# jayleicn/ClipBERT

Measured on AMD Instinct MI355X. Metric: clips/sec/node (2×2 frames, 224px, L_txt=32) at 1/2/4/8 MI355X, higher is better.
Workload: dtype bf16; 1 GPU; MSRVTT retrieval training step (msrvtt_ret_base_resnet50.json; BASELINE configs[1]/[2] family) at the metric's shape: 16 videos x N_clip=2 x N_frame=2 uint8 frames 224px + 2 texts/video (pos+neg, r=2) L_txt=32 per GPU = 32 clips, 64 frames, 64 (text, clip) pairs per step; ImageNorm + fwd + lse-pooling loss + bwd + all-reduce + clip + AdamW in the timed step; clips folded into one forward; mode=train, videos_per_gpu=16, n_clips=2, n_frames=2, img_size=224, txt_len=32, texts_per_video=2, pairs_per_gpu=64, score_agg_func=lse, clips_folded=True, input=uint8 frames in HBM, parallelism=dp1, hip_graph=True, replay_plan=eager hyper-parameter upload + one hipGraph, n_graphs=1, dropout=True

## Files before the change

clipbert_amd/_lib.py:

```python
import ctypes as C
import os

HERE = os.path.dirname(os.path.abspath(__file__))
LIB_PATH = os.path.join(HERE, "lib", "libclipbert_hip.so")

CB_F32, CB_BF16 = 0, 1
ACT_NONE, ACT_RELU, ACT_GELU, ACT_TANH = 0, 1, 2, 3
SPLITK_WS_COUNTER_BYTES = 65536
ACT_GELU_SAVE_GRAD, ACT_SAVED_GRAD = 4, 5
ROWK, ROWK_GATHER, KROW, KROW_TAPS, KROW_GATHER = 0, 1, 2, 3, 4
(HP_LR, HP_BETA1, HP_BETA2, HP_EPS, HP_WD, HP_BC1, HP_BC2, HP_MAX_NORM, HP_GRAD_SCALE, HP_SKIP, HP_COUNT) = range(11)
OPT_ADAMW, OPT_ADAM, OPT_ADAMAX = 0, 1, 2
YUV_LAYOUTS = {"i420": 0, "nv12": 1}
YUV_MATRICES = {"bt601": 0, "bt601-full": 1, "bt709": 2, "bt709-full": 3}

vp, i32, i64, f32, u64 = C.c_void_p, C.c_int32, C.c_int64, C.c_float, C.c_uint64


class GemmDesc(C.Structure):
    _fields_ = [
        ("dtype", i32), ("M", i32), ("N", i32), ("K", i32), ("a_mode", i32), ("b_mode", i32),
        ("A", vp), ("B", vp), ("lda", i64), ("ldb", i64), ("a_tab", vp), ("b_tab", vp),
        ("R", i32), ("S", i32), ("Cin", i32), ("H", i32), ("W", i32),
        ("sH", i64), ("sW", i64), ("flip_taps", i32), ("schedule", i32),
        ("C", vp), ("ldc", i64), ("c_rowmap", vp), ("c_f32", i32), ("accumulate", i32),
        ("split_k", i32), ("act", i32), ("scale", vp), ("shift", vp), ("residual", vp), ("ldr", i64),
        ("relu_after", i32), ("zero_fill_pitch", i32), ("mask", vp), ("ldm", i64), ("C2", vp), ("ldc2", i64),
        ("alpha", f32), ("dropout_p", f32), ("dropout_seed", u64), ("dropout_seed_ptr", vp), ("tile", i32),
        ("xcd_order", i32), ("a_bytes", i64), ("b_bytes", i64), ("gelu_grad_pre", vp), ("ld_gelu", i64), ("a_rowsum", vp),
        ("batch", i32), ("relu_bwd", i32), ("batch_stride_a", i64), ("batch_stride_b", i64), ("batch_stride_c", i64),
        ("batch_stride_rowsum", i64), ("post_scale", vp), ("post_scale2", vp), ("splitk_ws", vp), ("splitk_ws_bytes", i64),
        ("sq_slots", vp), ("sq_slots_n", i64),
    ]


class Res2Desc(C.Structure):
    _fields_ = [("x", vp), ("out", vp), ("w1", vp), ("w2", vp), ("w3", vp), ("wsc", vp),
                ("scale1", vp), ("shift1", vp), ("scale2", vp), ("shift2", vp), ("scale3", vp), ("shift3", vp),
                ("scale_sc", vp), ("shift_sc", vp), ("N", i32), ("H", i32), ("W", i32), ("cin", i32)]


_SIGNATURES = {
    "cb_gemm": [C.POINTER(GemmDesc), vp],
    "cb_res2_block": [C.POINTER(Res2Desc), vp],
    "cb_stem_pool": [vp, vp, vp, vp, vp, i32, i32, i32, i32, i32, i32, i32, vp],
    "cb_stem_pool_u8": [vp, vp, vp, vp, vp, vp, vp, i32, i32, i32, i32, i32, i32, i32, vp],
    "cb_gemm_plan": [vp, i32, vp],
    "cb_gemm_group": [vp, i32, vp],
    "cb_gemm_workspace_bytes": [vp, vp],
    "cb_build_pixel_table": [vp, i32, i32, i32, i32, i32, i64, i64, i64, vp],
    "cb_stem_pack": [i32, vp, i32, vp, vp, vp, i32, i32, i32, i32, i32, i32, vp],
    "cb_resize_pack_u8": [i32, vp, i64, vp, vp, i32, i32, vp, vp, vp, i32, i32, i32, i32, vp],
    "cb_resize_pack_yuv420": [i32, vp, i64, vp, vp, i32, i32, i32, vp, vp, vp, i32, i32, i32, i32, vp],
    "cb_image_norm": [vp, vp, vp, vp, i64, i64, vp],
    "cb_maxpool_fwd": [i32, vp, vp, i32, i32, i32, i32, i32, i32, i32, i32, i32, i32, vp],
    "cb_maxpool2_bwd": [i32, vp, vp, vp, vp, i32, i32, i32, i32, i32, i32, i32, vp],
    "cb_relu_scale_bwd": [i32, vp, vp, vp, vp, vp, vp, vp, i64, i32, vp],
    "cb_layernorm_fwd": [i32, vp, vp, vp, vp, vp, vp, i64, i32, f32, i32, i32, i32, vp],
    "cb_layernorm_bwd": [i32, vp, vp, vp, vp, vp, vp, vp, vp, i64, i32, vp, f32, u64, vp, i32, i32, i32, vp],
    "cb_layernorm_bwd_part": [i32, vp, vp, vp, vp, vp, vp, vp, i32, i64, i32, vp, f32, u64, vp, i32, i32, i32, vp],
    "cb_ln_partials_reduce": [vp, vp, vp, vp, i32, i32, i32, vp],
    "cb_comm_unique_id": [vp],
    "cb_comm_init": [i32, i32, vp],
    "cb_comm_info": [vp, vp],
    "cb_allreduce_bucket": [vp, i64, i32, vp],
    "cb_reduce_scatter_bucket": [vp, vp, i64, i32, vp],
    "cb_allgather_bucket": [vp, vp, i64, i32, vp],
    "cb_broadcast_bucket": [vp, i64, i32, i32, vp],
    "cb_comm_destroy": [],
    "cb_text_embed_fwd": [i32, vp, vp, vp, vp, vp, vp, vp, vp, vp, vp, i32, i32, i32, i32, f32, vp, vp, i32, vp],
    "cb_visual_embed_fwd": [i32, vp, vp, vp, vp, vp, vp, vp, vp, vp, vp, vp, vp, i32, i32, i32, i32, i32,
                            i32, i32, i32, f32, vp, vp],
    "cb_text_embed_bwd": [i32, vp, vp, vp, vp, vp, i32, i32, i32, i32, i64, i32, vp],
    "cb_head_loss": [i32, vp, vp, vp, vp, vp, i64, i32, f32, vp],
    "cb_retrieval_scores": [vp, vp, i64, i32, vp],
    "cb_sq_sum_fold": [vp, vp, i32, vp, i64, vp, vp, i32, vp],
    "cb_mean_fwd": [vp, i64, vp, vp],
    "cb_mean_bwd": [vp, i64, vp, vp],
    "cb_counter_add": [vp, i64, vp],
    "cb_zero": [vp, i64, vp],
    "cb_zero_ranges": [vp, vp, i32, vp],
    "cb_copy_ranges": [vp, vp, vp, i32, vp],
    "cb_visual_embed_bwd": [i32, vp, vp, vp, vp, vp, vp, vp, i32, i32, i32, i32, i32, i32, i32, i32, vp],
    "cb_attention_fwd": [i32, vp, vp, vp, vp, i32, i32, i32, f32, u64, vp, vp],
    "cb_attention_bwd": [i32, vp, vp, vp, vp, vp, vp, vp, i32, i32, i32, f32, u64, vp, vp],
# ... 65 lines not shown
```

clipbert_amd/csrc/common.hip:

```cpp
#include "common.h"

#include <stdarg.h>
#include <stdio.h>

namespace {
thread_local char g_err[512] = "";
}

int cb_fail(const char* fmt, ...) {
    va_list ap;
    va_start(ap, fmt);
    vsnprintf(g_err, sizeof(g_err), fmt, ap);
    va_end(ap);
    return -1;
}

int cb_launch_status(const char* what) {
    hipError_t e = hipGetLastError();
    if (e != hipSuccess) return cb_fail("%s: kernel launch failed: %s", what, hipGetErrorString(e));
    return 0;
}

extern "C" const char* cb_last_error(void) { return g_err; }
extern "C" int cb_version(void) { return 13; }
```

clipbert_amd/csrc/gemm.hip:

```cpp

#include "gemm8_impl.h"
#include "gemm_stream_impl.h"
#include <stdio.h>
#include <vector>

using namespace cbgemm;

namespace cbgemm {
extern template int launch_gemm<float, 64, 64, 2>(const GP&, bool, hipStream_t);
extern template int launch_gemm<bf16, 128, 128, 2>(const GP&, bool, hipStream_t);
extern template int launch_gemm<bf16, 128, 64, 2>(const GP&, bool, hipStream_t);
extern template int launch_gemm<bf16, 64, 64, 3>(const GP&, bool, hipStream_t);
extern template int launch_gemm<bf16, 128, 128, 1, 2>(const GP&, bool, hipStream_t);
extern template int launch_gemm_group<float, 64, 64, 2, 1>(const GroupArgs&, int, hipStream_t);
extern template int launch_gemm_group<bf16, 64, 64, 3, 1>(const GroupArgs&, int, hipStream_t);
extern template int launch_gemm_group<bf16, 128, 128, 1, 2>(const GroupArgs&, int, hipStream_t);
#define CB_G8_DECL(BM, BN, WGM, WGN, NST)                                                             \
    extern template int launch_gemm8_fwd<BM, BN, WGM, WGN, NST>(const GP&, int, float*, hipStream_t);   \
    extern template int launch_gemm8_dgrad<BM, BN, WGM, WGN, NST>(const GP&, int, float*, hipStream_t); \
    extern template int launch_gemm8_wgrad<BM, BN, WGM, WGN, NST>(const GP&, int, float*, hipStream_t);
CB_G8_DECL(256, 256, 2, 4, 2)
CB_G8_DECL(128, 256, 2, 4, 3)
CB_G8_DECL(256, 128, 4, 2, 3)
#undef CB_G8_DECL
// ... 78 lines not shown
#pragma unroll
        for (int r = 0; r < 8; ++r) v[r] += t[r];
    }
    if (p.scale) load8(p.scale + n, sc);
    if (p.shift) load8(p.shift + n, sh);
    const int64_t orow = p.c_rowmap ? (int64_t)p.c_rowmap[m] : (int64_t)m;
    epilogue8<T>(p, v, sc, sh, m, orow, n);
}

template <int BM, int BN, int WGM, int WGN, int NST>
int launch8(int form, const GP& p, int mode, float* ws, hipStream_t st) {
    if (form == 1) return launch_gemm8_fwd<BM, BN, WGM, WGN, NST>(p, mode, ws, st);
    if (form == 2) return launch_gemm8_dgrad<BM, BN, WGM, WGN, NST>(p, mode, ws, st);
    return launch_gemm8_wgrad<BM, BN, WGM, WGN, NST>(p, mode, ws, st);
}

int gemm_prepare(const cb_gemm_desc* d, Prepared& out) {
    CB_REQUIRE(d != nullptr, "cb_gemm: null descriptor");
    CB_REQUIRE(d->dtype == CB_F32 || d->dtype == CB_BF16, "cb_gemm: bad dtype %d", d->dtype);
    CB_REQUIRE(d->M >= 0 && d->N >= 0 && d->K >= 0, "cb_gemm: negative dims");
    CB_REQUIRE(d->A && d->B && d->C, "cb_gemm: null operand");
    const int esz = d->dtype == CB_BF16 ? 2 : 4;
    const int eps = 16 / esz;
    GP& p = out.p;
    p = GP{};
    p.A = d->A; p.B = d->B; p.C = d->C; p.C2 = d->C2; p.residual = d->residual; p.mask = d->mask;
    p.dact_pre = d->gelu_grad_pre; p.ldd = d->ld_gelu; p.a_rowsum = d->a_rowsum;
    p.relu_bwd = d->relu_bwd != 0; p.post_scale = d->post_scale; p.post_scale2 = d->post_scale2;
    if (p.relu_bwd) {
        CB_REQUIRE(d->mask && (!d->c_f32 || d->dtype == CB_F32) && !d->scale && !d->shift && d->act == CB_ACT_NONE && d->dropout_p <= 0.f && !d->relu_after &&
                   !d->gelu_grad_pre && (d->split_k <= 1),
                   "cb_gemm: relu_bwd needs a mask and excludes scale/shift/act/dropout/relu_after/gelu_grad_pre/split_k and an fp32 C next to bf16 operands");
        CB_REQUIRE((!d->post_scale || aligned16(d->post_scale)) && (!d->post_scale2 || aligned16(d->post_scale2)),
                   "cb_gemm: post_scale vectors must be 16-byte aligned");
    } else {
        CB_REQUIRE(!d->post_scale && !d->post_scale2, "cb_gemm: post_scale / post_scale2 need relu_bwd");
    }
    p.batch = d->batch > 1 ? d->batch : 1;
    p.bs_a = d->batch_stride_a * esz; p.bs_b = d->batch_stride_b * esz;
    p.bs_c = d->batch_stride_c * (d->c_f32 ? 4 : esz); p.bs_r = d->batch_stride_rowsum;
    if (p.batch > 1) {
        CB_REQUIRE(!d->C2 && !d->residual && !d->mask && !d->gelu_grad_pre && !d->a_tab && !d->b_tab && !d->c_rowmap,
                   "cb_gemm: batch > 1 supports plain operands only (no residual / mask / second output / gather / row map)");
        CB_REQUIRE((d->batch_stride_a * esz) % 16 == 0 && (d->batch_stride_b * esz) % 16 == 0 && (p.bs_c % 16) == 0,
                   "cb_gemm: batch strides must keep 16-byte alignment");
    }
    CB_REQUIRE(!d->a_rowsum || (d->a_mode == CB_KROW && d->b_mode == CB_KROW), "cb_gemm: a_rowsum needs the weight-gradient form (A and B both CB_KROW)");
    p.scale = d->scale; p.shift = d->shift; p.a_tab = d->a_tab; p.b_tab = d->b_tab; p.c_rowmap = d->c_rowmap; p.zfill = d->zero_fill_pitch;
    p.lda = d->lda; p.ldb = d->ldb; p.ldc = d->ldc; p.ldc2 = d->ldc2; p.ldr = d->ldr; p.ldm = d->ldm;
    p.sH = d->sH; p.sW = d->sW;
    p.M = d->M; p.N = d->N; p.K = d->K;
    p.a_mode = d->a_mode; p.b_mode = d->b_mode;
    p.R = d->R > 0 ? d->R : 1; p.S = d->S > 0 ? d->S : 1; p.Ct = d->Cin; p.H = d->H; p.W = d->W; p.flip = d->flip_taps;
    CB_REQUIRE(d->accumulate >= 0 && d->accumulate <= 2 && (d->accumulate != 2 || d->dtype == CB_BF16), "cb_gemm: bad accumulate %d (2 = first writer: bf16 problems)", d->accumulate);
    p.c_f32 = d->c_f32; p.accumulate = d->accumulate == 1; p.split_k = d->split_k > 0 ? d->split_k : 1;
    p.act = d->act; p.relu_after = d->relu_after;
    p.alpha = d->alpha == 0.f ? 1.f : d->alpha;
    p.dropout_p = d->dropout_p; p.seed = d->dropout_seed; p.seed_ptr = d->dropout_seed_ptr;
    const int bk = d->dtype == CB_BF16 ? Tr<bf16>::BK : Tr<float>::BK;
    p.ktiles = (d->K + bk - 1) / bk;
    {
        const bool ok = d->dtype == CB_BF16 && !d->c_f32 && (int64_t)d->M * (d->ldc > d->ldc2 ? d->ldc : d->ldc2) * 2 * (p.batch) < 0xffffffffll && !d->c_rowmap;
        p.wt = ok ? switches().wt : 0;
    }
    {
        const bool fe_off = switches().fast_epi_off;
        p.fast_epi = 0;
        auto rows_ok = [&](const void* q, int64_t ld) { return q == nullptr || (ld % 8 == 0 && aligned16(q) && (int64_t)d->M * ld * 2 < 0x7fffffffll); };
        const bool wg_store = !fe_off && d->dtype == CB_BF16 && d->c_f32 && d->a_mode == CB_KROW && d->accumulate != 1 && p.alpha == 1.f && !d->scale && !d->shift &&
                              d->act == CB_ACT_NONE && !d->C2 && !d->residual && !d->mask && !d->gelu_grad_pre && d->dropout_p <= 0.f && !d->relu_after && !d->c_rowmap &&
                              !d->zero_fill_pitch && !d->relu_bwd && d->N % 8 == 0 && d->ldc % 8 == 0 && aligned16(d->C) && (int64_t)d->M * d->ldc * 4 < 0xffffffffll;
        if (wg_store) p.fast_epi = FAST_EPI_F32;
        p.sq_slots = nullptr;
        if (d->sq_slots) {
            const int64_t need = (int64_t)((d->M + 63) / 64) * ((d->N + 63) / 64) * p.batch;
            CB_REQUIRE(wg_store, "cb_gemm: sq_slots needs a bf16 weight-gradient form storing an aligned fp32 C with a plain epilogue (accumulate 0 / 2)");
            CB_REQUIRE(d->sq_slots_n >= need, "cb_gemm: sq_slots_n %lld < %lld (one slot per 64x64 tile and batch member)", (long long)d->sq_slots_n, (long long)need);
            p.sq_slots = d->sq_slots;
        }
        const bool plain = !wg_store && !fe_off && p.wt == 1 && p.batch == 1 && d->accumulate != 1 && p.alpha == 1.f && !d->zero_fill_pitch && !d->a_rowsum &&
                           d->N % 8 == 0 && d->ldc % 8 == 0 && aligned16(d->C) && (!d->shift || aligned16(d->shift)) && (!d->scale || aligned16(d->scale)) &&
                           rows_ok(d->residual, d->ldr) && rows_ok(d->mask, d->ldm) && rows_ok(d->gelu_grad_pre, d->ld_gelu) &&
                           !(d->mask && d->gelu_grad_pre);
        if (plain && d->relu_bwd) {
            const bool ok = d->C2 && d->post_scale && d->ldc2 % 8 == 0 && aligned16(d->C2) && (int64_t)d->M * d->ldc2 * 2 < 0xffffffffll;
            const int flags = EF_RBWD | (d->residual ? EF_RES : 0) | (d->post_scale2 ? EF_PS2 : 0);
            if (ok)
                for (int i = 1; i < FAST_EPI_N; ++i)
                    if (FAST_EPI_COMBOS[i] == flags) { p.fast_epi = i; break; }
        } else if (plain) {
            int flags = 0;
            bool ok = true;
            if (d->scale) flags |= EF_SCALE;
            if (d->shift) flags |= EF_SHIFT;
            if (d->act == CB_ACT_RELU) flags |= EF_RELU;
            else if (d->act == CB_ACT_GELU_SAVE_GRAD && d->C2) flags |= EF_GELU2;
            else if (d->act == CB_ACT_GELU && !d->C2) flags |= EF_GELU1;
            else if (d->act == CB_ACT_SAVED_GRAD && d->gelu_grad_pre) flags |= EF_MULAUX;
            else if (d->act != CB_ACT_NONE) ok = false;
            if (d->C2 && !(flags & EF_GELU2)) ok = false;
            if (d->C2) ok = ok && d->ldc2 % 8 == 0 && aligned16(d->C2) && (int64_t)d->M * d->ldc2 * 2 < 0xffffffffll;
            if (d->gelu_grad_pre && !(flags & EF_MULAUX)) ok = false;
            if (d->dropout_p > 0.f) flags |= EF_DROP;
            if (d->residual) flags |= EF_RES;
            if (d->relu_after) flags |= EF_RELU_AFTER;
            if (d->mask) flags |= EF_MASK;
            if (ok)
                for (int i = 1; i < FAST_EPI_N; ++i)
                    if (FAST_EPI_COMBOS[i] == flags) { p.fast_epi = i; break; }
        }
    }
    const bool a_krow = d->a_mode == CB_KROW;
    const bool b_krow = d->b_mode == CB_KROW || d->b_mode == CB_KROW_TAPS || d->b_mode == CB_KROW_GATHER;
    CB_REQUIRE(d->a_mode == CB_ROWK || d->a_mode == CB_ROWK_GATHER || d->a_mode == CB_KROW, "cb_gemm: bad a_mode %d", d->a_mode);
    CB_REQUIRE(d->b_mode == CB_ROWK || b_krow, "cb_gemm: bad b_mode %d", d->b_mode);
    const int taps = p.R * p.S;
    const bool tapped = d->a_mode == CB_ROWK_GATHER || d->b_mode == CB_KROW_TAPS || d->b_mode == CB_KROW_GATHER;
    if (tapped) {
        CB_REQUIRE(p.Ct > 0, "cb_gemm: Cin (channels per tap) must be set for conv modes");
        CB_REQUIRE(p.Ct % eps == 0, "cb_gemm: channels per tap (%d) must be a multiple of %d", p.Ct, eps);
    }
    const int64_t lim = 0x7fffffffll;
    bool fast = d->a_bytes > 0 && d->b_bytes > 0 && d->a_bytes < lim && d->b_bytes < lim && aligned16(d->A) && aligned16(d->B);
    if (d->a_mode == CB_ROWK_GATHER) {
        CB_REQUIRE(d->a_tab, "cb_gemm: a_tab missing");
        CB_REQUIRE(d->K == taps * p.Ct, "cb_gemm: K (%d) != R*S*Cin (%d)", d->K, taps * p.Ct);
        fast = fast && (p.R == 1 || d->sH % eps == 0) && (p.S == 1 || d->sW % eps == 0);
    } else if (d->a_mode == CB_ROWK) {
        fast = fast && (d->lda % eps == 0) && (d->K % eps == 0);
    } else {
        const int64_t need = ((int64_t)(d->K - 1) * d->lda + (d->M + eps - 1) / eps * eps) * esz;
        fast = fast && (d->lda % eps == 0) && (d->M % eps == 0 || need <= d->a_bytes);
    }
    if (d->b_mode == CB_ROWK) {
        fast = fast && (d->ldb % eps == 0) && (d->K % eps == 0);
    } else if (d->b_mode == CB_KROW) {
        const int64_t need = ((int64_t)(d->K - 1) * d->ldb + (d->N + eps - 1) / eps * eps) * esz;
        fast = fast && (d->ldb % eps == 0) && (d->N % eps == 0 || need <= d->b_bytes);
    } else if (d->b_mode == CB_KROW_TAPS) {
        CB_REQUIRE(d->K == taps * p.Ct, "cb_gemm: K (%d) != R*S*Ct (%d)", d->K, taps * p.Ct);
        fast = fast && (d->ldb % eps == 0) && (d->N % eps == 0);
    } else {
        CB_REQUIRE(d->b_tab, "cb_gemm: b_tab missing");
        CB_REQUIRE(d->N == taps * p.Ct, "cb_gemm: N (%d) != R*S*Cin (%d)", d->N, taps * p.Ct);
        fast = fast && (p.R == 1 || d->sH % eps == 0) && (p.S == 1 || d->sW % eps == 0);
    }
    p.a_bytes = (uint32_t)(fast ? d->a_bytes : 0);
    p.b_bytes = (uint32_t)(fast ? d->b_bytes : 0);
    CB_REQUIRE(d->tile >= 0 && d->tile <= 9, "cb_gemm: bad tile %d", d->tile);
    CB_REQUIRE(d->xcd_order >= 0 && d->xcd_order <= 2, "cb_gemm: bad xcd_order %d", d->xcd_order);
    CB_REQUIRE(d->dropout_p >= 0.f && d->dropout_p < 1.f, "cb_gemm: dropout_p out of range");
    const int cesz = d->c_f32 ? 4 : esz;
    bool cv = (d->ldc % 4 == 0) && ((reinterpret_cast<uintptr_t>(d->C) % (4 * cesz)) == 0);
    if (d->C2) cv = cv && (d->ldc2 % 4 == 0) && ((reinterpret_cast<uintptr_t>(d->C2) % (4 * esz)) == 0);
    if (d->residual) cv = cv && (d->ldr % 4 == 0) && ((reinterpret_cast<uintptr_t>(d->residual) % (4 * esz)) == 0);
    if (d->mask) cv = cv && (d->ldm % 4 == 0) && ((reinterpret_cast<uintptr_t>(d->mask) % (4 * esz)) == 0);
    if (d->gelu_grad_pre) cv = cv && (d->ld_gelu % 4 == 0) && ((reinterpret_cast<uintptr_t>(d->gelu_grad_pre) % (4 * esz)) == 0);
    if (d->scale) cv = cv && aligned16(d->scale);
    if (d->shift) cv = cv && aligned16(d->shift);
// ... 50 lines not shown
        return cb_launch_status("cb_gemm (split-K reduce)");
    }
    if (d->dtype == CB_F32) return launch_gemm<float, 64, 64, 2>(p, pr.fast, st);
    CB_STAMP_ASSIGN(p, d, lp.tile, p.split_k, 0, 0, 1);
    if (lp.tile == 4) return launch_gemm<bf16, 128, 128, 1, 2>(p, pr.fast, st);
    if (lp.tile == 1) return launch_gemm<bf16, 128, 128, 2>(p, pr.fast, st);
    if (lp.tile == 3) return launch_gemm<bf16, 128, 64, 2>(p, pr.fast, st);
    return launch_gemm<bf16, 64, 64, 3>(p, pr.fast, st);
}

int gemm_run(const cb_gemm_desc* d, const Prepared& pr, void* stream) {
    LaunchPlan lp;
    const int rc = gemm_choose(d, pr, true, false, lp);
    if (lp.tile != 0 && switches().trace) trace_plan(d, pr, lp);
    return rc != 0 ? rc : gemm_launch(d, pr, lp, cb_stream(stream));
}
}

extern "C" int cb_gemm(const cb_gemm_desc* d, void* stream) {
    Prepared pr;
    bool empty;
    if (int rc = gemm_validate(d, pr, empty)) return rc;
    return empty ? 0 : gemm_run(d, pr, stream);
}

extern "C" int cb_gemm_plan(const cb_gemm_desc* d, int32_t use_table, int32_t* out4) {
    CB_REQUIRE(out4 != nullptr, "cb_gemm_plan: null output");
    out4[0] = out4[1] = out4[2] = out4[3] = 0;
    Prepared pr;
    LaunchPlan lp;
    bool empty;
    if (int rc = gemm_validate(d, pr, empty)) return rc;
    if (empty) return 0;
    if (int rc = gemm_choose(d, pr, use_table != 0, false, lp)) return rc;
    out4[0] = lp.tile; out4[1] = lp.split_k; out4[2] = lp.sched; out4[3] = lp.xcd_remap ? 1 : 2;
    return 0;
}

extern "C" int cb_gemm_workspace_bytes(const cb_gemm_desc* d, int64_t* bytes) {
    CB_REQUIRE(d != nullptr && bytes != nullptr, "cb_gemm_workspace_bytes: null argument");
    *bytes = 0;
    Prepared pr;
    LaunchPlan lp;
    bool empty;
    if (int rc = gemm_validate(d, pr, empty)) return rc;
    if (empty) return 0;
    if (int rc = gemm_choose(d, pr, true, true, lp)) return rc;
    if (lp.slab) *bytes = (int64_t)lp.split_k * pr.p.batch * d->M * d->N * 4 + CB_SPLITK_WS_COUNTER_BYTES;
    return 0;
}

namespace {
int group_class(const cb_gemm_desc* d, const Prepared& pr) {
    if (!pr.fast || d->zero_fill_pitch || d->tile >= 5 || d->tile == 1 || d->tile == 3) return -1;
    if (d->batch > 1 || d->a_rowsum) {
        const bool ok = d->dtype == CB_BF16 && pr.form == FORM_WGRAD && d->split_k <= 1 && d->tile != 2 && !d->c_rowmap;
        return ok ? GC_WGRAD_RS : -1;
    }
    return GROUP_CLASS_OF[pr.form];
}

struct GroupItem { const cb_gemm_desc* d; Prepared pr; int cls; };

bool group_split_free(const GroupItem& it) { return a_reduction_major(it.pr.form) && it.d->c_f32 && it.d->accumulate != 0 && it.pr.epi_scale_only; }
inline int64_t group_tiles(const cb_gemm_desc* d, int B) { return (int64_t)((d->M + B - 1) / B) * ((d->N + B - 1) / B); }

double group_cost(const std::vector<GroupItem*>& g, int tile, int s, int* splits) {
    const int B = tile == 4 ? 128 : 64;
    int maxkt = 1;
    for (auto* it : g) maxkt = it->pr.p.ktiles > maxkt ? it->pr.p.ktiles : maxkt;
    const int kt_target = (maxkt + s - 1) / s;
    int64_t W = 0;
    int kt_per_max = 1;
    double atom = 0.0;
    for (size_t i = 0; i < g.size(); ++i) {
        const cb_gemm_desc* d = g[i]->d;
        const int kt = g[i]->pr.p.ktiles;
        int si = g[i]->pr.p.split_k;
        if (group_split_free(*g[i])) {
            si = (kt + kt_target / 2) / kt_target;
            if (si < 1) si = 1;
            while (si > 1 && kt / si < 4) --si;
        }
        if (si > kt) si = kt > 0 ? kt : 1;
        splits[i] = si;
        W += group_tiles(d, B) * si;
        const int per = (kt + si - 1) / si;
        kt_per_max = per > kt_per_max ? per : kt_per_max;
        if (si > 1) atom += (double)d->M * d->N * 4.0 * si;
    }
    static const int cus = [] {
        int dev = 0, n = 0;
        return (hipGetDevice(&dev) == hipSuccess && hipDeviceGetAttribute(&n, hipDeviceAttributeMultiprocessorCount, dev) == hipSuccess && n > 0) ? n : 256;
    }();
    const int64_t per_cu = (W + cus - 1) / cus;
    double unit;
    if (tile == 4) unit = per_cu <= 1 ? 1.0 : 0.77;
    else unit = per_cu <= 1 ? 0.45 : (per_cu == 2 ? 0.35 : 0.30);
    return 8.0 + (double)per_cu * kt_per_max * unit + atom / 2.0e6;
}

struct GroupPlan {
    int tile = 2;
    int splits[GROUP_MAX];
    float* slab = nullptr;
    int* cnt = nullptr;
};
// ... 155 lines not shown
```

clipbert_amd/csrc/gemm_choose.h:

```cpp
#pragma once
#include "gemm_impl.h"
#include <cmath>
#include "gemm_tuned.h"
#include "gemm_model.h"

namespace cbgemm {
bool skinny_covers(const cb_gemm_desc* d, const GP& p);
}
using namespace cbgemm;

namespace {
inline int env_int(const char* name, int dflt) { const char* v = getenv(name); return v != nullptr ? atoi(v) : dflt; }
struct Switches {
    bool trace = getenv("CB_GEMM_TRACE") != nullptr;
    bool no_tuned = getenv("CB_GEMM_NO_TUNED") != nullptr;
    bool no_model = getenv("CB_GEMM_NO_MODEL") != nullptr;
    bool no_xcd_remap = getenv("CB_GEMM_NO_XCD_REMAP") != nullptr;
    bool no_stream = getenv("CB_GEMM_NO_STREAM") != nullptr;
    bool no_group = getenv("CB_GEMM_NO_GROUP") != nullptr;
    bool no_skinny = getenv("CB_GEMM_NO_SKINNY") != nullptr;
    bool group_slab_off = env_int("CB_GROUP_SLAB", 1) == 0;
    bool fast_epi_off = env_int("CB_GEMM_FAST_EPI", 1) == 0;
    int wt = env_int("CB_GEMM_WT", 1);
};
// ... 11 lines not shown
};
Form operand_form(int a_mode, int b_mode, int taps) {
    if (a_mode == CB_KROW) return b_mode == CB_KROW ? FORM_WGRAD : (b_mode == CB_KROW_GATHER ? FORM_WGRAD_GATHER : FORM_WGRAD_OTHER);
    if (b_mode == CB_ROWK) return a_mode == CB_ROWK ? FORM_FWD : FORM_FWD_GATHER;
    if (a_mode == CB_ROWK && (b_mode == CB_KROW || (b_mode == CB_KROW_TAPS && taps == 1))) return FORM_DGRAD;
    if (a_mode == CB_ROWK_GATHER && b_mode == CB_KROW_TAPS) return FORM_DGRAD_TAPS;
    return FORM_DGRAD_OTHER;
}
inline bool a_reduction_major(Form f) { return f >= FORM_WGRAD; }
inline int model_form(Form f) { return f >= FORM_WGRAD ? 2 : (f >= FORM_DGRAD ? 1 : 0); }
const int FORM8_OF[8] = {1, 1, 2, 2, 0, 3, 3, 0};
const int GROUP_CLASS_OF[8] = {GC_FWD, GC_FWD_GATHER, -1, -1, -1, GC_WGRAD, GC_WGRAD_GATHER, -1};

struct Prepared {
    GP p;
    bool fast, cv8;
    Form form;
    int taps;
    bool epi_scale_only;
    bool atomics_ok;
};
constexpr int GROUP_COUNTERS = CB_SPLITK_WS_COUNTER_BYTES / (int)sizeof(int);
inline int64_t splitk_payload_bytes(int64_t ws_bytes) { return ws_bytes > CB_SPLITK_WS_COUNTER_BYTES ? ws_bytes - CB_SPLITK_WS_COUNTER_BYTES : 0; }
inline int* splitk_counters(void* ws, int64_t ws_bytes) {
    return ws && ws_bytes > CB_SPLITK_WS_COUNTER_BYTES ? reinterpret_cast<int*>(reinterpret_cast<unsigned char*>(ws) + (ws_bytes - CB_SPLITK_WS_COUNTER_BYTES)) : nullptr;
}

struct ModelPick { int tile = 0, split = 0, sched = 0; double us = 1e300; };
const int MODEL_TILE_ID[7] = {2, 3, 1, 4, 5, 6, 7};
const int MODEL_BM[7] = {64, 128, 128, 128, 256, 128, 256};
const int MODEL_BN[7] = {64, 64, 128, 128, 256, 256, 128};

double model_us(int ti, int form, int64_t M, int64_t N, int64_t K, int64_t batch, int s, bool taps, bool m2, int c_esz) {
    using namespace cbgemm;
    const double* g = MODEL_G;
    const int64_t wg = ((M + MODEL_BM[ti] - 1) / MODEL_BM[ti]) * ((N + MODEL_BN[ti] - 1) / MODEL_BN[ti]) * batch * s;
    const int64_t kt = ((K + 63) / 64 + s - 1) / s;
    const double r = (double)wg / (256.0 * MODEL_OCC[ti]);
    const double q = ti >= 4 ? g[7] : g[3];
    const double rounds = q * std::ceil(r - 1e-9) + (1.0 - q) * (r > 1.0 ? r : 1.0);
    const double ck = MODEL_C[ti][form] * (1.0 + g[4] * (taps ? 1 : 0)) * (1.0 + g[8] * (m2 ? 1 : 0));
    const double ab = (double)(M * K + N * K) * 2.0 * batch, cb = (double)M * N * batch * c_esz;
    const double red = (ti >= 4 && s > 1) ? (double)M * N * batch * s * 8.0 : 0.0;
    const double atom = (ti < 4 && s > 1) ? (double)M * N * batch * s * 4.0 : 0.0;
    return MODEL_A[ti] + rounds * (MODEL_B[ti][form] + kt * ck) + ab / (g[0] * 1e6) + cb / (g[5] * 1e6) + red / (g[1] * 1e6) + atom / (g[2] * 1e6) +
           g[6] * (m2 ? 1 : 0);
}

ModelPick model_pick(const cb_gemm_desc* d, const Prepared& pr, bool can8, int64_t ws_bytes, bool free_split) {
    const GP& p = pr.p;
    const int form = model_form(pr.form), split_caller = p.split_k;
    const bool taps = pr.taps > 1;
    const int c_esz = d->c_f32 ? 4 : 2;
    const int64_t M = d->M, N = d->N, K = d->K, batch = p.batch;
    ModelPick best;
    auto consider = [&](int ti, int s, int sched) {
        const double us = model_us(ti, form, M, N, K, batch, s, taps, sched == 3, c_esz);
        if (us < best.us) { best.us = us; best.tile = MODEL_TILE_ID[ti]; best.split = s; best.sched = sched; }
    };
    static const int SPLITS4[] = {1, 2, 3, 4, 6, 8, 12, 16, 24, 32, 48};
    for (int ti = 0; ti < 4; ++ti) {
        if (N <= 64 && ti >= 2) continue;
        consider(ti, split_caller, 0);
        if (free_split)
            for (int s : SPLITS4)
                if (s != split_caller && s <= (p.ktiles / 4 > 1 ? p.ktiles / 4 : 1)) consider(ti, s, 0);
    }
    if (can8)
        for (int ti = 4; ti < 7; ++ti) {
            const int64_t tiles = ((M + MODEL_BM[ti] - 1) / MODEL_BM[ti]) * ((N + MODEL_BN[ti] - 1) / MODEL_BN[ti]) * batch;
            int cand[3] = {1, 0, 0};
            int n = 1;
            for (int target : {256, 512}) {
                const int s = (int)std::lround((double)target / (double)tiles);
                if (s > 1 && p.ktiles / s >= 2 && (int64_t)s * batch * M * N * 4 <= ws_bytes && s != cand[1]) cand[n++] = s;
            }
            for (int i = 0; i < n; ++i) { consider(ti, cand[i], 1); consider(ti, cand[i], 3); }
        }
    return best;
}

int stream_variant(const cb_gemm_desc* d, const Prepared& pr) {
    const GP& p = pr.p;
    if (!pr.fast || !pr.cv8 || d->dtype != CB_BF16 || pr.form != FORM_FWD || p.batch > 1 || p.split_k > 1) return -1;
    if (d->c_f32 || d->accumulate || d->c_rowmap || d->zero_fill_pitch || d->a_rowsum || d->gelu_grad_pre || d->dropout_p > 0.f || d->mask || d->relu_bwd ||
        d->C2) return -1;
    if (d->K % 8 != 0 || d->M < 64) return -1;
    if ((int64_t)d->M * (d->N > d->K ? d->N : d->K) * 2 >= 0x7fffffffll) return -1;
    if (p.ktiles == 1 && d->N % 256 == 0) return 0;
    if (p.ktiles == 2 && d->N % 128 == 0) return 1;
    return -1;
}

struct LaunchPlan {
    int tile = 0;
    int split_k = 1;
    int sched = 0;
    bool xcd_remap = false;
    bool slab = false;
    bool c_vec8 = false;
    int form8 = 0;
    int picked = 0;
};
struct Pick { int tile = 0, split = 0, sched = 0; };
constexpr int64_t WS_UNLIMITED = (int64_t)1 << 60;
constexpr int STREAM_MIN_ROWS = 32768;

int gemm_choose(const cb_gemm_desc* d, const Prepared& pr, bool use_table, bool assume_ws, LaunchPlan& lp) {
    const Switches& sw = switches();
    const GP& p = pr.p;
    const bool bf = d->dtype == CB_BF16, explicit_tile = d->tile != 0;
    const int split_caller = p.split_k;
    lp = LaunchPlan{};
    const bool covers9 = skinny_covers(d, p);
    CB_REQUIRE(d->tile != 9 || covers9, "cb_gemm: tile 9 (few rows) does not cover this problem (bf16, A k-contiguous, B k-contiguous or aligned reduction-major, no batch / K split / row sums)");
    if (d->tile == 9 || (!explicit_tile && use_table && !sw.no_skinny && covers9 && d->M <= 64)) { lp.tile = 9; return 0; }
    const int sv = stream_variant(d, pr);
    CB_REQUIRE(d->tile != 8 || sv >= 0, "cb_gemm: tile 8 (streaming) does not cover this problem (M=%d N=%d K=%d modes %d/%d)", d->M, d->N, d->K, d->a_mode, d->b_mode);
    const cbgemm::TunedEntry* tabled =
        (bf && use_table && !sw.no_tuned) ? cbgemm::tuned_lookup(d->a_mode, d->b_mode, d->M, d->N, d->K, p.batch, pr.taps, split_caller) : nullptr;
    if (d->tile == 8 || (!explicit_tile && use_table && !sw.no_stream && !tabled && sv >= 0 && d->M >= STREAM_MIN_ROWS && d->N <= 512)) {
        lp.tile = 8; lp.sched = sv; lp.c_vec8 = true;
        return 0;
    }

    const int form8 = (bf && pr.fast && pr.cv8 && (pr.form != FORM_DGRAD_TAPS || p.Ct % 64 == 0)) ? FORM8_OF[pr.form] : 0;
    const int64_t ws_room = assume_ws ? splitk_payload_bytes(WS_UNLIMITED)
                                      : (d->splitk_ws && aligned16(d->splitk_ws) ? splitk_payload_bytes(d->splitk_ws_bytes) : 0);
    const bool free_split = !explicit_tile && a_reduction_major(pr.form) && pr.atomics_ok;
    const int xcd = d->xcd_order != 0 ? d->xcd_order : (tabled ? tabled->xcd : 0);
    auto model = [&](bool allow8) {
        Pick k;
        if (!bf || sw.no_model) return k;
        const ModelPick mp = model_pick(d, pr, allow8 && form8 != 0, ws_room, free_split && !d->a_rowsum && p.batch == 1);
        k.tile = mp.tile; k.split = (mp.tile >= 5 || mp.split != split_caller) ? mp.split : 0; k.sched = mp.sched;
        return k;
    };
    auto split8 = [&](const Pick& k) { return explicit_tile ? split_caller : (k.split > 0 ? k.split : 1); };
    Pick pick;
    if (explicit_tile) pick.tile = d->tile;
    else if (tabled) pick = Pick{tabled->tile, tabled->new_split, tabled->sched};
    if (pick.tile >= 5 && form8 == 0) pick = Pick{};
    if (pick.tile == 0) pick = model(true);
    if (pick.tile >= 5 && d->sq_slots && split8(pick) > 1) pick = model(false);
    if (pick.tile >= 5) {
        int split = split8(pick);
        if (split > p.ktiles) split = p.ktiles;
        if (split > 1) {
            const int per = (p.ktiles + split - 1) / split;
            split = (p.ktiles + per - 1) / per;
            if ((int64_t)split * p.batch * d->M * d->N * 4 > ws_room) {
                pick = model(!explicit_tile);
                split = pick.split > 0 ? pick.split : 1;
            }
        }
        if (pick.tile >= 5) {
            lp.tile = lp.picked = pick.tile; lp.form8 = form8;
            lp.split_k = split; lp.slab = split > 1;
            lp.sched = d->schedule > 0 ? d->schedule : (pick.sched > 0 ? pick.sched : 3);
            lp.c_vec8 = true;
            lp.xcd_remap = !sw.no_xcd_remap && xcd != 2;
            CB_REQUIRE(d->schedule >= 0 && d->schedule <= 3, "cb_gemm: bad schedule %d", d->schedule);
            return 0;
        }
    }

    lp.picked = pick.tile; lp.form8 = form8;
    lp.tile = pick.tile == 0 ? 2 : pick.tile;
    if (!bf) lp.tile = 2;
    else if ((lp.tile == 1 || lp.tile == 4) && d->N <= 64) lp.tile = 3;
    lp.xcd_remap = !sw.no_xcd_remap && xcd != 2;
    int split = split_caller;
    if (d->tile >= 5 && split > 1 && !pr.atomics_ok) split = 1;
    if (d->accumulate == 2 || d->sq_slots) split = 1;
    if (pick.split > 0 && free_split) split = pick.split;
    if (split > 1) {
        CB_REQUIRE(d->c_f32 && d->accumulate == 1, "cb_gemm: split_k > 1 needs an fp32 output that is accumulated into (accumulate = 1)");
        CB_REQUIRE(pr.epi_scale_only, "cb_gemm: split_k > 1 supports only scale/alpha in the epilogue");
        if (split > p.ktiles) split = p.ktiles;
// ... 10 lines not shown
```

clipbert_amd/csrc/gemm_impl.h:

```cpp
#pragma once
#include "common.h"
#include <stdlib.h>
#include <type_traits>

namespace cbgemm {


constexpr int NTHREADS = 256;

template <typename T> struct Tr;
template <> struct Tr<bf16> { static constexpr int EPS = 8, BK = 64, SEGS = 8, ROWB = 128, RB = 8; };
template <> struct Tr<float> { static constexpr int EPS = 4, BK = 32, SEGS = 8, ROWB = 144, RB = 4; };

template <typename T> __device__ __forceinline__ int lds_off(int row, int seg);
template <> __device__ __forceinline__ int lds_off<bf16>(int row, int seg) { return row * 128 + ((seg ^ (row & 7)) << 4); }
template <> __device__ __forceinline__ int lds_off<float>(int row, int seg) { return row * 144 + (seg << 4); }

struct GP {
    const void* A; const void* B; void* C; void* C2; const void* residual; const void* mask;
    const void* dact_pre; float* a_rowsum; int64_t ldd;
    int relu_bwd; const float* post_scale; const float* post_scale2;
    int batch; int64_t bs_a, bs_b, bs_c, bs_r;
    const float* scale; const float* shift;
    const cb_pixel* a_tab; const cb_pixel* b_tab; const int32_t* c_rowmap;
    int64_t lda, ldb, ldc, ldc2, ldr, ldm, sH, sW;
    int M, N, K;
    int a_mode, b_mode;
    int R, S, Ct, H, W, flip;
    int c_f32, accumulate, split_k, act, relu_after;
    float alpha, dropout_p;
    uint64_t seed;
    const uint64_t* seed_ptr;
    short c_vec, c_vec8;
    short xcd_remap;
    short wt;
    int zfill;
    uint32_t a_bytes, b_bytes;
    int ktiles;
    int slab_base, cnt_base;
    int fast_epi;
    float* sq_slots;
#ifdef CB_STAMPS
    unsigned long long* stamps;
#endif
};

enum { EF_SCALE = 1, EF_SHIFT = 2, EF_RELU = 4, EF_GELU2 = 8, EF_DROP = 16, EF_RES = 32, EF_RELU_AFTER = 64, EF_MASK = 128, EF_MULAUX = 256,
       EF_RBWD = 512,
       EF_PS2 = 1024,
       EF_F32 = 2048,
       EF_GELU1 = 4096 };
constexpr int FAST_EPI_COMBOS[] = {
    -1,
    0,
    EF_SHIFT,
    EF_SHIFT | EF_GELU2,
    EF_SHIFT | EF_DROP | EF_RES,
    EF_SHIFT | EF_RES,
    EF_MULAUX,
    EF_RES,
    EF_SCALE | EF_SHIFT | EF_RELU,
    EF_SCALE | EF_SHIFT,
    EF_SCALE | EF_SHIFT | EF_RES | EF_RELU_AFTER,
    EF_SCALE | EF_MASK,
    EF_RBWD,
    EF_RBWD | EF_RES,
    EF_RBWD | EF_PS2,
    EF_RBWD | EF_PS2 | EF_RES,
    EF_F32,
    EF_SHIFT | EF_GELU1,
};
constexpr int FAST_EPI_F32 = 16;
constexpr int FAST_EPI_N = sizeof(FAST_EPI_COMBOS) / sizeof(int);

#ifdef CB_STAMPS
constexpr int CB_STAMP_WGS = 512, CB_STAMP_REC = 6, CB_STAMP_HDR = 3;
constexpr int CB_STAMP_AREA = CB_STAMP_HDR + CB_STAMP_WGS * CB_STAMP_REC;
struct Stamps {
    unsigned long long t[5];
    __device__ __forceinline__ void mark(int i) { t[i] = __builtin_amdgcn_s_memrealtime(); }
    __device__ __forceinline__ void flush(unsigned long long* area, unsigned lin, int tid) {
        if (!area || tid != 0) return;
        asm volatile("s_waitcnt vmcnt(0)" ::: "memory");
        const unsigned long long t4 = __builtin_amdgcn_s_memrealtime();
        atomicMin(area, t[0]);
        atomicMax(area + 1, t4);
        atomicAdd(area + 2, 1ull);
        if (lin < (unsigned)CB_STAMP_WGS) {
            unsigned long long* r = area + CB_STAMP_HDR + (size_t)lin * CB_STAMP_REC;
            r[0] = t[0]; r[1] = t[1]; r[2] = t[2]; r[3] = t[3]; r[4] = t4;
            unsigned hw;
            asm volatile("s_getreg_b32 %0, hwreg(HW_REG_HW_ID)" : "=s"(hw));
            unsigned xcc;
            asm volatile("s_getreg_b32 %0, hwreg(HW_REG_XCC_ID)" : "=s"(xcc));
            r[5] = ((unsigned long long)xcc << 32) | hw;
        }
    }
};
#define CB_STAMP_DECL() Stamps stamps_
#define CB_STAMP(i) stamps_.mark(i)
#define CB_STAMP_FLUSH(p, lin, tid) stamps_.flush((p).stamps, (lin), (tid))
#else
#define CB_STAMP_DECL() do {} while (0)
#define CB_STAMP(i) do {} while (0)
#define CB_STAMP_FLUSH(p, lin, tid) do {} while (0)
#endif

template <typename T> __device__ __forceinline__ u32x4 load_guarded(const T* src, int nvalid) {
    constexpr int EPS = Tr<T>::EPS;
    union { u32x4 v; T e[EPS]; } u;
#pragma unroll
    for (int i = 0; i < EPS; ++i) u.e[i] = (i < nvalid) ? src[i] : (T)0.f;
    return u.v;
}

constexpr uint32_t OOB = 0x80000000u;
typedef decltype(__builtin_amdgcn_make_buffer_rsrc((void*)nullptr, (short)0, 0, 0)) rsrc_t;
__device__ __forceinline__ rsrc_t make_rsrc(const void* p, uint32_t bytes) {
    return __builtin_amdgcn_make_buffer_rsrc(const_cast<void*>(p), (short)0, (int)bytes, 0x00020000);
}
__device__ __forceinline__ u32x4 bload16(rsrc_t r, uint32_t off) { return __builtin_amdgcn_raw_buffer_load_b128(r, off, 0, 0); }

struct Opnd {
    const void* base; const cb_pixel* tab; int64_t ld; int mode; uint32_t bytes;
};

template <typename T, int ROWS, bool FAST> struct RowkLoader {
    using X = Tr<T>;
    static constexpr bool TR = false;
    static constexpr bool KROW = false;
    static constexpr int NS = ROWS * X::SEGS / NTHREADS;
    static constexpr int ESZ = (int)sizeof(T);
    static_assert(ROWS * X::SEGS % NTHREADS == 0, "tile/threads mismatch");
    struct Stage { u32x4 r[NS]; };
    int64_t off[NS];
    uint32_t boff[NS];
    int ih[NS], iw[NS];
    bool ok[NS];
    int c, rr, ss;
    bool gather;
    rsrc_t rs;
    const T* base;

    __device__ __forceinline__ void init(const GP& p, const Opnd& o, int row0, int bound, int kt0, int tid) {
        gather = o.mode == CB_ROWK_GATHER;
        base = reinterpret_cast<const T*>(o.base);
        if constexpr (FAST) rs = make_rsrc(o.base, o.bytes);
        int k = kt0 * X::BK + (tid % X::SEGS) * X::EPS;
        c = k; rr = 0; ss = 0;
        if (gather) {
            int tap = k / p.Ct;
            c = k - tap * p.Ct;
            rr = tap / p.S; ss = tap - rr * p.S;
        }
#pragma unroll
        for (int i = 0; i < NS; ++i) {
            int idx = tid + i * NTHREADS;
            int row = row0 + idx / X::SEGS;
            ok[i] = row < bound;
            ih[i] = 0; iw[i] = 0;
            int64_t e = (int64_t)row * o.ld;
            if (gather) {
                cb_pixel px = {0, 0, 0};
                if (ok[i]) px = o.tab[row];
                e = px.off; ih[i] = px.ih0; iw[i] = px.iw0;
            }
            off[i] = e;
            boff[i] = ok[i] ? (uint32_t)e * (uint32_t)ESZ : OOB;
        }
    }
    template <bool CHECK> __device__ __forceinline__ void load(Stage& st, const GP& p) {
        const bool kv = gather ? (rr < p.R) : (c < p.K);
        const int klim = gather ? p.Ct : p.K;
        const int64_t tapoff = gather ? (rr * p.sH + ss * p.sW) : 0;
#pragma unroll
// ... 25 lines not shown
template <typename T, int ROWS, bool FAST> struct KrowLoader {
    using X = Tr<T>;
    static constexpr bool TR = false;
    static constexpr bool KROW = true;
    static constexpr int RBLK = ROWS / X::RB;
    static constexpr int CNT = RBLK * (X::BK / 4);
    static constexpr int NI = (CNT + NTHREADS - 1) / NTHREADS;
    static constexpr int ESZ = (int)sizeof(T);
    struct Stage { u32x4 r[NI][4]; };
    int mode, bound;
    int64_t ld;
    const cb_pixel* tab;
    const T* base;
    rsrc_t rs;
    int kb0[NI];
    int co[NI], tap[NI];
    int row[NI];
    int rr[NI], ss[NI];
    int64_t rowoff[NI];
    bool act[NI];

    __device__ __forceinline__ void init(const GP& p, const Opnd& o, int row0, int bnd, int kt0, int tid) {
        mode = o.mode; bound = bnd; ld = o.ld; tab = o.tab;
        base = reinterpret_cast<const T*>(o.base);
        if constexpr (FAST) rs = make_rsrc(o.base, o.bytes);
#pragma unroll
        for (int it = 0; it < NI; ++it) {
            int b = tid + it * NTHREADS;
            act[it] = b < CNT;
            int rb = b % RBLK, kb = b / RBLK;
            row[it] = row0 + rb * X::RB;
            kb0[it] = kt0 * X::BK + kb * 4;
            rowoff[it] = row[it];
            co[it] = kb0[it]; tap[it] = 0; rr[it] = 0; ss[it] = 0;
            if (mode == CB_KROW_TAPS) {
                tap[it] = kb0[it] / p.Ct;
                co[it] = kb0[it] - tap[it] * p.Ct;
            } else if (mode == CB_KROW_GATHER) {
                int tp = row[it] / p.Ct;
                int ch = row[it] - tp * p.Ct;
                rr[it] = tp / p.S; ss[it] = tp - rr[it] * p.S;
                rowoff[it] = rr[it] * p.sH + ss[it] * p.sW + ch;
            }
        }
    }
    template <bool CHECK> __device__ __forceinline__ void load(Stage& st, const GP& p) {
        u32x4 z = {0u, 0u, 0u, 0u};
#pragma unroll
        for (int it = 0; it < NI; ++it) {
            if (!act[it]) { st.r[it][0] = z; st.r[it][1] = z; st.r[it][2] = z; st.r[it][3] = z; continue; }
            const int nvalid = bound - row[it];
            int64_t ro = rowoff[it];
            if (mode == CB_KROW_TAPS) {
                int tapw = p.flip ? (p.R * p.S - 1 - tap[it]) : tap[it];
                ro = (int64_t)tapw * bound + row[it];
            }
#pragma unroll
            for (int j = 0; j < 4; ++j) {
                const int k = kb0[it] + j;
                bool v = k < p.K && nvalid > 0;
                int64_t e;
                if (mode == CB_KROW_GATHER) {
                    cb_pixel px = {0, 0, 0};
                    if (v) px = tab[k];
                    v = v && (unsigned)(px.ih0 + rr[it]) < (unsigned)p.H && (unsigned)(px.iw0 + ss[it]) < (unsigned)p.W;
                    e = px.off + ro;
                } else if (mode == CB_KROW_TAPS) {
                    e = (int64_t)(co[it] + j) * ld + ro;
                } else {
                    e = (int64_t)k * ld + ro;
                }
                if constexpr (FAST) {
                    st.r[it][j] = bload16(rs, v ? (uint32_t)e * (uint32_t)ESZ : OOB);
                } else {
                    st.r[it][j] = v ? load_guarded<T>(base + e, nvalid) : z;
                }
            }
            kb0[it] += X::BK;
            if (mode == CB_KROW_TAPS) {
                co[it] += X::BK;
                while (co[it] >= p.Ct) { co[it] -= p.Ct; ++tap[it]; }
            }
        }
    }
    __device__ __forceinline__ void store(const Stage& st, unsigned char* tile, int tid) const {
#pragma unroll
        for (int it = 0; it < NI; ++it) {
            int b = tid + it * NTHREADS;
            if (b >= CNT) continue;
            int rb = b % RBLK, kb = b / RBLK;
            int r0 = rb * X::RB;
            if constexpr (sizeof(T) == 2) {
#pragma unroll
                for (int d = 0; d < 4; ++d) {
                    uint32_t a0 = st.r[it][0][d], a1 = st.r[it][1][d], a2 = st.r[it][2][d], a3 = st.r[it][3][d];
                    u32x2 even = {(a0 & 0xffffu) | (a1 << 16), (a2 & 0xffffu) | (a3 << 16)};
                    u32x2 odd = {(a0 >> 16) | (a1 & 0xffff0000u), (a2 >> 16) | (a3 & 0xffff0000u)};
                    *reinterpret_cast<u32x2*>(tile + lds_off<T>(r0 + 2 * d, kb >> 1) + (kb & 1) * 8) = even;
                    *reinterpret_cast<u32x2*>(tile + lds_off<T>(r0 + 2 * d + 1, kb >> 1) + (kb & 1) * 8) = odd;
                }
            } else {
#pragma unroll
                for (int e = 0; e < 4; ++e) {
                    u32x4 o = {st.r[it][0][e], st.r[it][1][e], st.r[it][2][e], st.r[it][3][e]};
                    *reinterpret_cast<u32x4*>(tile + lds_off<T>(r0 + e, kb)) = o;
                }
            }
// ... 91 lines not shown
    const cb_pixel* tab;
    uint32_t ldb;
    uint32_t voff[NI];
    int kb0[NI];
    int co[NI], tap[NI];
    int rr[NI], ss[NI];
    cb_pixel px[NI][KB];
    bool act[NI];
    uint32_t bound;

    __device__ __forceinline__ void init(const GP& p, const Opnd& o, int row0, int bnd, int kt0, int tid) {
        rs = make_rsrc(o.base, o.bytes);
        tab = o.tab; ldb = (uint32_t)o.ld * ESZ; bound = (uint32_t)bnd;
#pragma unroll
        for (int it = 0; it < NI; ++it) {
            const int b = ((tid + SHIFT) % NTHREADS) + it * NTHREADS;
            const int kb = b % NKB, rb = b / NKB;
            const int row = row0 + rb * X::RB;
            act[it] = (b < CNT) && (row < bnd);
            kb0[it] = kt0 * X::BK + kb * KB;
            co[it] = kb0[it]; tap[it] = 0; rr[it] = 0; ss[it] = 0;
            if constexpr (KMODE == KM_PLAIN) {
                voff[it] = ((uint32_t)kb0[it] * (uint32_t)o.ld + (uint32_t)row) * ESZ;
            } else if constexpr (KMODE == KM_TAPS) {
                tap[it] = kb0[it] / p.Ct;
                co[it] = kb0[it] - tap[it] * p.Ct;
                voff[it] = (uint32_t)row * ESZ;
            } else {
                const int tp = row / p.Ct, ch = row - tp * p.Ct;
                rr[it] = tp / p.S; ss[it] = tp - rr[it] * p.S;
                voff[it] = (uint32_t)(rr[it] * (int)p.sH + ss[it] * (int)p.sW + ch) * ESZ;
#pragma unroll
                for (int j = 0; j < KB; ++j) {
                    cb_pixel e = {0, (int16_t)-30000, (int16_t)-30000};
                    if (act[it] && kb0[it] + j < p.K) e = tab[kb0[it] + j];
                    px[it][j] = e;
                }
            }
        }
    }
    template <bool CHECK> __device__ __forceinline__ void load(Stage& st, const GP& p) {
#pragma unroll
        for (int it = 0; it < NI; ++it) {
            if constexpr (KMODE == KM_PLAIN) {
#pragma unroll
                for (int j = 0; j < KB; ++j) {
                    bool v = act[it];
                    if (CHECK) v = v && (kb0[it] + j < p.K);
                    st.r[it][j] = bload16(rs, v ? voff[it] + (uint32_t)j * ldb : OOB);
                }
                voff[it] += X::BK * ldb;
                kb0[it] += X::BK;
            } else if constexpr (KMODE == KM_TAPS) {
                const int tapw = p.flip ? (p.R * p.S - 1 - tap[it]) : tap[it];
                const bool v = act[it] && tap[it] < p.R * p.S;
                const uint32_t base = (uint32_t)co[it] * ldb + (uint32_t)tapw * bound * ESZ + voff[it];
#pragma unroll
                for (int j = 0; j < KB; ++j) st.r[it][j] = bload16(rs, v ? base + (uint32_t)j * ldb : OOB);
                co[it] += X::BK;
                while (co[it] >= p.Ct) { co[it] -= p.Ct; ++tap[it]; }
            } else {
#pragma unroll
                for (int j = 0; j < KB; ++j) {
                    const cb_pixel e = px[it][j];
                    const bool v = (unsigned)(e.ih0 + rr[it]) < (unsigned)p.H && (unsigned)(e.iw0 + ss[it]) < (unsigned)p.W;
                    st.r[it][j] = bload16(rs, v ? (uint32_t)e.off * ESZ + voff[it] : OOB);
                }
                kb0[it] += X::BK;
#pragma unroll
                for (int j = 0; j < KB; ++j) {
                    cb_pixel e = {0, (int16_t)-30000, (int16_t)-30000};
                    if (act[it] && kb0[it] + j < p.K) e = tab[kb0[it] + j];
                    px[it][j] = e;
                }
            }
        }
    }
    __device__ __forceinline__ void store(const Stage& st, unsigned char* tile, int tid) const {
#pragma unroll
        for (int it = 0; it < NI; ++it) {
            const int b = ((tid + SHIFT) % NTHREADS) + it * NTHREADS;
            if (b >= CNT) continue;
            const int kb = b % NKB, rb = b / NKB;
            const int r0 = rb * X::RB;
            if constexpr (sizeof(T) == 2 && KB == 8) {
#pragma unroll
                for (int d = 0; d < 4; ++d) {
                    u32x4 even, odd;
#pragma unroll
                    for (int q = 0; q < 4; ++q) {
                        even[q] = __builtin_amdgcn_perm(st.r[it][2 * q + 1][d], st.r[it][2 * q][d], 0x05040100u);
                        odd[q] = __builtin_amdgcn_perm(st.r[it][2 * q + 1][d], st.r[it][2 * q][d], 0x07060302u);
                    }
                    *reinterpret_cast<u32x4*>(tile + lds_off<T>(r0 + 2 * d, kb)) = even;
                    *reinterpret_cast<u32x4*>(tile + lds_off<T>(r0 + 2 * d + 1, kb)) = odd;
                }
            } else if constexpr (sizeof(T) == 2 && KB == 2) {
#pragma unroll
                for (int d = 0; d < 4; ++d) {
                    const uint32_t even = __builtin_amdgcn_perm(st.r[it][1][d], st.r[it][0][d], 0x05040100u);
                    const uint32_t odd = __builtin_amdgcn_perm(st.r[it][1][d], st.r[it][0][d], 0x07060302u);
                    *reinterpret_cast<uint32_t*>(tile + lds_off<T>(r0 + 2 * d, kb >> 2) + (kb & 3) * 4) = even;
                    *reinterpret_cast<uint32_t*>(tile + lds_off<T>(r0 + 2 * d + 1, kb >> 2) + (kb & 3) * 4) = odd;
                }
            } else if constexpr (sizeof(T) == 2) {
#pragma unroll
                for (int d = 0; d < 4; ++d) {
// ... 45 lines not shown
    static constexpr int CH = ROWS / 8;
    static constexpr int NS = CH * X::BK / NTHREADS;
    static_assert(CH * X::BK % NTHREADS == 0, "tile/threads mismatch");
    static constexpr uint32_t ESZ = 2;
    struct Stage { u32x4 r[NS]; };
    rsrc_t rs;
    const cb_pixel* tab;
    uint32_t ldb, bound;
    uint32_t voff[NS];
    int kl[NS];
    int co[NS], tap[NS];
    int rr, ss;
    cb_pixel px[NS];
    bool act[NS];

    __device__ __forceinline__ void init(const GP& p, const Opnd& o, int row0, int bnd, int kt0, int tid) {
        rs = make_rsrc(o.base, o.bytes);
        tab = o.tab; ldb = (uint32_t)o.ld * ESZ; bound = (uint32_t)bnd;
        rr = 0; ss = 0;
#pragma unroll
        for (int i = 0; i < NS; ++i) {
            const int idx = tid + i * NTHREADS;
            const int chunk = idx % CH, kline = idx / CH;
            const int row = row0 + chunk * 8;
            act[i] = row < bnd;
            kl[i] = kt0 * X::BK + kline;
            co[i] = kl[i]; tap[i] = 0;
            if constexpr (KMODE == KM_PLAIN) {
                voff[i] = ((uint32_t)kl[i] * (uint32_t)o.ld + (uint32_t)row) * ESZ;
            } else if constexpr (KMODE == KM_TAPS) {
                tap[i] = kl[i] / p.Ct;
                co[i] = kl[i] - tap[i] * p.Ct;
                voff[i] = (uint32_t)row * ESZ;
            } else {
                const int tp = row / p.Ct, ch = row - tp * p.Ct;
                rr = tp / p.S; ss = tp - rr * p.S;
                voff[i] = (uint32_t)(rr * (int)p.sH + ss * (int)p.sW + ch) * ESZ;
                cb_pixel e = {0, (int16_t)-30000, (int16_t)-30000};
                if (act[i] && kl[i] < p.K) e = tab[kl[i]];
                px[i] = e;
            }
        }
    }
    template <bool CHECK> __device__ __forceinline__ void load(Stage& st, const GP& p) {
#pragma unroll
        for (int i = 0; i < NS; ++i) {
            if constexpr (KMODE == KM_PLAIN) {
                bool v = act[i];
                if (CHECK) v = v && (kl[i] < p.K);
                st.r[i] = bload16(rs, v ? voff[i] : OOB);
                voff[i] += X::BK * ldb;
                kl[i] += X::BK;
            } else if constexpr (KMODE == KM_TAPS) {
                const int tapw = p.flip ? (p.R * p.S - 1 - tap[i]) : tap[i];
                const bool v = act[i] && tap[i] < p.R * p.S;
                st.r[i] = bload16(rs, v ? (uint32_t)co[i] * ldb + (uint32_t)tapw * bound * ESZ + voff[i] : OOB);
                co[i] += X::BK;
                while (co[i] >= p.Ct) { co[i] -= p.Ct; ++tap[i]; }
            } else {
                const cb_pixel e = px[i];
                const bool v = (unsigned)(e.ih0 + rr) < (unsigned)p.H && (unsigned)(e.iw0 + ss) < (unsigned)p.W;
                st.r[i] = bload16(rs, v ? (uint32_t)e.off * ESZ + voff[i] : OOB);
                kl[i] += X::BK;
                cb_pixel nx = {0, (int16_t)-30000, (int16_t)-30000};
                if (act[i] && kl[i] < p.K) nx = tab[kl[i]];
                px[i] = nx;
            }
        }
    }
    __device__ __forceinline__ void store(const Stage& st, unsigned char* tile, int tid) const {
#pragma unroll
        for (int i = 0; i < NS; ++i) {
            const int idx = tid + i * NTHREADS;
            const int chunk = idx % CH, kline = idx / CH;
            *reinterpret_cast<u32x4*>(tile + kline * (ROWS * 2) + ((chunk ^ tr_chunk_swz<ROWS>(kline)) << 4)) = st.r[i];
        }
    }
};

struct TileId { int bx, by, bz; };
__device__ __forceinline__ TileId tile_id(const GP& p) {
    TileId t;
    if (!p.xcd_remap) { t.bx = blockIdx.x; t.by = blockIdx.y; t.bz = blockIdx.z; return t; }
    const unsigned gx = gridDim.x, gy = gridDim.y;
    const unsigned total = gx * gy * gridDim.z;
    const unsigned lin = blockIdx.x + gx * (blockIdx.y + gy * blockIdx.z);
    const unsigned xcd = lin & 7u, i = lin >> 3;
    const unsigned q = total >> 3, r = total & 7u;
    const unsigned l2 = (xcd < r ? xcd * (q + 1) : r * (q + 1) + (xcd - r) * q) + i;
    t.bx = (int)(l2 % gx);
    const unsigned rest = l2 / gx;
    t.by = (int)(rest % gy);
    t.bz = (int)(rest / gy);
    return t;
}

__device__ __forceinline__ void apply_batch(GP& p, TileId& t) {
    if (p.batch <= 1) return;
    const int b = t.bz / p.split_k;
    t.bz -= b * p.split_k;
    const int64_t oa = b * p.bs_a, ob = b * p.bs_b;
    p.A = reinterpret_cast<const unsigned char*>(p.A) + oa;
    p.B = reinterpret_cast<const unsigned char*>(p.B) + ob;
    p.C = reinterpret_cast<unsigned char*>(p.C) + b * p.bs_c;
    if (p.a_bytes) p.a_bytes -= (uint32_t)oa;
    if (p.b_bytes) p.b_bytes -= (uint32_t)ob;
    if (p.a_rowsum) p.a_rowsum += b * p.bs_r;
}

template <typename T>
__device__ __forceinline__ float act_of(int act, float v) {
    if constexpr (sizeof(T) == 2) {
        if (act == CB_ACT_GELU || act == CB_ACT_GELU_SAVE_GRAD) return gelu_erf_pk(v);
    }
    return apply_act(act, v);
}

template <typename T>
__device__ __forceinline__ float scale_shift(float x, float sc, float sh) {
    if constexpr (sizeof(T) == 2) return __builtin_fmaf(x, sc, sh);
    else {
#pragma clang fp contract(off)
        const float t = x * sc;
        return t + sh;
    }
}

template <typename T>
__device__ __forceinline__ void epilogue_vec(const GP& p, f32x4 v, int m, int64_t orow, int nb) {
    v = v * p.alpha;
    if (p.relu_bwd) {
        T* c = reinterpret_cast<T*>(p.C) + orow * p.ldc + nb;
        if (p.accumulate) v = v + load4(c);
        if (p.residual) v = v + load4(reinterpret_cast<const T*>(p.residual) + orow * p.ldr + nb);
        const f32x4 mk = load4(reinterpret_cast<const T*>(p.mask) + orow * p.ldm + nb);
#pragma unroll
        for (int r = 0; r < 4; ++r) v[r] = mk[r] > 0.f ? v[r] : 0.f;
        if (p.C2) store4(reinterpret_cast<T*>(p.C2) + orow * p.ldc2 + nb, p.post_scale2 ? v * load4(p.post_scale2 + nb) : v);
        store4(c, p.post_scale ? v * load4(p.post_scale + nb) : v);
        return;
    }
    if (p.scale && p.shift) {
        const f32x4 sc = load4(p.scale + nb), sh = load4(p.shift + nb);
#pragma unroll
        for (int r = 0; r < 4; ++r) v[r] = scale_shift<T>(v[r], sc[r], sh[r]);
    }
    else if (p.scale) v = v * load4(p.scale + nb);
    else if (p.shift) v = v + load4(p.shift + nb);
    if (p.act == CB_ACT_GELU_SAVE_GRAD && p.C2) {
        f32x4 dv;
#pragma unroll
        for (int r = 0; r < 4; ++r) {
            float y, dy;
            if constexpr (sizeof(T) == 2) gelu_erf_both_pk(v[r], y, dy);
            else gelu_erf_both(v[r], y, dy);
            v[r] = y; dv[r] = dy;
        }
        store4(reinterpret_cast<T*>(p.C2) + orow * p.ldc2 + nb, dv);
    } else {
        if (p.C2) store4(reinterpret_cast<T*>(p.C2) + orow * p.ldc2 + nb, v);
        if (p.act != CB_ACT_NONE) {
#pragma unroll
            for (int r = 0; r < 4; ++r) v[r] = act_of<T>(p.act, v[r]);
        }
    }
    if (p.dropout_p > 0.f) {
        v = v * dropout_mult4(p.seed, (uint64_t)m * ((p.N + 3) >> 2) + (nb >> 2), p.dropout_p);
    }
    if (p.residual) v = v + load4(reinterpret_cast<const T*>(p.residual) + orow * p.ldr + nb);
    if (p.relu_after) {
#pragma unroll
        for (int r = 0; r < 4; ++r) v[r] = v[r] > 0.f ? v[r] : 0.f;
    }
    if (p.mask) {
        f32x4 mk = load4(reinterpret_cast<const T*>(p.mask) + orow * p.ldm + nb);
#pragma unroll
        for (int r = 0; r < 4; ++r) v[r] = mk[r] > 0.f ? v[r] : 0.f;
    }
    if (p.dact_pre) {
        f32x4 pr = load4(reinterpret_cast<const T*>(p.dact_pre) + orow * p.ldd + nb);
#pragma unroll
        for (int r = 0; r < 4; ++r) v[r] *= p.act == CB_ACT_SAVED_GRAD ? pr[r] : gelu_erf_grad(pr[r]);
    }
    if (p.c_f32) {
        float* c = reinterpret_cast<float*>(p.C) + orow * p.ldc + nb;
        if (p.split_k > 1) {
#pragma unroll
            for (int r = 0; r < 4; ++r) atomicAdd(c + r, v[r]);
        } else {
            if (p.accumulate) v = v + load4(c);
            store4(c, v);
        }
    } else {
        T* c = reinterpret_cast<T*>(p.C) + orow * p.ldc + nb;
        if (p.accumulate) v = v + load4(c);
        store4(c, v);
    }
}

template <typename T>
__device__ __forceinline__ void epilogue_elem(const GP& p, float x, int m, int64_t orow, int n) {
    x *= p.alpha;
    if (p.relu_bwd) {
        T* c = reinterpret_cast<T*>(p.C) + orow * p.ldc + n;
        if (p.accumulate) x += to_f32(*c);
        if (p.residual) x += to_f32(reinterpret_cast<const T*>(p.residual)[orow * p.ldr + n]);
        x = to_f32(reinterpret_cast<const T*>(p.mask)[orow * p.ldm + n]) > 0.f ? x : 0.f;
        if (p.C2) reinterpret_cast<T*>(p.C2)[orow * p.ldc2 + n] = from_f32<T>(p.post_scale2 ? x * p.post_scale2[n] : x);
        *c = from_f32<T>(p.post_scale ? x * p.post_scale[n] : x);
        return;
    }
    if (p.scale && p.shift) x = scale_shift<T>(x, p.scale[n], p.shift[n]);
    else if (p.scale) x *= p.scale[n];
    else if (p.shift) x += p.shift[n];
    if (p.act == CB_ACT_GELU_SAVE_GRAD && p.C2) {
        float dx;
        if constexpr (sizeof(T) == 2) gelu_erf_both_pk(x, x, dx);
        else gelu_erf_both(x, x, dx);
        reinterpret_cast<T*>(p.C2)[orow * p.ldc2 + n] = from_f32<T>(dx);
    } else {
        if (p.C2) reinterpret_cast<T*>(p.C2)[orow * p.ldc2 + n] = from_f32<T>(x);
        x = act_of<T>(p.act, x);
    }
    if (p.dropout_p > 0.f) x *= dropout_mult1(p.seed, (uint64_t)m * ((p.N + 3) >> 2) + (n >> 2), n & 3, p.dropout_p);
    if (p.residual) x += to_f32(reinterpret_cast<const T*>(p.residual)[orow * p.ldr + n]);
    if (p.relu_after) x = x > 0.f ? x : 0.f;
    if (p.mask) x = to_f32(reinterpret_cast<const T*>(p.mask)[orow * p.ldm + n]) > 0.f ? x : 0.f;
    if (p.dact_pre) {
        const float t = to_f32(reinterpret_cast<const T*>(p.dact_pre)[orow * p.ldd + n]);
        x *= p.act == CB_ACT_SAVED_GRAD ? t : gelu_erf_grad(t);
    }
    if (p.c_f32) {
        float* c = reinterpret_cast<float*>(p.C) + orow * p.ldc + n;
        if (p.split_k > 1) atomicAdd(c, x);
        else *c = p.accumulate ? (*c + x) : x;
    } else {
        T* c = reinterpret_cast<T*>(p.C) + orow * p.ldc + n;
        *c = from_f32<T>(p.accumulate ? (to_f32(*c) + x) : x);
    }
}

__device__ __forceinline__ void load8(const float* q, float (&v)[8]) {
    f32x4 a = load4(q), b = load4(q + 4);
#pragma unroll
    for (int r = 0; r < 4; ++r) { v[r] = a[r]; v[4 + r] = b[r]; }
}
__device__ __forceinline__ void load8(const bf16* q, float (&v)[8]) {
    bf16x8 x = *reinterpret_cast<const bf16x8*>(q);
#pragma unroll
    for (int r = 0; r < 8; ++r) v[r] = (float)x[r];
}
__device__ __forceinline__ void store8(float* q, const float (&v)[8]) {
    f32x4 a = {v[0], v[1], v[2], v[3]}, b = {v[4], v[5], v[6], v[7]};
    store4(q, a); store4(q + 4, b);
}
__device__ __forceinline__ void store8(bf16* q, const float (&v)[8]) {
    bf16x8 x;
#pragma unroll
    for (int r = 0; r < 8; ++r) x[r] = (bf16)v[r];
    *reinterpret_cast<bf16x8*>(q) = x;
}

template <int AUX = 16 >
__device__ __forceinline__ void store8_wt(void* base, int64_t elem_off, const float (&v)[8]) {
    union { bf16x8 x; u32x4 r; } u;
#pragma unroll
    for (int r = 0; r < 8; ++r) u.x[r] = (bf16)v[r];
    const rsrc_t rs = __builtin_amdgcn_make_buffer_rsrc(base, (short)0, (int)0xffffffffu, 0x00020000);
    __builtin_amdgcn_raw_buffer_store_b128(u.r, rs, (uint32_t)(elem_off * 2), 0, AUX);
}

template <typename T>
__device__ __forceinline__ void zero_patch8(T* base, int64_t ld, int64_t orow, int n, int pitch) {
    const float z[8] = {0.f, 0.f, 0.f, 0.f, 0.f, 0.f, 0.f, 0.f};
    store8(base + (orow + 1) * ld + n, z);
    store8(base + (orow + pitch) * ld + n, z);
    store8(base + (orow + pitch + 1) * ld + n, z);
}

#ifdef CB_EPI_NOSTORE
#define CB_EPI_ST(...) do { if (p.alpha == 12345.f) { __VA_ARGS__; } } while (0)
#else
#define CB_EPI_ST(...) do { __VA_ARGS__; } while (0)
#endif
template <typename T, int EPF = 0>
__device__ __forceinline__ void epilogue8(const GP& p, float (&v)[8], const float (&sc)[8], const float (&sh)[8],
                                          int m, int64_t orow, int n, bf16x8 rpre = bf16x8{}, bf16x8 apre = bf16x8{}) {
    auto load_res = [&](float (&t)[8]) {
        if constexpr (EPF == 2) {
#pragma unroll
            for (int r = 0; r < 8; ++r) t[r] = (float)rpre[r];
        } else load8(reinterpret_cast<const T*>(p.residual) + orow * p.ldr + n, t);
    };
    auto load_aux = [&](const void* base, int64_t ld, float (&t)[8]) {
        if constexpr (EPF >= 1) {
#pragma unroll
            for (int r = 0; r < 8; ++r) t[r] = (float)apre[r];
        } else load8(reinterpret_cast<const T*>(base) + orow * ld + n, t);
    };
#ifdef CB_EPI_NOMATH
    if constexpr (sizeof(T) == 2) {
        if (!p.c_f32 && p.wt) {
            store8_wt(p.C, orow * p.ldc + n, v);
            if (p.C2) store8_wt(p.C2, orow * p.ldc2 + n, v);
            return;
        }
    }
#endif
#pragma unroll
    for (int r = 0; r < 8; ++r) v[r] *= p.alpha;
    if (p.relu_bwd) {
        T* c = reinterpret_cast<T*>(p.C) + orow * p.ldc + n;
        float t[8];
        if (p.accumulate) {
            load8(c, t);
#pragma unroll
            for (int r = 0; r < 8; ++r) v[r] += t[r];
        }
        if (p.residual) {
            load_res(t);
#pragma unroll
            for (int r = 0; r < 8; ++r) v[r] += t[r];
        }
        load_aux(p.mask, p.ldm, t);
#pragma unroll
        for (int r = 0; r < 8; ++r) v[r] = t[r] > 0.f ? v[r] : 0.f;
        if (p.C2) {
            float u[8];
            if (p.post_scale2) {
                load8(p.post_scale2 + n, t);
#pragma unroll
                for (int r = 0; r < 8; ++r) u[r] = v[r] * t[r];
            } else {
#pragma unroll
                for (int r = 0; r < 8; ++r) u[r] = v[r];
            }
            if constexpr (sizeof(T) == 2) {
                if (p.wt) CB_EPI_ST(store8_wt(p.C2, orow * p.ldc2 + n, u));
                else CB_EPI_ST(store8(reinterpret_cast<T*>(p.C2) + orow * p.ldc2 + n, u));
            } else CB_EPI_ST(store8(reinterpret_cast<T*>(p.C2) + orow * p.ldc2 + n, u));
        }
        if (p.post_scale) {
            load8(p.post_scale + n, t);
#pragma unroll
            for (int r = 0; r < 8; ++r) v[r] *= t[r];
        }
        if constexpr (sizeof(T) == 2) {
            if (p.wt) CB_EPI_ST(store8_wt(p.C, orow * p.ldc + n, v));
            else CB_EPI_ST(store8(c, v));
        } else CB_EPI_ST(store8(c, v));
        if (p.zfill) {
            zero_patch8(reinterpret_cast<T*>(p.C), p.ldc, orow, n, p.zfill);
            if (p.C2) zero_patch8(reinterpret_cast<T*>(p.C2), p.ldc2, orow, n, p.zfill);
        }
        return;
    }
    if (p.scale && p.shift) {
#pragma unroll
        for (int r = 0; r < 8; ++r) v[r] = scale_shift<T>(v[r], sc[r], sh[r]);
    } else if (p.scale) {
#pragma unroll
        for (int r = 0; r < 8; ++r) v[r] *= sc[r];
    } else if (p.shift) {
#pragma unroll
        for (int r = 0; r < 8; ++r) v[r] += sh[r];
    }
    const bool save_grad = p.act == CB_ACT_GELU_SAVE_GRAD && p.C2 != nullptr;
    float dv[8];
    if (save_grad) {
#pragma unroll
        for (int r = 0; r < 8; r += 2) {
            if constexpr (sizeof(T) == 2) {
                f32x2 y, dy;
                gelu_erf_both2(f32x2{v[r], v[r + 1]}, y, dy);
                v[r] = y[0]; v[r + 1] = y[1]; dv[r] = dy[0]; dv[r + 1] = dy[1];
            } else {
                gelu_erf_both(v[r], v[r], dv[r]);
                gelu_erf_both(v[r + 1], v[r + 1], dv[r + 1]);
            }
        }
    }
    if (p.C2) {
        const float (&w)[8] = save_grad ? dv : v;
        if constexpr (sizeof(T) == 2) {
            if (p.wt & 2) CB_EPI_ST(store8_wt<18 >(p.C2, orow * p.ldc2 + n, w));
            else if (p.wt) CB_EPI_ST(store8_wt(p.C2, orow * p.ldc2 + n, w));
            else CB_EPI_ST(store8(reinterpret_cast<T*>(p.C2) + orow * p.ldc2 + n, w));
        } else CB_EPI_ST(store8(reinterpret_cast<T*>(p.C2) + orow * p.ldc2 + n, w));
    }
    if (p.act != CB_ACT_NONE && !save_grad) {
#pragma unroll
        for (int r = 0; r < 8; ++r) v[r] = act_of<T>(p.act, v[r]);
    }
    if (p.dropout_p > 0.f) {
        const uint64_t grp = (uint64_t)m * ((p.N + 3) >> 2) + (n >> 2);
        const f32x4 d0 = dropout_mult4(p.seed, grp, p.dropout_p), d1 = dropout_mult4(p.seed, grp + 1, p.dropout_p);
#pragma unroll
        for (int r = 0; r < 4; ++r) { v[r] *= d0[r]; v[4 + r] *= d1[r]; }
    }
    if (p.residual) {
        float t[8];
        load_res(t);
#pragma unroll
        for (int r = 0; r < 8; ++r) v[r] += t[r];
    }
    if (p.relu_after) {
#pragma unroll
        for (int r = 0; r < 8; ++r) v[r] = v[r] > 0.f ? v[r] : 0.f;
    }
    if (p.mask) {
        float t[8];
        load_aux(p.mask, p.ldm, t);
#pragma unroll
        for (int r = 0; r < 8; ++r) v[r] = t[r] > 0.f ? v[r] : 0.f;
    } else if (p.dact_pre) {
        float t[8];
        load_aux(p.dact_pre, p.ldd, t);
        if (p.act == CB_ACT_SAVED_GRAD) {
#pragma unroll
            for (int r = 0; r < 8; ++r) v[r] *= t[r];
        } else {
#pragma unroll
            for (int r = 0; r < 8; ++r) v[r] *= gelu_erf_grad(t[r]);
        }
    }
    if (p.c_f32) {
        float* c = reinterpret_cast<float*>(p.C) + orow * p.ldc + n;
        if (p.accumulate) {
            float t[8];
            load8(c, t);
#pragma unroll
            for (int r = 0; r < 8; ++r) v[r] += t[r];
        }
        CB_EPI_ST(store8(c, v));
    } else {
        T* c = reinterpret_cast<T*>(p.C) + orow * p.ldc + n;
        if (p.accumulate) {
            float t[8];
            load8(c, t);
#pragma unroll
            for (int r = 0; r < 8; ++r) v[r] += t[r];
        }
        if constexpr (sizeof(T) == 2) {
            if (p.wt) CB_EPI_ST(store8_wt(p.C, orow * p.ldc + n, v));
            else CB_EPI_ST(store8(c, v));
        } else CB_EPI_ST(store8(c, v));
    }
    if (p.zfill) {
        if (p.c_f32) zero_patch8(reinterpret_cast<float*>(p.C), p.ldc, orow, n, p.zfill);
        else zero_patch8(reinterpret_cast<T*>(p.C), p.ldc, orow, n, p.zfill);
        if (p.C2) zero_patch8(reinterpret_cast<T*>(p.C2), p.ldc2, orow, n, p.zfill);
    }
}

__device__ __forceinline__ u32x4 pack_bf16x8(const f32x2 (&v)[4]) {
    union { bf16x8 x; u32x4 r; } u;
#pragma unroll
    for (int r = 0; r < 4; ++r) { u.x[2 * r] = (bf16)v[r][0]; u.x[2 * r + 1] = (bf16)v[r][1]; }
    return u.r;
}
__device__ __forceinline__ void unpack_bf16x8(u32x4 raw, f32x2 (&v)[4]) {
    union { u32x4 r; bf16x8 x; } u;
    u.r = raw;
#pragma unroll
    for (int r = 0; r < 4; ++r) v[r] = f32x2{(float)u.x[2 * r], (float)u.x[2 * r + 1]};
}

template <int FLAGS, int NT, int BN, int PR, int NPASS, typename StageFn>
__device__ __forceinline__ void fast_epilogue(const GP& p, unsigned char* smem, int m0, int n0, int tid, StageFn stage, const bf16x8* pre_r = nullptr,
                                              const bf16x8* pre_a = nullptr, int tile_lin = 0) {
    constexpr int SROW = BN * 4 + 16, CPR = BN / 8, ITER = PR * CPR / NT, RSTEP = NT / CPR, NCH = NPASS * ITER;
    static_assert(PR * CPR % NT == 0 && NT % CPR == 0, "chunk map");
    constexpr bool HAS_RES = (FLAGS & EF_RES) != 0, HAS_AUX = (FLAGS & (EF_MASK | EF_MULAUX | EF_RBWD)) != 0;
    constexpr bool ALL = NCH <= 8;
    constexpr bool ROLL = (FLAGS & (EF_GELU2 | EF_GELU1)) != 0 || NPASS > 2;
    const int cc = tid % CPR, n = n0 + cc * 8, rl0 = tid / CPR;
    const bool nok = n < p.N;
    const unsigned char* const read_base = smem + rl0 * SROW + cc * 32;
    const rsrc_t rc = __builtin_amdgcn_make_buffer_rsrc(p.C, (short)0, (int)0xffffffffu, 0x00020000);
    const rsrc_t rc2 = __builtin_amdgcn_make_buffer_rsrc((FLAGS & (EF_GELU2 | EF_RBWD)) ? p.C2 : p.C, (short)0, (int)0xffffffffu, 0x00020000);
    constexpr uint32_t CESZ = (FLAGS & EF_F32) ? 4u : 2u;
    const uint32_t ldcb = (uint32_t)p.ldc * CESZ, ldc2b = (uint32_t)p.ldc2 * 2u, nb = (uint32_t)n * 2u;
    float sq = 0.f;
    const rsrc_t rr = make_rsrc(HAS_RES ? p.residual : p.C, HAS_RES ? (uint32_t)((int64_t)p.M * p.ldr * 2) : 0u);
    const void* auxp = (FLAGS & (EF_MASK | EF_RBWD)) ? p.mask : p.dact_pre;
    const int64_t lda = (FLAGS & (EF_MASK | EF_RBWD)) ? p.ldm : p.ldd;
    const rsrc_t ra = make_rsrc(HAS_AUX ? auxp : p.C, HAS_AUX ? (uint32_t)((int64_t)p.M * lda * 2) : 0u);
    const uint32_t ldrb = (uint32_t)p.ldr * 2u, ldab = (uint32_t)lda * 2u;
    f32x2 sc[4], sh[4];
#pragma unroll
    for (int r = 0; r < 4; ++r) { sc[r] = f32x2{1.f, 1.f}; sh[r] = f32x2{0.f, 0.f}; }
    if (nok) {
        if constexpr ((FLAGS & EF_SCALE) != 0) {
            const f32x4 a = load4(p.scale + n), b = load4(p.scale + n + 4);
            sc[0] = f32x2{a[0], a[1]}; sc[1] = f32x2{a[2], a[3]}; sc[2] = f32x2{b[0], b[1]}; sc[3] = f32x2{b[2], b[3]};
        }
        if constexpr ((FLAGS & EF_SHIFT) != 0) {
            const f32x4 a = load4(p.shift + n), b = load4(p.shift + n + 4);
            sh[0] = f32x2{a[0], a[1]}; sh[1] = f32x2{a[2], a[3]}; sh[2] = f32x2{b[0], b[1]}; sh[3] = f32x2{b[2], b[3]};
        }
        if constexpr ((FLAGS & EF_RBWD) != 0) {
            const f32x4 a = load4(p.post_scale + n), b = load4(p.post_scale + n + 4);
            sc[0] = f32x2{a[0], a[1]}; sc[1] = f32x2{a[2], a[3]}; sc[2] = f32x2{b[0], b[1]}; sc[3] = f32x2{b[2], b[3]};
            if constexpr ((FLAGS & EF_PS2) != 0) {
                const f32x4 c = load4(p.post_scale2 + n), e = load4(p.post_scale2 + n + 4);
                sh[0] = f32x2{c[0], c[1]}; sh[1] = f32x2{c[2], c[3]}; sh[2] = f32x2{e[0], e[1]}; sh[3] = f32x2{e[2], e[3]};
            }
        }
    }
    u32x4 res[HAS_RES ? (ALL ? NCH : ITER) : 1], aux[HAS_AUX ? (ALL ? NCH : ITER) : 1];
    auto request = [&](int h) __attribute__((always_inline)) {
#pragma unroll
        for (int it = 0; it < ITER; ++it) {
            const int m = m0 + h * PR + rl0 + it * RSTEP;
            const bool ok = m < p.M && nok;
            const int slot = (ALL ? h * ITER : 0) + it;
            if constexpr (HAS_RES) {
                if (ALL && pre_r) { union { bf16x8 x; u32x4 r; } u; u.x = pre_r[h * ITER + it]; res[slot] = u.r; }
                else res[slot] = bload16(rr, ok ? (uint32_t)m * ldrb + nb : OOB);
            }
            if constexpr (HAS_AUX) {
                if (ALL && pre_a) { union { bf16x8 x; u32x4 r; } u; u.x = pre_a[h * ITER + it]; aux[slot] = u.r; }
                else aux[slot] = bload16(ra, ok ? (uint32_t)m * ldab + nb : OOB);
            }
        }
    };
    auto chunk = [&](int h, int it, int slot) __attribute__((always_inline)) {
        const int m = m0 + h * PR + rl0 + it * RSTEP;
        if (!(m < p.M && nok)) return;
        const f32x4 a = *reinterpret_cast<const f32x4*>(read_base + it * RSTEP * SROW);
        const f32x4 b = *reinterpret_cast<const f32x4*>(read_base + it * RSTEP * SROW + 16);
        if constexpr ((FLAGS & EF_F32) != 0) {
            union { f32x4 f; u32x4 r; } ua, ub;
            ua.f = a; ub.f = b;
            const uint32_t off = (uint32_t)m * ldcb + (uint32_t)n * 4u;
            __builtin_amdgcn_raw_buffer_store_b128(ua.r, rc, off, 0, 0);
            __builtin_amdgcn_raw_buffer_store_b128(ub.r, rc, off + 16u, 0, 0);
            sq += (a[0] * a[0] + a[1] * a[1]) + (a[2] * a[2] + a[3] * a[3]) + (b[0] * b[0] + b[1] * b[1]) + (b[2] * b[2] + b[3] * b[3]);
            return;
        }
        f32x2 v[4] = {f32x2{a[0], a[1]}, f32x2{a[2], a[3]}, f32x2{b[0], b[1]}, f32x2{b[2], b[3]}};
        if constexpr ((FLAGS & EF_RBWD) != 0) {
            f32x2 t[4];
            if constexpr (HAS_RES) {
                unpack_bf16x8(res[slot], t);
#pragma unroll
                for (int r = 0; r < 4; ++r) v[r] = v[r] + t[r];
            }
            unpack_bf16x8(aux[slot], t);
            f32x2 u[4];
#pragma unroll
            for (int r = 0; r < 4; ++r) {
                v[r] = f32x2{t[r][0] > 0.f ? v[r][0] : 0.f, t[r][1] > 0.f ? v[r][1] : 0.f};
                u[r] = (FLAGS & EF_PS2) != 0 ? v[r] * sh[r] : v[r];
                v[r] = v[r] * sc[r];
            }
            __builtin_amdgcn_raw_buffer_store_b128(pack_bf16x8(u), rc2, (uint32_t)m * ldc2b + nb, 0, 16 );
            __builtin_amdgcn_raw_buffer_store_b128(pack_bf16x8(v), rc, (uint32_t)m * ldcb + nb, 0, 16 );
            return;
        }
#pragma unroll
        for (int r = 0; r < 4; ++r) {
            if constexpr ((FLAGS & EF_SCALE) != 0 && (FLAGS & EF_SHIFT) != 0) v[r] = pk_fma(v[r], sc[r], sh[r]);
            else if constexpr ((FLAGS & EF_SCALE) != 0) v[r] = v[r] * sc[r];
            else if constexpr ((FLAGS & EF_SHIFT) != 0) v[r] = v[r] + sh[r];
        }
        if constexpr ((FLAGS & EF_GELU2) != 0) {
            f32x2 dv[4];
#pragma unroll
            for (int r = 0; r < 4; ++r) gelu_erf_both2(v[r], v[r], dv[r]);
            __builtin_amdgcn_raw_buffer_store_b128(pack_bf16x8(dv), rc2, (uint32_t)m * ldc2b + nb, 0, 16 );
        }
        if constexpr ((FLAGS & EF_GELU1) != 0) {
#pragma unroll
            for (int r = 0; r < 4; ++r) { f32x2 dv; gelu_erf_both2(v[r], v[r], dv); }
        }
        if constexpr ((FLAGS & EF_RELU) != 0) {
#pragma unroll
            for (int r = 0; r < 4; ++r) v[r] = f32x2{fmaxf(v[r][0], 0.f), fmaxf(v[r][1], 0.f)};
        }
        if constexpr ((FLAGS & EF_DROP) != 0) {
            const uint64_t grp = (uint64_t)m * ((p.N + 3) >> 2) + (n >> 2);
            const f32x4 d0 = dropout_mult4(p.seed, grp, p.dropout_p), d1 = dropout_mult4(p.seed, grp + 1, p.dropout_p);
            v[0] = v[0] * f32x2{d0[0], d0[1]}; v[1] = v[1] * f32x2{d0[2], d0[3]};
            v[2] = v[2] * f32x2{d1[0], d1[1]}; v[3] = v[3] * f32x2{d1[2], d1[3]};
        }
        if constexpr (HAS_RES) {
            f32x2 t[4];
            unpack_bf16x8(res[slot], t);
#pragma unroll
            for (int r = 0; r < 4; ++r) v[r] = v[r] + t[r];
        }
        if constexpr ((FLAGS & EF_RELU_AFTER) != 0) {
#pragma unroll
            for (int r = 0; r < 4; ++r) v[r] = f32x2{fmaxf(v[r][0], 0.f), fmaxf(v[r][1], 0.f)};
        }
        if constexpr (HAS_AUX) {
            f32x2 t[4];
            unpack_bf16x8(aux[slot], t);
#pragma unroll
            for (int r = 0; r < 4; ++r) {
                if constexpr ((FLAGS & EF_MASK) != 0) v[r] = f32x2{t[r][0] > 0.f ? v[r][0] : 0.f, t[r][1] > 0.f ? v[r][1] : 0.f};
                else v[r] = v[r] * t[r];
            }
        }
        __builtin_amdgcn_raw_buffer_store_b128(pack_bf16x8(v), rc, (uint32_t)m * ldcb + nb, 0, 16 );
    };
    auto pass = [&](int h) __attribute__((always_inline)) {
        if constexpr ((HAS_RES || HAS_AUX) && !ALL) request(h);
        __syncthreads();
        stage(h);
        __syncthreads();
        if constexpr ((FLAGS & (EF_GELU2 | EF_GELU1)) != 0) {
#pragma unroll 1
            for (int it = 0; it < ITER; ++it) chunk(h, it, 0);
        } else {
#pragma unroll
            for (int it = 0; it < ITER; ++it) chunk(h, it, (ALL ? h * ITER : 0) + it);
        }
    };
    if constexpr ((HAS_RES || HAS_AUX) && ALL) {
#pragma unroll
        for (int h = 0; h < NPASS; ++h) request(h);
    }
    if constexpr (ROLL && !((HAS_RES || HAS_AUX) && ALL)) {
#pragma unroll 1
        for (int h = 0; h < NPASS; ++h) pass(h);
    } else {
#pragma unroll
        for (int h = 0; h < NPASS; ++h) pass(h);
    }
    if constexpr ((FLAGS & EF_F32) != 0) {
        if (p.sq_slots) {
            sq = wave_sum(sq);
            __syncthreads();
            float* red = reinterpret_cast<float*>(smem);
            if ((tid & 63) == 0) red[tid >> 6] = sq;
            __syncthreads();
            if (tid == 0) {
                float t = 0.f;
#pragma unroll
                for (int w = 0; w < NT / 64; ++w) t += red[w];
                p.sq_slots[tile_lin] = t;
            }
        }
    }
}

__host__ __device__ constexpr bool fe_in_form(int idx, int form) {
    if (form == 1) return idx == 1 || idx == 2 || idx == 3 || idx == 4 || idx == 5 || idx == 8 || idx == 9 || idx == 10 || idx == 17;
    if (form == 2) return idx == 1 || idx == 6 || idx == 7 || (idx >= 11 && idx <= 15);
    return true;
}
template <int NT, int BN, int PR, int NPASS, bool WG = false, int FORM = 0, typename StageFn>
__device__ __forceinline__ void fast_epilogue_dispatch(const GP& p, unsigned char* smem, int m0, int n0, int tid, StageFn stage,
                                                       const bf16x8* pre_r = nullptr, const bf16x8* pre_a = nullptr, int tile_lin = 0) {
    if constexpr (WG) {
        fast_epilogue<EF_F32, NT, BN, PR, NPASS>(p, smem, m0, n0, tid, stage, nullptr, nullptr, tile_lin);
        return;
    }
    switch (p.fast_epi) {
#define CB_FE_CASE(I) case I: if constexpr (fe_in_form(I, FORM)) fast_epilogue<FAST_EPI_COMBOS[I], NT, BN, PR, NPASS>(p, smem, m0, n0, tid, stage, pre_r, pre_a); break;
        CB_FE_CASE(1) CB_FE_CASE(2) CB_FE_CASE(3) CB_FE_CASE(4) CB_FE_CASE(5) CB_FE_CASE(6) CB_FE_CASE(7) CB_FE_CASE(8) CB_FE_CASE(9) CB_FE_CASE(10)
        CB_FE_CASE(11) CB_FE_CASE(12) CB_FE_CASE(13) CB_FE_CASE(14) CB_FE_CASE(15) CB_FE_CASE(17)
#undef CB_FE_CASE
        default: break;
    }
}
static_assert(FAST_EPI_N == 18 && FAST_EPI_COMBOS[FAST_EPI_F32] == EF_F32, "fast_epilogue_dispatch lists every combination");

template <int BM, int BN, bool WITH_R = true>
struct EpiPre {
    static constexpr int WM = BM / 2, CPR = BN / 8, ITER = WM * CPR / NTHREADS, NCH = 2 * ITER;
    static constexpr bool HAS_R = WITH_R;
    bf16x8 r[WITH_R ? NCH : 1], a[NCH];
};

template <typename T, int BM, int BN, bool WITH_R>
__device__ __forceinline__ void epi_prefetch(const GP& p, EpiPre<BM, BN, WITH_R>& pre, int m0, int n0, int tid) {
    using E = EpiPre<BM, BN, WITH_R>;
    const int cc = tid % E::CPR, n = n0 + cc * 8;
    const void* aux = p.mask ? p.mask : p.dact_pre;
    const int64_t lda = p.mask ? p.ldm : p.ldd;
#pragma unroll
    for (int h = 0; h < 2; ++h)
#pragma unroll
        for (int it = 0; it < E::ITER; ++it) {
            const int m = m0 + h * E::WM + (tid + it * NTHREADS) / E::CPR;
            bf16x8 z = {};
            if constexpr (WITH_R) pre.r[h * E::ITER + it] = z;
            pre.a[h * E::ITER + it] = z;
            if (m < p.M && n < p.N) {
                const int64_t orow = p.c_rowmap ? (int64_t)p.c_rowmap[m] : (int64_t)m;
                if constexpr (WITH_R) {
                    if (p.residual) pre.r[h * E::ITER + it] = *reinterpret_cast<const bf16x8*>(reinterpret_cast<const T*>(p.residual) + orow * p.ldr + n);
                }
                if (aux) pre.a[h * E::ITER + it] = *reinterpret_cast<const bf16x8*>(reinterpret_cast<const T*>(aux) + orow * lda + n);
            }
        }
}

template <typename T, int BM, int BN, int SMEM_BYTES, int EPF = 0, bool WG = false, int FORM = 0>
__device__ __forceinline__ void tile_epilogue(GP& p, f32x4 (&acc)[BM / 32][BN / 32], unsigned char* smem, int m0, int n0, int tid,
                                              const EpiPre<BM, BN, EPF != 1>& pre = EpiPre<BM, BN, EPF != 1>{}, bool use_pre = false, int tile_lin = 0) {
    constexpr int WM = BM / 2, WN = BN / 2, FM = WM / 16, FN = WN / 16;
    const int lane = tid & 63, wave = tid >> 6;
    const int wm = wave >> 1, wn = wave & 1;
    if (p.dropout_p > 0.f && p.seed_ptr) p.seed += *p.seed_ptr;
    const bool fast = p.c_vec && (n0 + BN <= p.N);
    if constexpr (sizeof(T) == 2) {
        if (p.c_vec8 && p.fast_epi != 0 && (WG == (p.fast_epi == FAST_EPI_F32)) && fe_in_form(p.fast_epi, FORM)) {
            static_assert((BM / 2) * (BN * 4 + 16) <= SMEM_BYTES, "staging does not fit");
            auto stage = [&](int h) __attribute__((always_inline)) {
                if (wm == h) {
#pragma unroll
                    for (int i = 0; i < FM; ++i)
#pragma unroll
                        for (int j = 0; j < FN; ++j)
                            *reinterpret_cast<f32x4*>(smem + (i * 16 + (lane & 15)) * (BN * 4 + 16) + (wn * WN + j * 16 + 4 * (lane >> 4)) * 4) = acc[i][j];
                }
            };
            const bf16x8* pre_r = nullptr;
            const bf16x8* pre_a = nullptr;
            if constexpr (EPF == 2) { if (use_pre) pre_r = pre.r; }
            if constexpr (EPF != 0) { if (use_pre) pre_a = pre.a; }
            fast_epilogue_dispatch<NTHREADS, BN, BM / 2, 2, WG, FORM>(p, smem, m0, n0, tid, stage, pre_r, pre_a, tile_lin);
            return;
        }
    }
    if (p.c_vec8) {
        constexpr int SROW = BN * 4 + 16;
        constexpr int CPR = BN / 8;
        constexpr int ITER = WM * CPR / NTHREADS;
        static_assert(WM * SROW <= SMEM_BYTES, "staging does not fit");
        static_assert(WM * CPR % NTHREADS == 0 && NTHREADS % CPR == 0, "chunk map");
        const int cc = tid % CPR, n = n0 + cc * 8;
        const bool nok = n < p.N;
        float sc[8], sh[8];
        if (p.scale && nok) load8(p.scale + n, sc);
        if (p.shift && nok) load8(p.shift + n, sh);
#pragma unroll 1
        for (int h = 0; h < 2; ++h) {
            __syncthreads();
            if (wm == h) {
#pragma unroll
                for (int i = 0; i < FM; ++i)
#pragma unroll
                    for (int j = 0; j < FN; ++j)
                        *reinterpret_cast<f32x4*>(smem + (i * 16 + (lane & 15)) * SROW + (wn * WN + j * 16 + 4 * (lane >> 4)) * 4) = acc[i][j];
            }
            __syncthreads();
#pragma unroll 1
            for (int it = 0; it < ITER; ++it) {
                const int rl = (tid + it * NTHREADS) / CPR;
                const int m = m0 + h * WM + rl;
                bf16x8 rp = {}, ap = {};
                if constexpr (EPF != 0) {
                    if (use_pre) {
#pragma unroll
                        for (int q = 0; q < 2 * ITER; ++q) {
                            if (q == h * ITER + it) {
                                if constexpr (EPF == 2) rp = pre.r[q];
                                ap = pre.a[q];
                            }
                        }
                    }
                }
                if (m < p.M && nok) {
                    const int64_t orow = p.c_rowmap ? (int64_t)p.c_rowmap[m] : (int64_t)m;
                    float v[8];
                    load8(reinterpret_cast<const float*>(smem + rl * SROW + cc * 32), v);
                    if constexpr (EPF == 2) {
                        if (use_pre) epilogue8<T, 2>(p, v, sc, sh, m, orow, n, rp, ap);
                        else epilogue8<T>(p, v, sc, sh, m, orow, n);
                    } else if constexpr (EPF == 1) {
                        if (use_pre) epilogue8<T, 1>(p, v, sc, sh, m, orow, n, bf16x8{}, ap);
                        else epilogue8<T>(p, v, sc, sh, m, orow, n);
                    } else epilogue8<T>(p, v, sc, sh, m, orow, n);
                }
            }
        }
    } else if (p.split_k > 1 && p.c_vec) {
        constexpr int SROW = BN * 4 + 16;
        static_assert(WM * SROW <= SMEM_BYTES, "staging does not fit");
        float* cbase = reinterpret_cast<float*>(p.C);
#pragma unroll
        for (int h = 0; h < 2; ++h) {
            __syncthreads();
            if (wm == h) {
#pragma unroll
                for (int i = 0; i < FM; ++i)
#pragma unroll
                    for (int j = 0; j < FN; ++j)
                        *reinterpret_cast<f32x4*>(smem + (i * 16 + (lane & 15)) * SROW + (wn * WN + j * 16 + 4 * (lane >> 4)) * 4) = acc[i][j];
            }
            __syncthreads();
#pragma unroll 4
            for (int idx = tid; idx < WM * BN; idx += NTHREADS) {
                const int rl = idx / BN, cl = idx % BN;
                const int m = m0 + h * WM + rl, n = n0 + cl;
                if (m < p.M && n < p.N) {
                    const int64_t orow = p.c_rowmap ? (int64_t)p.c_rowmap[m] : (int64_t)m;
                    float x = *reinterpret_cast<const float*>(smem + rl * SROW + cl * 4) * p.alpha;
                    if (p.scale) x *= p.scale[n];
#ifdef CB_EPI_NOATOMIC
                    cbase[orow * p.ldc + n] = x;
#else
                    atomicAdd(cbase + orow * p.ldc + n, x);
#endif
                }
            }
        }
    } else if (fast) {
#pragma unroll
        for (int i = 0; i < FM; ++i) {
            const int m = m0 + wm * WM + i * 16 + (lane & 15);
            const bool mok = m < p.M;
            const int64_t orow = (mok && p.c_rowmap) ? (int64_t)p.c_rowmap[m] : (int64_t)m;
#pragma unroll
            for (int j = 0; j < FN; ++j) {
                const int nb = n0 + wn * WN + j * 16 + 4 * (lane >> 4);
                if (mok) epilogue_vec<T>(p, acc[i][j], m, orow, nb);
            }
        }
    } else {
        float* stage = reinterpret_cast<float*>(smem);
        static_assert(WM * BN * 4 <= SMEM_BYTES, "staging does not fit");
#pragma unroll
        for (int h = 0; h < 2; ++h) {
            __syncthreads();
            if (wm == h) {
#pragma unroll
                for (int i = 0; i < FM; ++i)
#pragma unroll
                    for (int j = 0; j < FN; ++j)
                        *reinterpret_cast<f32x4*>(stage + (i * 16 + (lane & 15)) * BN + wn * WN + j * 16 + 4 * (lane >> 4)) = acc[i][j];
            }
            __syncthreads();
            for (int idx = tid; idx < WM * BN; idx += NTHREADS) {
                const int rl = idx / BN, cl = idx % BN;
                const int m = m0 + h * WM + rl, n = n0 + cl;
                if (m < p.M && n < p.N) {
                    const int64_t orow = p.c_rowmap ? (int64_t)p.c_rowmap[m] : (int64_t)m;
                    epilogue_elem<T>(p, stage[idx], m, orow, n);
                }
            }
        }
    }
}


template <typename T, int BM, int BN, typename LA, typename LB, int PF, bool RS, int OCC>
__device__ __forceinline__ void gemm_tile(GP& p, TileId bid, float* slab = nullptr, int* cnt = nullptr) {
    using X = Tr<T>;
    constexpr int BK = X::BK;
    constexpr int WM = BM / 2, WN = BN / 2, FM = WM / 16, FN = WN / 16;
    constexpr int TILE_A = BM * X::ROWB, TILE_B = BN * X::ROWB;
    constexpr int SMEM_BYTES = 2 * (TILE_A + TILE_B);
    __shared__ __attribute__((aligned(16))) unsigned char smem[SMEM_BYTES];

    const int tid = threadIdx.x, lane = tid & 63, wave = tid >> 6;
    const int wm = wave >> 1, wn = wave & 1;
    CB_STAMP_DECL();
    CB_STAMP(0);
#ifdef CB_STAMPS
    const unsigned stamp_lin = (unsigned)bid.bx + (unsigned)((p.N + BN - 1) / BN) * ((unsigned)bid.by + (unsigned)((p.M + BM - 1) / BM) * (unsigned)bid.bz);
#endif
    const int tile_lin = ((p.batch > 1 ? bid.bz / p.split_k : 0) * ((p.M + BM - 1) / BM) + bid.by) * ((p.N + BN - 1) / BN) + bid.bx;
    apply_batch(p, bid);
    const int m0 = bid.by * BM, n0 = bid.bx * BN;
    const int kt_per = (p.ktiles + p.split_k - 1) / p.split_k;
    const int kt0 = bid.bz * kt_per;
    const int nt = ((kt0 + kt_per < p.ktiles) ? kt0 + kt_per : p.ktiles) - kt0;
    if (nt <= 0) return;

    LA la;
    LB lb;
    {
        Opnd oa = {p.A, p.a_tab, p.lda, p.a_mode, p.a_bytes};
        Opnd ob = {p.B, p.b_tab, p.ldb, p.b_mode, p.b_bytes};
        la.init(p, oa, m0, p.M, kt0, tid);
        lb.init(p, ob, n0, p.N, kt0, tid);
    }
    typename LA::Stage sa[PF];
    typename LB::Stage sb[PF];

    auto load_tiles = [&](typename LA::Stage& xa, typename LB::Stage& xb) {
        la.template load<false>(xa, p);
        lb.template load<false>(xb, p);
    };
    auto load_tiles_checked = [&](typename LA::Stage& xa, typename LB::Stage& xb) {
        la.template load<true>(xa, p);
        lb.template load<true>(xb, p);
    };
    auto store_tiles = [&](const typename LA::Stage& xa, const typename LB::Stage& xb, int buf) {
        unsigned char* As = smem + buf * (TILE_A + TILE_B);
        la.store(xa, As, tid);
        lb.store(xb, As + TILE_A, tid);
    };

    f32x4 acc[FM][FN];
#pragma unroll
    for (int i = 0; i < FM; ++i)
#pragma unroll
        for (int j = 0; j < FN; ++j) { f32x4 z = {0.f, 0.f, 0.f, 0.f}; acc[i][j] = z; }
    f32x4 accr[RS ? FM : 1];
#pragma unroll
    for (int i = 0; i < (RS ? FM : 1); ++i) { f32x4 z = {0.f, 0.f, 0.f, 0.f}; accr[i] = z; }
    const bool rs_on = RS && p.a_rowsum != nullptr && bid.bx == 0 && wn == 0;

#pragma unroll
    for (int s = 0; s < PF; ++s)
        if (s < nt) load_tiles_checked(sa[s], sb[s]);
    constexpr bool DGRAD = sizeof(T) == 2 && !LA::KROW && LB::KROW;
    constexpr int EPF = !DGRAD ? 0 : (BM * BN <= 128 * 64 ? 2 : (OCC >= 2 ? 1 : 0));
    EpiPre<BM, BN, EPF != 1> epre;
    const bool epf_on = EPF != 0 && p.c_vec8 && (EPF == 2 ? p.relu_bwd != 0 : (p.dact_pre != nullptr && !p.relu_bwd));
    if constexpr (EPF != 0) {
        if (epf_on) epi_prefetch<T, BM, BN, EPF != 1>(p, epre, m0, n0, tid);
    }
    store_tiles(sa[0], sb[0], 0);
    if (PF < nt) load_tiles_checked(sa[0], sb[0]);
// ... 220 lines not shown
        if constexpr (GATHER) {
            int tap = k / p.Ct;
            c = k - tap * p.Ct;
            rr = tap / p.S; ss = tap - rr * p.S;
        }
#pragma unroll
        for (int i = 0; i < NI; ++i) {
            const int row = row0 + (i * 4 + wave) * 8 + rin;
            const bool ok = row < bound;
            ih[i] = 0; iw[i] = 0;
            if constexpr (GATHER) {
                cb_pixel px = {0, 0, 0};
                if (ok) px = o.tab[row];
                ih[i] = px.ih0; iw[i] = px.iw0;
                voff[i] = ok ? (uint32_t)px.off * 2u : OOB;
            } else {
                voff[i] = ok ? ((uint32_t)row * (uint32_t)o.ld + (uint32_t)k) * 2u : OOB;
            }
        }
    }
    template <bool CHECK> __device__ __forceinline__ void issue(const GP& p, unsigned char* tile, int wave) {
        if constexpr (GATHER) {
            const bool kv = rr < p.R;
            const uint32_t koff = (uint32_t)(rr * (int)p.sH + ss * (int)p.sW + c) * 2u;
#pragma unroll
            for (int i = 0; i < NI; ++i) {
                const bool v = kv && (unsigned)(ih[i] + rr) < (unsigned)p.H && (unsigned)(iw[i] + ss) < (unsigned)p.W;
                dma16(rs, tile + (i * 4 + wave) * 1024, v ? voff[i] + koff : OOB);
            }
            if (p.Ct >= X::BK) {
                c += X::BK;
                if (c >= p.Ct) { c -= p.Ct; if (++ss == p.S) { ss = 0; ++rr; } }
            } else {
                ss += X::BK / p.Ct;
                while (ss >= p.S) { ss -= p.S; ++rr; }
            }
        } else {
#pragma unroll
            for (int i = 0; i < NI; ++i) {
                uint32_t o32 = voff[i];
                if (CHECK && krem <= 0) o32 = OOB;
                dma16(rs, tile + (i * 4 + wave) * 1024, o32);
                voff[i] += X::BK * 2u;
            }
            krem -= X::BK;
        }
    }
};

inline bool aligned16(const void* p) { return (reinterpret_cast<uintptr_t>(p) & 15) == 0; }

template <typename T, int BM, int BN, int PF, int OCC, typename LA, typename LB, bool RS = false>
int launch_k(const GP& p, hipStream_t st) {
    dim3 grid((p.N + BN - 1) / BN, (p.M + BM - 1) / BM, p.split_k * (p.batch > 1 ? p.batch : 1));
    hipLaunchKernelGGL((gemm_kernel<T, BM, BN, LA, LB, PF, RS, OCC>), grid, dim3(NTHREADS), 0, st, p);
    return cb_launch_status("cb_gemm");
}
template <typename T, int BM, int BN, int PF, int OCC, typename LA, typename LB>
int launch_wgrad(const GP& p, hipStream_t st) {
    if (p.a_rowsum) return launch_k<T, BM, BN, PF, OCC, LA, LB, true>(p, st);
    return launch_k<T, BM, BN, PF, OCC, LA, LB, false>(p, st);
}

template <typename T, int BM, int BN, int PF, int OCC = 1>
int launch_gemm(const GP& p, bool fast, hipStream_t st) {
    const bool a_krow = p.a_mode == CB_KROW;
    const bool b_krow = p.b_mode != CB_ROWK;
    if (a_krow && !b_krow) return cb_fail("cb_gemm: unsupported operand mode combination (A KROW with B ROWK)");
    if (fast) {
        const int taps = p.R * p.S;
        if constexpr (sizeof(T) == 2) {
            if constexpr (BN < 128) {
                if (p.a_mode == CB_ROWK && (p.b_mode == CB_KROW || (p.b_mode == CB_KROW_TAPS && taps == 1)))
                    return launch_k<T, BM, BN, PF, OCC, RowkFast<T, BM, false>, KrowTr<BN, KM_PLAIN>>(p, st);
                if (p.a_mode == CB_ROWK_GATHER && p.b_mode == CB_KROW_TAPS && p.Ct % Tr<bf16>::BK == 0)
                    return launch_k<T, BM, BN, PF, OCC, RowkFast<T, BM, true>, KrowTr<BN, KM_TAPS>>(p, st);
            }
            if (p.a_mode == CB_KROW && p.b_mode == CB_KROW)
                return launch_wgrad<T, BM, BN, PF, OCC, KrowTr<BM, KM_PLAIN>, KrowTr<BN, KM_PLAIN>>(p, st);
            if (p.a_mode == CB_KROW && p.b_mode == CB_KROW_GATHER)
                return launch_k<T, BM, BN, PF, OCC, KrowTr<BM, KM_PLAIN>, KrowTr<BN, KM_GATHER>>(p, st);
        }
        if (p.a_mode == CB_ROWK && p.b_mode == CB_ROWK)
            return launch_k<T, BM, BN, PF, OCC, RowkFast<T, BM, false>, RowkFast<T, BN, false>>(p, st);
        if (p.a_mode == CB_ROWK_GATHER && p.b_mode == CB_ROWK)
            return launch_k<T, BM, BN, PF, OCC, RowkFast<T, BM, true>, RowkFast<T, BN, false>>(p, st);
        constexpr int KB1B = BN >= 128 ? 4 : 2;
        constexpr int KB2A = BM >= 128 ? 8 : 4, KB2B = BN >= 128 ? 8 : 4;
        if (p.a_mode == CB_ROWK && (p.b_mode == CB_KROW || (p.b_mode == CB_KROW_TAPS && taps == 1)))
            return launch_k<T, BM, BN, PF, OCC, RowkFast<T, BM, false>, KrowFast<T, BN, KM_PLAIN, KB1B, 0>>(p, st);
        if (p.a_mode == CB_ROWK_GATHER && p.b_mode == CB_KROW_TAPS)
            return launch_k<T, BM, BN, PF, OCC, RowkFast<T, BM, true>, KrowFast<T, BN, KM_TAPS, KB1B, 0>>(p, st);
        if (p.a_mode == CB_KROW && p.b_mode == CB_KROW)
            return launch_wgrad<T, BM, BN, PF, OCC, KrowFast<T, BM, KM_PLAIN, KB2A, 0>, KrowFast<T, BN, KM_PLAIN, KB2B, 128>>(p, st);
        if (p.a_mode == CB_KROW && p.b_mode == CB_KROW_GATHER)
            return launch_k<T, BM, BN, PF, OCC, KrowFast<T, BM, KM_PLAIN, KB2A, 0>, KrowFast<T, BN, KM_GATHER, KB2B, 128>>(p, st);
    }
    if (!a_krow && !b_krow) return launch_k<T, BM, BN, PF, OCC, RowkLoader<T, BM, false>, RowkLoader<T, BN, false>>(p, st);
    if (!a_krow) return launch_k<T, BM, BN, PF, OCC, RowkLoader<T, BM, false>, KrowLoader<T, BN, false>>(p, st);
    if (p.b_mode == CB_KROW) return launch_wgrad<T, BM, BN, PF, OCC, KrowLoader<T, BM, false>, KrowLoader<T, BN, false>>(p, st);
    return launch_k<T, BM, BN, PF, OCC, KrowLoader<T, BM, false>, KrowLoader<T, BN, false>>(p, st);
}

enum { GC_WGRAD = 0,
       GC_WGRAD_GATHER = 1,
       GC_FWD = 2,
       GC_FWD_GATHER = 3,
// ... 36 lines not shown
```

clipbert_amd/csrc/gemm_skinny.hip:

```cpp
#include "gemm_impl.h"

namespace cbgemm {
namespace {
constexpr int SK_BM = 32, SK_BN = 64, SK_NB = 6;
constexpr int SK_STEP_BYTES = 32 * SK_BN * 2;

__device__ __forceinline__ bf16x8 sk_load_rowk(const bf16* base, int64_t ld, int row, bool row_ok, int k, int K, bool vec) {
    bf16x8 z;
#pragma unroll
    for (int e = 0; e < 8; ++e) z[e] = (bf16)0.f;
    if (!row_ok || k >= K) return z;
    const bf16* q = base + (int64_t)row * ld + k;
    if (vec) return *reinterpret_cast<const bf16x8*>(q);
#pragma unroll
    for (int e = 0; e < 8; ++e)
        if (k + e < K) z[e] = q[e];
    return z;
}

template <bool BKROW>
__global__ void __launch_bounds__(256) gemm_skinny_kernel(GP p, int a_vec, int b_vec) {
    constexpr int STAGE = BKROW ? 4 * SK_NB * SK_STEP_BYTES : 0, RED = 4 * SK_BM * SK_BN * 4;
    __shared__ __attribute__((aligned(16))) unsigned char smem[STAGE > RED ? STAGE : RED];
    const int tid = threadIdx.x, lane = tid & 63, wave = tid >> 6;
// ... 52 lines not shown
                    *reinterpret_cast<bf16x8*>(stage + q * SK_STEP_BYTES + kline * (SK_BN * 2) + ((chunk ^ tr_chunk_swz<SK_BN>(kline)) << 4)) = bq[q][c];
                }
            __syncthreads();
        }
#pragma unroll
        for (int q = 0; q < SK_NB; ++q) {
            bf16x8 bfr[4];
#pragma unroll
            for (int j = 0; j < 4; ++j) {
                if constexpr (BKROW) bfr[j] = tr_frag<SK_BN>(stage + q * SK_STEP_BYTES, j * 16, 0, lane);
                else bfr[j] = bq[q][j];
            }
#pragma unroll
            for (int i = 0; i < 2; ++i)
#pragma unroll
                for (int j = 0; j < 4; ++j) acc[i][j] = __builtin_amdgcn_mfma_f32_16x16x32_bf16(bfr[j], af[q][i], acc[i][j], 0, 0, 0);
        }
        if constexpr (BKROW) __syncthreads();
    }

    __syncthreads();
    float* red = reinterpret_cast<float*>(smem);
#pragma unroll
    for (int i = 0; i < 2; ++i)
#pragma unroll
        for (int j = 0; j < 4; ++j)
            *reinterpret_cast<f32x4*>(red + (wave * SK_BM + i * 16 + r16) * SK_BN + j * 16 + 4 * (lane >> 4)) = acc[i][j];
    __syncthreads();
    const int row = tid >> 3, c8 = (tid & 7) * 8;
    f32x4 v0 = {0.f, 0.f, 0.f, 0.f}, v1 = v0;
#pragma unroll
    for (int w = 0; w < 4; ++w) {
        v0 = v0 + *reinterpret_cast<const f32x4*>(red + (w * SK_BM + row) * SK_BN + c8);
        v1 = v1 + *reinterpret_cast<const f32x4*>(red + (w * SK_BM + row) * SK_BN + c8 + 4);
    }
    const int m = m0 + row, n = n0 + c8;
    if (m >= p.M || n >= p.N) return;
    const int64_t orow = p.c_rowmap ? (int64_t)p.c_rowmap[m] : (int64_t)m;
    if (p.c_vec && n + 8 <= p.N) {
        epilogue_vec<bf16>(p, v0, m, orow, n);
        epilogue_vec<bf16>(p, v1, m, orow, n + 4);
    } else {
#pragma unroll
        for (int e = 0; e < 4; ++e) {
            if (n + e < p.N) epilogue_elem<bf16>(p, v0[e], m, orow, n + e);
            if (n + 4 + e < p.N) epilogue_elem<bf16>(p, v1[e], m, orow, n + 4 + e);
        }
    }
}
}

bool skinny_covers(const cb_gemm_desc* d, const GP& p) {
    if (d->dtype != CB_BF16 || d->a_mode != CB_ROWK || (d->b_mode != CB_ROWK && d->b_mode != CB_KROW)) return false;
    if (p.batch > 1 || p.split_k > 1 || d->zero_fill_pitch || d->a_rowsum || d->sq_slots || d->accumulate == 2) return false;
    if (d->b_mode == CB_KROW && !(d->N % 8 == 0 && d->ldb % 8 == 0 && aligned16(d->B))) return false;
    return true;
}

int launch_gemm_skinny(const cb_gemm_desc* d, GP& p, hipStream_t st) {
    const int a_vec = d->lda % 8 == 0 && d->K % 8 == 0 && aligned16(d->A);
    const int b_vec = d->ldb % 8 == 0 && d->K % 8 == 0 && aligned16(d->B);
    p.fast_epi = 0;
    const dim3 grid((unsigned)((d->N + SK_BN - 1) / SK_BN), (unsigned)((d->M + SK_BM - 1) / SK_BM));
    if (d->b_mode == CB_KROW) hipLaunchKernelGGL((gemm_skinny_kernel<true>), grid, dim3(256), 0, st, p, a_vec, b_vec);
    else hipLaunchKernelGGL((gemm_skinny_kernel<false>), grid, dim3(256), 0, st, p, a_vec, b_vec);
    return cb_launch_status("cb_gemm");
}
}
```

clipbert_amd/gemm_log.py:

```python
from typing import Callable, Dict, List

import torch

from . import ops

MFMA_PEAK_TFLOPS = 2500.0
HBM_PEAK_GBS = 8000.0

FAMILY_BOUND = {
    "encoder linear (fwd + dgrad)": "mfma",
    "resnet 1x1 conv, K <= 256 (fwd + dgrad)": "hbm",
    "resnet 1x1 conv, K > 256 (fwd + dgrad)": "mfma",
    "conv 3x3 / 7x7 (fwd + dgrad)": "mfma",
    "weight gradients (linear + conv)": "mfma",
    "fused frozen front: stem + res2 blocks (fwd)": "hbm",
}
FUSED = "fused frozen front: stem + res2 blocks (fwd)"


def _problem(d) -> dict:
    batch = max(1, int(d.batch))
    taps = max(1, int(d.R) * int(d.S))
    esz = 4 if d.dtype == ops.CB_F32 else 2
    c_esz = 4 if d.c_f32 else esz
    wgrad = d.a_mode == ops.KROW
    gather = d.a_mode == ops.ROWK_GATHER or d.b_mode in (ops.KROW_GATHER, ops.KROW_TAPS)
    cnn = bool(d.scale) or bool(d.relu_bwd) or bool(d.a_tab) or bool(d.b_tab) or bool(d.c_rowmap) or d.zero_fill_pitch != 0 or bool(d.post_scale)
    M, N, K = int(d.M), int(d.N), int(d.K)
    K_alg = 147 if (d.a_mode == ops.ROWK_GATHER and int(d.R) == 7 and int(d.Cin) == 32 and K == 224) else K
    cnn = cnn or (wgrad and K % 49 == 0 and K >= 49) or (not wgrad and M % 49 == 0 and M >= 49 * 16)
    if wgrad:
        fam = "weight gradients (linear + conv)"
        alg = batch * ((K * M + K * N / taps) * esz + (2 if d.accumulate else 1) * M * N * c_esz)
    else:
        if gather and taps > 1:
            fam = "conv 3x3 / 7x7 (fwd + dgrad)"
        elif cnn:
            fam = "resnet 1x1 conv, K <= 256 (fwd + dgrad)" if K <= 256 else "resnet 1x1 conv, K > 256 (fwd + dgrad)"
        else:
            fam = "encoder linear (fwd + dgrad)"
        extra = sum(1 for p in (d.residual, d.mask, d.C2, d.gelu_grad_pre) if p) + (1 if d.accumulate else 0) + (2 if d.relu_bwd else 0)
        alg = batch * ((M * K / taps + N * K) * esz + M * N * c_esz + extra * M * N * esz)
    return {"family": fam, "flop": 2.0 * M * N * K_alg * batch, "bytes": float(alg), "M": M, "N": N, "K": K, "batch": batch, "taps": taps,
            "form": "wgrad" if wgrad else ("dgrad" if d.b_mode in (ops.KROW, ops.KROW_TAPS) else "fwd")}


class GemmLog:

    def __init__(self):
        self.launches: List[dict] = []

    def __enter__(self):
        self._gemm, self._group = ops.gemm, ops.gemm_group
        self._stem, self._res2 = ops.stem_pool, ops.res2_block

        def stem_pool(packed, weight, scale, shift, oh, ow):
            n, hp, wp, _ = packed.shape
            m = n * oh * ow
            pooled = n * ((oh - 1) // 2 + 1) * ((ow - 1) // 2 + 1)
            prob = {"family": FUSED, "flop": 2.0 * m * 64 * 147, "bytes": float(packed.numel() * 2 + pooled * 64 * 2), "M": m, "N": 64, "K": 147, "batch": 1,
                    "taps": 49, "form": "fwd"}
            self.launches.append({"problems": [prob], "replay": (lambda: self._stem(packed, weight, scale, shift, oh, ow))})
            return self._stem(packed, weight, scale, shift, oh, ow)

        self._stem8 = ops.stem_pool_u8

        def stem_pool_u8(frames, mean, std, weight, scale, shift):
            n, _c, h, w = frames.shape
            oh, ow = (h + 6 - 7) // 2 + 1, (w + 6 - 7) // 2 + 1
            m = n * oh * ow
            pooled = n * ((oh - 1) // 2 + 1) * ((ow - 1) // 2 + 1)
            prob = {"family": FUSED, "flop": 2.0 * m * 64 * 147, "bytes": float(frames.numel() + pooled * 64 * 2), "M": m, "N": 64, "K": 147, "batch": 1,
                    "taps": 49, "form": "fwd"}
            self.launches.append({"problems": [prob], "replay": (lambda: self._stem8(frames, mean, std, weight, scale, shift))})
            return self._stem8(frames, mean, std, weight, scale, shift)

        def res2_block(x, w1, w2, w3, ss1, ss2, ss3, wsc=None, sssc=None):
            n, h, w, cin = x.shape
            m = n * h * w
            kk = cin * 64 + 9 * 64 * 64 + 64 * 256 + (cin * 256 if wsc is not None else 0)
            prob = {"family": FUSED, "flop": 2.0 * m * kk, "bytes": float(m * (cin + 256) * 2), "M": m, "N": 256, "K": kk // 256, "batch": 1, "taps": 9, "form": "fwd"}
            self.launches.append({"problems": [prob], "replay": (lambda: self._res2(x, w1, w2, w3, ss1, ss2, ss3, wsc=wsc, sssc=sssc))})
            return self._res2(x, w1, w2, w3, ss1, ss2, ss3, wsc=wsc, sssc=sssc)

        def gemm(a, b, M, N, K, **kw):
            d = ops.gemm_desc(a, b, M, N, K, **kw)
            self.launches.append({"problems": [_problem(d)], "replay": (lambda a=a, b=b, M=M, N=N, K=K, kw=kw: self._gemm(a, b, M, N, K, **kw))})
            return self._gemm(a, b, M, N, K, **kw)

        def gemm_group(descs, like):
            descs = list(descs)
            if descs:
                self.launches.append({"problems": [_problem(d) for d in descs], "replay": (lambda descs=descs, like=like: self._group(descs, like))})
            return self._group(descs, like)

        ops.gemm, ops.gemm_group = gemm, gemm_group
        ops.stem_pool, ops.res2_block = stem_pool, res2_block
# ... 54 lines not shown
```

clipbert_amd/modeling/cnn.py:

```python
from typing import Optional

import torch
from torch import nn

from .. import ops
from ..data import RawFrames
from ..ops import ACT_NONE, ACT_RELU, KROW, KROW_GATHER, KROW_TAPS, ROWK_GATHER
from .modules import RESNET50_STAGES, BottleneckBlock, Conv2d, _Detectron2Model, _GridConv, as_config
from .runtime import Runtime, _pick_split


def _out_hw(h, w, k, stride, pad):
    return (h + 2 * pad - k) // stride + 1, (w + 2 * pad - k) // stride + 1


def conv_gather(rt: Runtime, operand, n, h, w, c, k, stride, pad, device, out_hw=None, taps=None, sN=None, sH=None):
    oh, ow = out_hw or _out_hw(h, w, k, stride, pad)
    sN, sH = h * w * c if sN is None else sN, w * c if sH is None else sH
    R, S, cin = taps or (k, k, c)
    tab = rt.table(n, oh, ow, stride, pad, sN, sH, c, device)
    kw = dict(R=R, S=S, Cin=cin, H=h, W=w, sH=sH, sW=c)
    kw.update(dict(a_mode=ROWK_GATHER, a_tab=tab, lda=0) if operand == "a" else dict(b_mode=KROW_GATHER, b_tab=tab, ldb=0))
    return kw


def _conv_fwd(rt: Runtime, x, conv, act=ACT_NONE, residual=None, relu_after=False):
    n, h, w, cin = x.shape
    k, s, p = conv.k, conv.stride, conv.pad
    oh, ow = _out_hw(h, w, k, s, p)
    cout = conv.cout
    m = n * oh * ow
    y = torch.empty(n, oh, ow, cout, dtype=x.dtype, device=x.device)
    wk = rt.bank.compute(conv.weight).view(cout, k * k * cin)
    scale, shift = conv.scale_shift()
    res2d = residual.view(m, cout) if residual is not None else None
    plain = k == 1 and s == 1
    gather = {} if plain else conv_gather(rt, "a", n, h, w, cin, k, s, p, x.device)
    ops.gemm(x.view(m, cin) if plain else x, wk, m, cout, k * k * cin, out=y.view(m, cout), ldb=k * k * cin, **gather, scale=scale, shift=shift,
             act=act, residual=res2d, relu_after=relu_after)
    return y


def _conv_dgrad(rt: Runtime, g, conv, in_shape, scale=None, mask=None, residual=None, out=None, accumulate=False, fuse=None):
    n, h, w, cin = in_shape
    _, oh, ow, cout = g.shape
    k, s, p = conv.k, conv.stride, conv.pad
    wk = rt.bank.compute(conv.weight).view(cout, k * k * cin)
    mi = n * h * w
    zfill = w if (k == 1 and s == 2 and h % 2 == 0 and w % 2 == 0 and cin % 8 == 0) else 0
    alloc = torch.zeros if (s > 1 and not zfill) else torch.empty
    if out is None:
        out = alloc(n, h, w, cin, dtype=g.dtype, device=g.device)
    o2 = out.view(mi, cin)
    r2 = residual.view(mi, cin) if residual is not None else None
    k2 = mask.view(mi, cin) if mask is not None else None
    extra = {}
    second = None
    if fuse is not None:
        assert mask is None and scale is None
        y, s_a, s_b = fuse
        second = alloc(n, h, w, cin, dtype=g.dtype, device=g.device)
        k2 = y.view(mi, cin)
        extra = dict(relu_bwd=True, post_scale=s_a, post_scale2=s_b, out2=second.view(mi, cin))
    if k == 1:
        rowmap = rt.strided_rowmap(n, h, w, oh, ow, s, g.device) if s > 1 else None
        ops.gemm(g.view(n * oh * ow, cout), wk, n * oh * ow, cin, cout, out=o2, b_mode=KROW_TAPS, ldb=cin, R=1, S=1,
                 Cin=cout, c_rowmap=rowmap, scale=scale, mask=k2, residual=r2, accumulate=accumulate, zero_fill_pitch=zfill if s > 1 else 0,
                 **extra)
    else:
        assert s == 1
        ops.gemm(g, wk, mi, cin, k * k * cout, out=o2, b_mode=KROW_TAPS, ldb=k * k * cin, flip_taps=True,
                 **conv_gather(rt, "a", n, oh, ow, cout, k, 1, k - 1 - p, g.device), scale=scale, mask=k2, residual=r2,
                 accumulate=accumulate, **extra)
    return (out, second) if fuse is not None else out


def _conv_wgrad(rt: Runtime, g, x, conv, pending=None):
    gw = rt.bank.grad_image(conv.weight)
    if gw is None:
        return
    n, h, w, cin = x.shape
    _, oh, ow, cout = g.shape
    k, s, p = conv.k, conv.stride, conv.pad
    m = n * oh * ow
    kk = k * k * cin
    split, tile = _pick_split(cout, kk, m)
    bank = rt.bank
    acc, slots = True, None
    if bank.take_fresh_param(conv.weight):
        if rt.dtype == torch.bfloat16 and kk % 8 == 0:
            acc = 2
            slots = bank.fold_take(ops.sq_slot_count(cout, kk), "cnn")
        else:
            ops.zero_(gw)
    else:
        bank.fold_invalidate()
    run = ops.gemm if pending is None else (lambda *a, **kw: pending.append(ops.gemm_desc(*a, **kw)))
    plain = k == 1 and s == 1
    xkw = dict(b_mode=KROW, ldb=cin) if plain else conv_gather(rt, "b", n, h, w, cin, k, s, p, x.device)
    run(g.view(m, cout), x.view(m, cin) if plain else x, cout, kk, m, out=gw.view(cout, kk), a_mode=KROW, lda=cout, **xkw, accumulate=acc,
        split_k=split, tile=tile, sq_slots=slots)


def _stem_weight(rt: Runtime, conv: Conv2d):
    if rt.stem_w is None:
        w = conv.weight.detach().float()
        wp = torch.zeros(64, 7, 8, 4, dtype=torch.float32, device=w.device)
        wp[:, :, :7, :3] = w.permute(0, 2, 3, 1)
        rt.stem_w = wp.view(64, 224).to(rt.dtype).contiguous()
    return rt.stem_w


def _block_trainable(rt: Runtime, blk: BottleneckBlock) -> bool:
    return any(rt.bank.is_trainable(c.weight) for c in (blk.conv1, blk.conv2, blk.conv3) + ((blk.shortcut,) if blk.shortcut is not None else ()))


def _res2_block_fused(rt: Runtime, x, blk: BottleneckBlock):
    w = lambda conv: rt.bank.compute(conv.weight)
    sc = blk.shortcut
    return ops.res2_block(x, w(blk.conv1), w(blk.conv2), w(blk.conv3), blk.conv1.scale_shift(), blk.conv2.scale_shift(), blk.conv3.scale_shift(),
                          wsc=w(sc) if sc is not None else None, sssc=sc.scale_shift() if sc is not None else None)


def _res2_fusable(rt: Runtime, x, blk: BottleneckBlock, save: bool) -> bool:
    if rt.dtype != torch.bfloat16:
        return False
    if save and _block_trainable(rt, blk):
        return False
    c1, c2, c3 = blk.conv1, blk.conv2, blk.conv3
    return (c1.cout == 64 and c2.cin == 64 and c2.cout == 64 and c3.cout == 256 and c1.stride == 1 and c1.k == 1 and c2.k == 3 and c2.stride == 1
            and c3.k == 1 and c1.cin in (64, 256) and (blk.shortcut is not None) == (c1.cin == 64) and x.shape[-1] == c1.cin and x.is_contiguous())


def _stem_forward(bb: "GridFeatBackbone", x5):
    rt = bb.rt
    b, t, c, h, w = x5.shape
    n = b * t
    stem = bb.feature.backbone.stem.conv1
    oh, ow = _out_hw(h, w, 7, 2, 3)
    fused = rt.dtype == torch.bfloat16 and w % 2 == 0
    if isinstance(x5, RawFrames):
        table, host_table = x5.packed_table()
        if x5.pixfmt == "rgb":
            packed = ops.resize_pack_u8(x5.flat, table, n, h, rt.dtype, bb.pixel_mean, bb.pixel_std, hwc=x5.hwc, pad=3, extra_w=2,
                                        host_table=host_table)
        else:
            packed = ops.resize_pack_yuv420(x5.flat, table, n, h, rt.dtype, bb.pixel_mean, bb.pixel_std, layout=x5.pixfmt, matrix=x5.matrix,
                                            pad=3, extra_w=2, host_table=host_table)
    else:
        x4 = x5.reshape(n, c, h, w)
        if not x4.is_contiguous():
            x4 = x4.contiguous()
        u8 = x4.dtype == torch.uint8
        if u8 and fused:
            return ops.stem_pool_u8(x4, bb.pixel_mean, bb.pixel_std, _stem_weight(rt, stem), *stem.scale_shift())
        packed = ops.stem_pack(x4, rt.dtype, 3, bb.pixel_mean, bb.pixel_std, extra_w=2) if u8 else ops.stem_pack(x4.float(), rt.dtype, 3, extra_w=2)
    scale, shift = stem.scale_shift()
    if fused:
        return ops.stem_pool(packed, _stem_weight(rt, stem), scale, shift, oh, ow)
    hp, wp = packed.shape[1], packed.shape[2]
    y = torch.empty(n, oh, ow, 64, dtype=rt.dtype, device=x5.device)
    ops.gemm(packed, _stem_weight(rt, stem), n * oh * ow, 64, 224, out=y.view(-1, 64), ldb=224,
             **conv_gather(rt, "a", n, hp, wp, 4, 7, 2, 0, x5.device, out_hw=(oh, ow), taps=(7, 1, 32)), scale=scale, shift=shift, act=ACT_RELU)
    return ops.maxpool_fwd(y, 3, 2, 1)


def cnn_forward(bb: "GridFeatBackbone", x5, save: bool):
    rt = bb.rt
    b, t = x5.shape[:2]
    net = bb.feature.backbone
    x = _stem_forward(bb, x5)
    saved = []
    for name, _nb, _mid, _cout, _s in RESNET50_STAGES:
        for blk in getattr(net, name):
            if _res2_fusable(rt, x, blk, save):
                x = _res2_block_fused(rt, x, blk)
                continue
            sc = _conv_fwd(rt, x, blk.shortcut) if blk.shortcut is not None else x
            y1 = _conv_fwd(rt, x, blk.conv1, act=ACT_RELU)
            y2 = _conv_fwd(rt, y1, blk.conv2, act=ACT_RELU)
            out = _conv_fwd(rt, y2, blk.conv3, residual=sc, relu_after=True)
            if save and _block_trainable(rt, blk):
                saved.append((blk, x, y1, y2, out))
            x = out
    gconv = bb.grid_encoder[0]
    gy = _conv_fwd(rt, x, gconv)
    grid = ops.maxpool_fwd(gy, 2, 2, 0, relu=True)
    return grid.view(b, t, *grid.shape[1:]), (saved, x, gy, grid) if save else None


def cnn_backward(bb: "GridFeatBackbone", saved_pack, dgrid: torch.Tensor):
    for _ in cnn_backward_steps(bb, saved_pack, dgrid):
        bb.rt.fire_if_last("cnn")


def cnn_backward_steps(bb: "GridFeatBackbone", saved_pack, dgrid: torch.Tensor):
    rt = bb.rt
    saved, res5, gy, grid = saved_pack
    gconv = bb.grid_encoder[0]
    dg = ops.maxpool2_bwd(gy, grid, dgrid.reshape(grid.shape).contiguous(), relu=True)
    _conv_wgrad(rt, dg, res5, gconv)
    if not saved:
        return
    res5_ids = {id(b) for b in bb.feature.backbone.res5}
    first_res5 = min((i for i, rec in enumerate(saved) if id(rec[0]) in res5_ids), default=None)
    stage_of = {id(b): name for name, *_ in RESNET50_STAGES for b in getattr(bb.feature.backbone, name)}
    pend = []

    def flush():
        ops.gemm_group(pend, dg)
        pend.clear()

    def fuse_spec(i):
        b, _x, _y1, _y2, o = saved[i]
        s3_, _ = b.conv3.scale_shift()
        ssc_ = b.shortcut.scale_shift()[0] if b.shortcut is not None else None
        return (o, s3_, ssc_)

    g3, sec = _conv_dgrad(rt, dg, gconv, res5.shape, fuse=fuse_spec(len(saved) - 1))
    for idx in range(len(saved) - 1, -1, -1):
        blk, x, y1, y2, out = saved[idx]
        need_dx = idx > 0
        s2, _ = blk.conv2.scale_shift()
        s1, _ = blk.conv1.scale_shift()
        dz, gsc = (sec, None) if blk.shortcut is None else (None, sec)
        _conv_wgrad(rt, g3, y2, blk.conv3, pend)
        if blk.shortcut is not None:
            _conv_wgrad(rt, gsc, x, blk.shortcut, pend)
        g2 = _conv_dgrad(rt, g3, blk.conv3, y2.shape, scale=s2, mask=y2)
        _conv_wgrad(rt, g2, y1, blk.conv2, pend)
        g1 = _conv_dgrad(rt, g2, blk.conv2, y1.shape, scale=s1, mask=y1)
        _conv_wgrad(rt, g1, x, blk.conv1, pend)
        if idx == 0 or stage_of.get(id(saved[idx - 1][0])) != stage_of.get(id(blk)):
            flush()
        if idx == first_res5 and idx > 0:
            yield "grid_encoder+res5"
        if need_dx:
            spec = fuse_spec(idx - 1)
            if blk.shortcut is None:
                g3, sec = _conv_dgrad(rt, g1, blk.conv1, x.shape, residual=dz, fuse=spec)
            else:
                dout = _conv_dgrad(rt, g1, blk.conv1, x.shape)
                g3, sec = _conv_dgrad(rt, gsc, blk.shortcut, x.shape, out=dout, accumulate=True, fuse=spec)


class _CnnFn(torch.autograd.Function):
    @staticmethod
    def forward(ctx, anchor, x5, bb):
        save = ctx.needs_input_grad[0] and bb.has_trainable()
        grid, pack = cnn_forward(bb, x5, save)
        ctx.bb, ctx.pack = bb, pack
        if pack is not None:
            bb.rt.pending_cnn_nodes += 1
        return grid

    @staticmethod
    def backward(ctx, dgrid):
        if ctx.pack is not None:
            cnn_backward(ctx.bb, ctx.pack, dgrid.contiguous())
            ctx.pack = None
            ctx.bb.rt.node_done("cnn")
        return None, None, None


class GridFeatBackbone(nn.Module):
    def __init__(self, detectron2_model_cfg=None, config=None, input_format="BGR", freeze_at=2):
        super().__init__()
        assert input_format == "BGR", "detectron 2 image input format should be BGR"
        config = as_config(config)
        self.detectron2_model_cfg = detectron2_model_cfg
        self.feature = _Detectron2Model()
        self.grid_encoder = nn.ModuleList([_GridConv(config.backbone_channel_in_size, config.hidden_size)])
        self.input_format = input_format
        self.config = config
        self.pixel_mean = (123.675, 116.28, 103.53)
        self.pixel_std = (1.0, 1.0, 1.0)
        self.rt: Optional[Runtime] = None
        net = self.feature.backbone
        frozen = [net.stem] + ([net.res2] if freeze_at >= 2 else [])
        for mod in frozen:
            for p in mod.parameters():
                p.requires_grad = False

    @property
    def config_file(self):
        return f"clipbert_amd R-50 grid backbone (detectron2 cfg: {self.detectron2_model_cfg})"

    def has_trainable(self):
        return any(p.requires_grad for p in self.parameters())

    def forward(self, x):
        return _CnnFn.apply(self.rt.anchor, x, self)


def cnn_early_split(model) -> Optional[int]:
    bank = model.rt.bank
# ... 11 lines not shown
```

clipbert_amd/modeling/runtime.py:

```python
from typing import Optional

import torch

from .. import ops
from ..params import ParamBank

_HOOK = {"encoder": "after_encoder_backward", "cnn": "after_res5_backward"}


class Runtime:
    def __init__(self):
        self.bank: Optional[ParamBank] = None
        self.dtype = torch.bfloat16
        self.tables = {}
        self.rowmaps = {}
        self.seed_dev: Optional[torch.Tensor] = None
        self.anchor: Optional[torch.Tensor] = None
        self.stem_w = None
        self.after_encoder_backward = None
        self.pending_encoder_nodes = 0
        self.after_res5_backward = None
        self.pending_cnn_nodes = 0
        self.prepare_args = None
        self._ln_off = None
        self.forward_count = 0

    def begin_step(self):
        self.pending_encoder_nodes = self.pending_cnn_nodes = 0

    def fire_if_last(self, kind, left=1):
        hook = getattr(self, _HOOK[kind])
        if hook is not None and getattr(self, f"pending_{kind}_nodes") <= left:
            hook()

    def node_done(self, kind, fire=False):
        setattr(self, f"pending_{kind}_nodes", max(0, getattr(self, f"pending_{kind}_nodes") - 1))
        if fire:
            self.fire_if_last(kind, left=0)

    def table(self, n, oh, ow, stride, pad, sN, sH, sW, device):
        key = (n, oh, ow, stride, pad, sN, sH, sW, str(device))
        t = self.tables.get(key)
        if t is None:
            t = ops.build_pixel_table(n, oh, ow, stride, pad, sN, sH, sW, device)
            self.tables[key] = t
        return t

    def strided_rowmap(self, n, h, w, oh, ow, stride, device):
        key = (n, h, w, oh, ow, stride, str(device))
        t = self.rowmaps.get(key)
        if t is None:
            t = (torch.arange(n).view(n, 1, 1) * (h * w) + (torch.arange(oh) * stride).view(1, oh, 1) * w
                 + (torch.arange(ow) * stride).view(1, 1, ow)).reshape(-1).to(torch.int32).to(device)
            self.rowmaps[key] = t
        return t


def _pick_split(mo, no, kred):
    ktiles = (kred + 63) // 64
    b64 = ((mo + 63) // 64) * ((no + 63) // 64)
    if b64 >= 200 or ktiles < 64:
        return 1, 0
    split = max(1, min(ktiles // 8, (400 + b64 // 2) // b64))
    return split, 0


_SITE_EMB, _SITE_ATTN, _SITE_SELF_OUT, _SITE_OUT, _SITE_POOL, _SITE_REG = 1, 2, 3, 4, 5, 6


def _seed(site, layer=0, fwd=0):
    return ((site * 1000003 + layer * 7919) * 2654435761 + fwd * 0x9E3779B97F4A7C15) % (1 << 62)
```

clipbert_amd/ops.py:

```python
import ctypes as C
import os
from typing import Optional

import torch

from . import _lib
from ._lib import (ACT_GELU, ACT_GELU_SAVE_GRAD, ACT_NONE, ACT_RELU, ACT_SAVED_GRAD, ACT_TANH, CB_BF16, CB_F32, KROW, KROW_GATHER,
                   KROW_TAPS, ROWK, ROWK_GATHER, GemmDesc)

_ALLOW_HOST_POINTERS = False


def dtype_code(t: torch.dtype) -> int:
    if t == torch.bfloat16:
        return CB_BF16
    if t == torch.float32:
        return CB_F32
    raise TypeError(f"unsupported dtype {t}")


def _ptr(t: Optional[torch.Tensor]):
    if t is None:
        return None
    if not t.is_cuda and not _ALLOW_HOST_POINTERS:
        raise RuntimeError("clipbert_amd ops need CUDA(HIP) tensors: there is no CPU path")
    return t.data_ptr()


def _extent_bytes(t: torch.Tensor) -> int:
    return t.untyped_storage().nbytes() - t.storage_offset() * t.element_size()


def _stream(t: torch.Tensor):
    if t.is_cuda:
        return torch.cuda.current_stream(t.device).cuda_stream
    return None


def _chk(rc, what):
    _lib.check(rc, what)


def gemm_desc(a: torch.Tensor, b: torch.Tensor, M: int, N: int, K: int, *, out: torch.Tensor, a_mode=ROWK,
              b_mode=ROWK, lda=None, ldb=None, ldc=None, a_tab=None, b_tab=None, R=1, S=1, Cin=0, H=0, W=0,
              sH=0, sW=0, flip_taps=False, c_rowmap=None, accumulate=False, split_k=1, act=ACT_NONE,
              scale=None, shift=None, residual=None, ldr=None, relu_after=False, mask=None, ldm=None,
              out2=None, ldc2=None, alpha=1.0, dropout_p=0.0, dropout_seed=0, seed_ptr=None, tile=0, gelu_grad_pre=None, a_rowsum=None, batch=1, batch_strides=None,
              relu_bwd=False, post_scale=None, post_scale2=None, xcd_order=0, zero_fill_pitch=0, splitk_ws=None, schedule=0, sq_slots=None) -> GemmDesc:
    d = GemmDesc()
    d.dtype = dtype_code(a.dtype)
    assert b.dtype == a.dtype
    d.M, d.N, d.K = M, N, K
    d.a_mode, d.b_mode = a_mode, b_mode
    d.A, d.B = _ptr(a), _ptr(b)
    d.lda = lda if lda is not None else a.stride(0)
    d.ldb = ldb if ldb is not None else b.stride(0)
    d.a_tab, d.b_tab = _ptr(a_tab), _ptr(b_tab)
    d.R, d.S, d.Cin, d.H, d.W, d.sH, d.sW = R, S, Cin, H, W, sH, sW
    d.flip_taps = int(flip_taps)
    d.C = _ptr(out)
    d.ldc = ldc if ldc is not None else out.stride(0)
    d.c_rowmap = _ptr(c_rowmap)
    d.zero_fill_pitch = zero_fill_pitch
    d.c_f32 = int(out.dtype == torch.float32)
    d.accumulate = int(accumulate)
    d.split_k = split_k
    d.act = act
    d.scale, d.shift = _ptr(scale), _ptr(shift)
    d.residual = _ptr(residual)
    d.ldr = (ldr if ldr is not None else residual.stride(0)) if residual is not None else 0
    d.relu_after = int(relu_after)
    d.mask = _ptr(mask)
    d.ldm = (ldm if ldm is not None else mask.stride(0)) if mask is not None else 0
    d.C2 = _ptr(out2)
    d.ldc2 = (ldc2 if ldc2 is not None else out2.stride(0)) if out2 is not None else 0
    d.alpha = alpha
    d.dropout_p = dropout_p
    d.dropout_seed = dropout_seed
    d.dropout_seed_ptr = _ptr(seed_ptr)
    if _KEY_LOG is not None:
        _KEY_LOG.append((a_mode, b_mode, M, N, K, batch, R * S, split_k))
    if tile == 0 and _LAUNCH_OVERRIDE:
        ov = _LAUNCH_OVERRIDE.get((a_mode, b_mode, M, N, K, batch, R * S, split_k))
        if ov is not None:
            tile, xcd_order, schedule = ov[0], ov[1], ov[3]
            d.split_k = ov[2] if ov[2] > 0 else split_k
    d.tile = tile
    d.schedule = schedule
    d.xcd_order = xcd_order
    d.a_bytes = _extent_bytes(a)
    d.b_bytes = _extent_bytes(b)
    if gelu_grad_pre is not None:
        d.gelu_grad_pre, d.ld_gelu = _ptr(gelu_grad_pre), gelu_grad_pre.stride(0)
    if a_rowsum is not None:
        assert a_rowsum.dtype == torch.float32
        d.a_rowsum = _ptr(a_rowsum)
    if relu_bwd:
        d.relu_bwd = 1
        d.post_scale, d.post_scale2 = _ptr(post_scale), _ptr(post_scale2)
    if batch > 1:
        d.batch = batch
        d.batch_stride_a, d.batch_stride_b, d.batch_stride_c, d.batch_stride_rowsum = batch_strides
    if splitk_ws is None and d.dtype == CB_BF16 and not _SPLITK_OFF:
        splitk_ws = splitk_workspace(a.device)
    if splitk_ws is not None:
        d.splitk_ws, d.splitk_ws_bytes = _ptr(splitk_ws), splitk_ws.numel() * splitk_ws.element_size()
    if sq_slots is not None:
        assert sq_slots.dtype == torch.float32 and sq_slots.is_contiguous()
        d.sq_slots, d.sq_slots_n = _ptr(sq_slots), sq_slots.numel()
    d._refs = (a, b, out, a_tab, b_tab, c_rowmap, scale, shift, residual, mask, out2, seed_ptr, gelu_grad_pre, a_rowsum, post_scale,
               post_scale2, splitk_ws, sq_slots)
    return d


def gemm(a: torch.Tensor, b: torch.Tensor, M: int, N: int, K: int, *, out: torch.Tensor, **kw):
    d = gemm_desc(a, b, M, N, K, out=out, **kw)
    _chk(_lib.get().cb_gemm(C.byref(d), _stream(a)), "cb_gemm")
    return out


def gemm_plan(a: torch.Tensor, b: torch.Tensor, M: int, N: int, K: int, *, out: torch.Tensor, use_table: bool = True, **kw):
    d = gemm_desc(a, b, M, N, K, out=out, **kw)
    plan = (C.c_int32 * 4)()
    _chk(_lib.get().cb_gemm_plan(C.byref(d), 1 if use_table else 0, plan), "cb_gemm_plan")
    return tuple(plan)


def gemm_group(descs, like: torch.Tensor):
    n = len(descs)
    if n == 0:
        return
    arr = (GemmDesc * n)()
    for i, d in enumerate(descs):
        C.memmove(C.byref(arr[i]), C.byref(d), C.sizeof(GemmDesc))
    _chk(_lib.get().cb_gemm_group(C.cast(arr, C.c_void_p), n, _stream(like)), "cb_gemm_group")


_KEY_LOG = None
_LAUNCH_OVERRIDE = {}
_TILE_ID = {"128x128": 1, "64x64": 2, "128x64": 3, "128x128o2": 4, "8w256x256": 5, "8w128x256": 6, "8w256x128": 7}


def parse_launch_config(name: str):
    parts = name.split("/")
    tile = _TILE_ID[parts[0]]
    xcd = 1 if parts[1] == "xcd" else 2
    split = ([int(x[1:]) for x in parts[2:] if x[0] == "s"] or [0])[0]
    sched = ([int(x[1:]) + 1 for x in parts[2:] if x[0] == "m"] or [0])[0]
    return (tile, xcd, split or (1 if tile >= 5 else 0), sched)


for _item in filter(None, os.environ.get("CB_LAUNCH_OVERRIDE", "").split(";")):
    _k, _, _c = _item.partition("=")
    _LAUNCH_OVERRIDE[tuple(int(x) for x in _k.split(","))] = parse_launch_config(_c)
_SPLITK_WS = {}
_SPLITK_OFF = False
SPLITK_WS_BYTES = 128 << 20


def splitk_workspace(device) -> torch.Tensor:
    dev = torch.device(device)
    key = str(dev)
    ws = _SPLITK_WS.get(key)
    if ws is None:
# ... 526 lines not shown
```

include/clipbert_hip.h:

```cpp
#ifndef CLIPBERT_HIP_H
#define CLIPBERT_HIP_H

#include <stddef.h>
#include <stdint.h>

#ifdef __cplusplus
extern "C" {
#endif

enum { CB_F32 = 0, CB_BF16 = 1 };
enum { CB_SPLITK_WS_COUNTER_BYTES = 65536 };
enum { CB_ACT_NONE = 0, CB_ACT_RELU = 1, CB_ACT_GELU = 2, CB_ACT_TANH = 3,
       CB_ACT_GELU_SAVE_GRAD = 4,
       CB_ACT_SAVED_GRAD = 5 };

enum {
    CB_ROWK = 0,
    CB_ROWK_GATHER = 1,
    CB_KROW = 2,
    CB_KROW_TAPS = 3,
    CB_KROW_GATHER = 4
};

typedef struct { int32_t off; int16_t ih0; int16_t iw0; } cb_pixel;

typedef struct {
    int32_t dtype;
    int32_t M, N, K;
    int32_t a_mode, b_mode;
    const void* A; const void* B;
    int64_t lda, ldb;
    const cb_pixel* a_tab;
    const cb_pixel* b_tab;
    int32_t R, S, Cin;
    int32_t H, W;
    int64_t sH, sW;
    int32_t flip_taps;
    int32_t schedule;
    void* C; int64_t ldc;
    const int32_t* c_rowmap;
    int32_t c_f32;
    int32_t accumulate;
    int32_t split_k;
    int32_t act;
    const float* scale;
    const float* shift;
    const void* residual; int64_t ldr;
    int32_t relu_after;
    int32_t zero_fill_pitch;
    const void* mask; int64_t ldm;
    void* C2; int64_t ldc2;
    float alpha;
    float dropout_p;
    uint64_t dropout_seed;
    const uint64_t* dropout_seed_ptr;
    int32_t tile;
    int32_t xcd_order;
    int64_t a_bytes, b_bytes;
    const void* gelu_grad_pre; int64_t ld_gelu;
    float* a_rowsum;
    int32_t batch;
    int32_t relu_bwd;
    int64_t batch_stride_a, batch_stride_b, batch_stride_c, batch_stride_rowsum;
    const float* post_scale; const float* post_scale2;
    void* splitk_ws;
    int64_t splitk_ws_bytes;
    float* sq_slots;
    int64_t sq_slots_n;
} cb_gemm_desc;

int cb_gemm(const cb_gemm_desc* d, void* stream);
int cb_gemm_plan(const cb_gemm_desc* d, int32_t use_table, int32_t* out4);
int cb_gemm_workspace_bytes(const cb_gemm_desc* d, int64_t* bytes);
int cb_gemm_group(const cb_gemm_desc* descs, int32_t n, void* stream);

int cb_build_pixel_table(cb_pixel* tab, int32_t N, int32_t OH, int32_t OW, int32_t stride, int32_t pad,
                         int64_t sN, int64_t sH, int64_t sW, void* stream);

int cb_stem_pack(int32_t dtype, const void* src, int32_t src_u8, const float* mean3, const float* std3,
                 void* dst, int32_t N, int32_t H, int32_t W, int32_t Hp, int32_t Wp, int32_t pad,
                 void* stream);

int cb_resize_pack_u8(int32_t dtype, const uint8_t* flat, int64_t flat_bytes, const int64_t* table, const int64_t* table_host, int32_t N,
                      int32_t hwc, const float* mean3, const float* std3, void* dst, int32_t S, int32_t Hp, int32_t Wp, int32_t pad,
                      void* stream);

enum { CB_YUV_I420 = 0, CB_YUV_NV12 = 1 };
enum { CB_YUV_BT601 = 0, CB_YUV_BT601_FULL = 1, CB_YUV_BT709 = 2, CB_YUV_BT709_FULL = 3 };
int cb_resize_pack_yuv420(int32_t dtype, const uint8_t* flat, int64_t flat_bytes, const int64_t* table, const int64_t* table_host, int32_t N,
                          int32_t layout, int32_t matrix, const float* mean3, const float* std3, void* dst, int32_t S, int32_t Hp, int32_t Wp,
                          int32_t pad, void* stream);

int cb_image_norm(const uint8_t* src, float* dst, const float* mean3, const float* std3,
                  int64_t n_images, int64_t hw, void* stream);

int cb_maxpool_fwd(int32_t dtype, const void* x, void* y, int32_t N, int32_t H, int32_t W, int32_t C,
                   int32_t OH, int32_t OW, int32_t k, int32_t stride, int32_t pad, int32_t relu,
                   void* stream);
int cb_maxpool2_bwd(int32_t dtype, const void* x, const void* y, const void* dy, void* dx, int32_t N,
                    int32_t H, int32_t W, int32_t C, int32_t OH, int32_t OW, int32_t relu, void* stream);

int cb_stem_pool(const void* packed, const void* weight, const float* scale, const float* shift, void* out, int32_t N, int32_t Hp,
                 int32_t Wp, int32_t OH, int32_t OW, int32_t PH, int32_t PW, void* stream);
int cb_stem_pool_u8(const uint8_t* frames, const float* mean3, const float* std3, const void* weight, const float* scale, const float* shift,
                    void* out, int32_t N, int32_t H, int32_t W, int32_t OH, int32_t OW, int32_t PH, int32_t PW, void* stream);

typedef struct cb_res2_desc {
    const void* x; void* out;
    const void* w1; const void* w2; const void* w3; const void* wsc;
    const float* scale1; const float* shift1; const float* scale2; const float* shift2; const float* scale3; const float* shift3;
    const float* scale_sc; const float* shift_sc;
    int32_t N, H, W, cin;
} cb_res2_desc;
int cb_res2_block(const cb_res2_desc* desc, void* stream);

int cb_relu_scale_bwd(int32_t dtype, const void* dy, const void* y, const float* scale, void* g,
                      void* dz, const float* scale2, void* g2, int64_t rows, int32_t C, void* stream);

int cb_layernorm_fwd(int32_t dtype, const void* x, const float* gamma, const float* beta, void* y,
                     float* mean, float* rstd, int64_t rows, int32_t D, float eps, int32_t seg_len,
                     int32_t seg_stride, int32_t seg_off, void* stream);
// ... 116 lines not shown
```

Before: 4126 clips/s.

## Move ResNet stride-2 downsampling to block tails and add parity-class stride-2 dgrad

Restructures the ResNet blocks so a downsampling block's stride is applied at the tail of the previous block. The residual is gathered through a new res_rowmap epilogue input, and the next block's 1x1 convs work on a compact even-pixel input. Adds a dgrad_s2 GEMM mode that splits a stride-2 3x3 transposed-conv gradient into four parity classes with reduced tap sets, avoiding multiplications by structural zeros. The aim is less wasted conv FLOPs and memory traffic in forward and backward, at the cost of new epilogue variants, rowmap gathers, and paths that bypass the tuned table and grouping.

```diff
diff --git a/clipbert_amd/_lib.py b/clipbert_amd/_lib.py
--- a/clipbert_amd/_lib.py
+++ b/clipbert_amd/_lib.py
@@ -30,7 +30,7 @@
         ("xcd_order", i32), ("a_bytes", i64), ("b_bytes", i64), ("gelu_grad_pre", vp), ("ld_gelu", i64), ("a_rowsum", vp),
         ("batch", i32), ("relu_bwd", i32), ("batch_stride_a", i64), ("batch_stride_b", i64), ("batch_stride_c", i64),
         ("batch_stride_rowsum", i64), ("post_scale", vp), ("post_scale2", vp), ("splitk_ws", vp), ("splitk_ws_bytes", i64),
-        ("sq_slots", vp), ("sq_slots_n", i64),
+        ("sq_slots", vp), ("sq_slots_n", i64), ("res_rowmap", vp), ("res_rows", i32), ("dgrad_s2", i32),
     ]
 
 
diff --git a/clipbert_amd/csrc/common.hip b/clipbert_amd/csrc/common.hip
--- a/clipbert_amd/csrc/common.hip
+++ b/clipbert_amd/csrc/common.hip
@@ -22,4 +22,4 @@
 }
 
 extern "C" const char* cb_last_error(void) { return g_err; }
-extern "C" int cb_version(void) { return 13; }
+extern "C" int cb_version(void) { return 14; }
diff --git a/clipbert_amd/csrc/gemm.hip b/clipbert_amd/csrc/gemm.hip
--- a/clipbert_amd/csrc/gemm.hip
+++ b/clipbert_amd/csrc/gemm.hip
@@ -154,6 +154,18 @@
     p.M = d->M; p.N = d->N; p.K = d->K;
     p.a_mode = d->a_mode; p.b_mode = d->b_mode;
     p.R = d->R > 0 ? d->R : 1; p.S = d->S > 0 ? d->S : 1; p.Ct = d->Cin; p.H = d->H; p.W = d->W; p.flip = d->flip_taps;
+    p.res_rowmap = d->res_rowmap;
+    if (d->res_rowmap) {
+        CB_REQUIRE(d->residual && d->res_rows > 0 && p.batch == 1 && (int64_t)d->res_rows * d->ldr * esz < 0x7fffffffll,
+                   "cb_gemm: res_rowmap needs a residual of res_rows > 0 rows that ends below 2 GiB, and one problem per launch");
+    }
+    if (d->dgrad_s2) {
+        CB_REQUIRE(d->a_mode == CB_ROWK_GATHER && d->b_mode == CB_KROW_TAPS && d->R == 3 && d->S == 3 && d->M % 4 == 0 && d->c_rowmap &&
+                   d->ldb == (int64_t)9 * d->N && p.batch == 1 && d->split_k <= 1 && !d->zero_fill_pitch,
+                   "cb_gemm: dgrad_s2 needs A CB_ROWK_GATHER, B CB_KROW_TAPS with R = S = 3 and ldb = 9 N, M a multiple of 4, c_rowmap, no batch / K split / zero fill");
+        p.cls_rows = d->M / 4;
+        p.flip = 0;
+    }
     CB_REQUIRE(d->accumulate >= 0 && d->accumulate <= 2 && (d->accumulate != 2 || d->dtype == CB_BF16), "cb_gemm: bad accumulate %d (2 = first writer: bf16 problems)", d->accumulate);
     p.c_f32 = d->c_f32; p.accumulate = d->accumulate == 1; p.split_k = d->split_k > 0 ? d->split_k : 1;
     p.act = d->act; p.relu_after = d->relu_after;
@@ -162,7 +174,8 @@
     const int bk = d->dtype == CB_BF16 ? Tr<bf16>::BK : Tr<float>::BK;
     p.ktiles = (d->K + bk - 1) / bk;
     {
-        const bool ok = d->dtype == CB_BF16 && !d->c_f32 && (int64_t)d->M * (d->ldc > d->ldc2 ? d->ldc : d->ldc2) * 2 * (p.batch) < 0xffffffffll && !d->c_rowmap;
+        const bool ok = d->dtype == CB_BF16 && !d->c_f32 && (int64_t)d->M * (d->ldc > d->ldc2 ? d->ldc : d->ldc2) * 2 * (p.batch) < 0xffffffffll &&
+                        (!d->c_rowmap || d->dgrad_s2);
         p.wt = ok ? switches().wt : 0;
     }
     {
@@ -182,11 +195,11 @@
         }
         const bool plain = !wg_store && !fe_off && p.wt == 1 && p.batch == 1 && d->accumulate != 1 && p.alpha == 1.f && !d->zero_fill_pitch && !d->a_rowsum &&
                            d->N % 8 == 0 && d->ldc % 8 == 0 && aligned16(d->C) && (!d->shift || aligned16(d->shift)) && (!d->scale || aligned16(d->scale)) &&
-                           rows_ok(d->residual, d->ldr) && rows_ok(d->mask, d->ldm) && rows_ok(d->gelu_grad_pre, d->ld_gelu) &&
+                           (d->res_rowmap ? (d->ldr % 8 == 0 && aligned16(d->residual)) : rows_ok(d->residual, d->ldr)) && rows_ok(d->mask, d->ldm) && rows_ok(d->gelu_grad_pre, d->ld_gelu) &&
                            !(d->mask && d->gelu_grad_pre);
         if (plain && d->relu_bwd) {
             const bool ok = d->C2 && d->post_scale && d->ldc2 % 8 == 0 && aligned16(d->C2) && (int64_t)d->M * d->ldc2 * 2 < 0xffffffffll;
-            const int flags = EF_RBWD | (d->residual ? EF_RES : 0) | (d->post_scale2 ? EF_PS2 : 0);
+            const int flags = EF_RBWD | (d->residual ? EF_RES : 0) | (d->post_scale2 ? EF_PS2 : 0) | (d->res_rowmap ? EF_RMAP : 0) | (d->dgrad_s2 ? EF_CMAP : 0);
             if (ok)
                 for (int i = 1; i < FAST_EPI_N; ++i)
                     if (FAST_EPI_COMBOS[i] == flags) { p.fast_epi = i; break; }
@@ -205,8 +218,10 @@
             if (d->gelu_grad_pre && !(flags & EF_MULAUX)) ok = false;
             if (d->dropout_p > 0.f) flags |= EF_DROP;
             if (d->residual) flags |= EF_RES;
+            if (d->res_rowmap) flags |= EF_RMAP;
             if (d->relu_after) flags |= EF_RELU_AFTER;
             if (d->mask) flags |= EF_MASK;
+            if (d->dgrad_s2) flags |= EF_CMAP;
             if (ok)
                 for (int i = 1; i < FAST_EPI_N; ++i)
                     if (FAST_EPI_COMBOS[i] == flags) { p.fast_epi = i; break; }
@@ -363,7 +378,7 @@
 
 namespace {
 int group_class(const cb_gemm_desc* d, const Prepared& pr) {
-    if (!pr.fast || d->zero_fill_pitch || d->tile >= 5 || d->tile == 1 || d->tile == 3) return -1;
+    if (!pr.fast || d->zero_fill_pitch || d->tile >= 5 || d->tile == 1 || d->tile == 3 || d->res_rowmap || d->dgrad_s2) return -1;
     if (d->batch > 1 || d->a_rowsum) {
         const bool ok = d->dtype == CB_BF16 && pr.form == FORM_WGRAD && d->split_k <= 1 && d->tile != 2 && !d->c_rowmap;
         return ok ? GC_WGRAD_RS : -1;
diff --git a/clipbert_amd/csrc/gemm_choose.h b/clipbert_amd/csrc/gemm_choose.h
--- a/clipbert_amd/csrc/gemm_choose.h
+++ b/clipbert_amd/csrc/gemm_choose.h
@@ -87,7 +87,7 @@
     const int form = model_form(pr.form), split_caller = p.split_k;
     const bool taps = pr.taps > 1;
     const int c_esz = d->c_f32 ? 4 : 2;
-    const int64_t M = d->M, N = d->N, K = d->K, batch = p.batch;
+    const int64_t M = d->M, N = d->N, K = d->dgrad_s2 ? d->K / 4 : d->K, batch = p.batch;
     ModelPick best;
     auto consider = [&](int ti, int s, int sched) {
         const double us = model_us(ti, form, M, N, K, batch, s, taps, sched == 3, c_esz);
@@ -119,7 +119,7 @@
     const GP& p = pr.p;
     if (!pr.fast || !pr.cv8 || d->dtype != CB_BF16 || pr.form != FORM_FWD || p.batch > 1 || p.split_k > 1) return -1;
     if (d->c_f32 || d->accumulate || d->c_rowmap || d->zero_fill_pitch || d->a_rowsum || d->gelu_grad_pre || d->dropout_p > 0.f || d->mask || d->relu_bwd ||
-        d->C2) return -1;
+        d->C2 || d->res_rowmap) return -1;
     if (d->K % 8 != 0 || d->M < 64) return -1;
     if ((int64_t)d->M * (d->N > d->K ? d->N : d->K) * 2 >= 0x7fffffffll) return -1;
     if (p.ktiles == 1 && d->N % 256 == 0) return 0;
@@ -153,13 +153,15 @@
     const int sv = stream_variant(d, pr);
     CB_REQUIRE(d->tile != 8 || sv >= 0, "cb_gemm: tile 8 (streaming) does not cover this problem (M=%d N=%d K=%d modes %d/%d)", d->M, d->N, d->K, d->a_mode, d->b_mode);
     const cbgemm::TunedEntry* tabled =
-        (bf && use_table && !sw.no_tuned) ? cbgemm::tuned_lookup(d->a_mode, d->b_mode, d->M, d->N, d->K, p.batch, pr.taps, split_caller) : nullptr;
+        (bf && use_table && !sw.no_tuned && !d->dgrad_s2) ? cbgemm::tuned_lookup(d->a_mode, d->b_mode, d->M, d->N, d->K, p.batch, pr.taps, split_caller) : nullptr;
+    if (!tabled && bf && use_table && !sw.no_tuned && pr.form == FORM_FWD)
+        tabled = cbgemm::tuned_lookup(CB_ROWK_GATHER, d->b_mode, d->M, d->N, d->K, p.batch, 1, split_caller);
     if (d->tile == 8 || (!explicit_tile && use_table && !sw.no_stream && !tabled && sv >= 0 && d->M >= STREAM_MIN_ROWS && d->N <= 512)) {
         lp.tile = 8; lp.sched = sv; lp.c_vec8 = true;
         return 0;
     }
 
-    const int form8 = (bf && pr.fast && pr.cv8 && (pr.form != FORM_DGRAD_TAPS || p.Ct % 64 == 0)) ? FORM8_OF[pr.form] : 0;
+    const int form8 = (bf && pr.fast && pr.cv8 && (pr.form != FORM_DGRAD_TAPS || p.Ct % 64 == 0) && !d->res_rowmap && !d->dgrad_s2) ? FORM8_OF[pr.form] : 0;
     const int64_t ws_room = assume_ws ? splitk_payload_bytes(WS_UNLIMITED)
                                       : (d->splitk_ws && aligned16(d->splitk_ws) ? splitk_payload_bytes(d->splitk_ws_bytes) : 0);
     const bool free_split = !explicit_tile && a_reduction_major(pr.form) && pr.atomics_ok;
diff --git a/clipbert_amd/csrc/gemm_impl.h b/clipbert_amd/csrc/gemm_impl.h
--- a/clipbert_amd/csrc/gemm_impl.h
+++ b/clipbert_amd/csrc/gemm_impl.h
@@ -19,14 +19,19 @@
 struct GP {
     const void* A; const void* B; void* C; void* C2; const void* residual; const void* mask;
     const void* dact_pre; float* a_rowsum; int64_t ldd;
-    int relu_bwd; const float* post_scale; const float* post_scale2;
-    int batch; int64_t bs_a, bs_b, bs_c, bs_r;
+    int relu_bwd;
+    int cls_rows;
+    const float* post_scale; const float* post_scale2;
+    int batch;
+    int fast_epi;
+    int64_t bs_a, bs_b, bs_c, bs_r;
     const float* scale; const float* shift;
     const cb_pixel* a_tab; const cb_pixel* b_tab; const int32_t* c_rowmap;
     int64_t lda, ldb, ldc, ldc2, ldr, ldm, sH, sW;
     int M, N, K;
     int a_mode, b_mode;
-    int R, S, Ct, H, W, flip;
+    int R, S, Ct, H, W;
+    int flip;
     int c_f32, accumulate, split_k, act, relu_after;
     float alpha, dropout_p;
     uint64_t seed;
@@ -38,7 +43,7 @@
     uint32_t a_bytes, b_bytes;
     int ktiles;
     int slab_base, cnt_base;
-    int fast_epi;
+    const int32_t* res_rowmap;
     float* sq_slots;
 #ifdef CB_STAMPS
     unsigned long long* stamps;
@@ -49,7 +54,9 @@
        EF_RBWD = 512,
        EF_PS2 = 1024,
        EF_F32 = 2048,
-       EF_GELU1 = 4096 };
+       EF_GELU1 = 4096,
+       EF_RMAP = 8192,
+       EF_CMAP = 16384 };
 constexpr int FAST_EPI_COMBOS[] = {
     -1,
     0,
@@ -69,6 +76,9 @@
     EF_RBWD | EF_PS2 | EF_RES,
     EF_F32,
     EF_SHIFT | EF_GELU1,
+    EF_SCALE | EF_SHIFT | EF_RES | EF_RELU_AFTER | EF_RMAP,
+    EF_RBWD | EF_RES | EF_RMAP,
+    EF_SCALE | EF_MASK | EF_CMAP,
 };
 constexpr int FAST_EPI_F32 = 16;
 constexpr int FAST_EPI_N = sizeof(FAST_EPI_COMBOS) / sizeof(int);
@@ -121,6 +131,15 @@
 }
 __device__ __forceinline__ u32x4 bload16(rsrc_t r, uint32_t off) { return __builtin_amdgcn_raw_buffer_load_b128(r, off, 0, 0); }
 
+constexpr int TAP_S2 = 16;
+__device__ __forceinline__ int tap_weight(const GP& p, int tap) {
+    if (p.flip >= TAP_S2) {
+        const int jr = p.S == 2 ? tap >> 1 : tap, js = p.S == 2 ? tap & 1 : 0;
+        return p.flip - TAP_S2 - 6 * jr - 2 * js;
+    }
+    return p.flip ? (p.R * p.S - 1 - tap) : tap;
+}
+
 struct Opnd {
     const void* base; const cb_pixel* tab; int64_t ld; int mode; uint32_t bytes;
 };
@@ -252,7 +271,7 @@
             const int nvalid = bound - row[it];
             int64_t ro = rowoff[it];
             if (mode == CB_KROW_TAPS) {
-                int tapw = p.flip ? (p.R * p.S - 1 - tap[it]) : tap[it];
+                int tapw = tap_weight(p, tap[it]);
                 ro = (int64_t)tapw * bound + row[it];
             }
 #pragma unroll
@@ -450,7 +469,7 @@
                 voff[it] += X::BK * ldb;
                 kb0[it] += X::BK;
             } else if constexpr (KMODE == KM_TAPS) {
-                const int tapw = p.flip ? (p.R * p.S - 1 - tap[it]) : tap[it];
+                const int tapw = tap_weight(p, tap[it]);
                 const bool v = act[it] && tap[it] < p.R * p.S;
                 const uint32_t base = (uint32_t)co[it] * ldb + (uint32_t)tapw * bound * ESZ + voff[it];
 #pragma unroll
@@ -602,7 +621,7 @@
                 voff[i] += X::BK * ldb;
                 kl[i] += X::BK;
             } else if constexpr (KMODE == KM_TAPS) {
-                const int tapw = p.flip ? (p.R * p.S - 1 - tap[i]) : tap[i];
+                const int tapw = tap_weight(p, tap[i]);
                 const bool v = act[i] && tap[i] < p.R * p.S;
                 st.r[i] = bload16(rs, v ? (uint32_t)co[i] * ldb + (uint32_t)tapw * bound * ESZ + voff[i] : OOB);
                 co[i] += X::BK;
@@ -658,6 +677,21 @@
     if (p.a_rowsum) p.a_rowsum += b * p.bs_r;
 }
 
+template <int BM, int BK>
+__device__ __forceinline__ void dgrad_s2_class(GP& p, TileId& bid) {
+    if (p.cls_rows <= 0) return;
+    const int cls = 3 - (bid.by & 3);
+    bid.by >>= 2;
+    const int py = cls >> 1, px = cls & 1;
+    p.M = p.cls_rows;
+    p.R = 1 + py; p.S = 1 + px;
+    p.K = p.R * p.S * p.Ct;
+    p.ktiles = (p.K + BK - 1) / BK;
+    p.flip = TAP_S2 + 3 * (1 + py) + (1 + px);
+    p.c_rowmap += (int64_t)cls * p.cls_rows;
+}
+inline int dgrad_s2_grid_y(const GP& p, int BM) { return p.cls_rows > 0 ? 4 * ((p.cls_rows + BM - 1) / BM) : (p.M + BM - 1) / BM; }
+
 template <typename T>
 __device__ __forceinline__ float act_of(int act, float v) {
     if constexpr (sizeof(T) == 2) {
@@ -676,13 +710,15 @@
     }
 }
 
-template <typename T>
-__device__ __forceinline__ void epilogue_vec(const GP& p, f32x4 v, int m, int64_t orow, int nb) {
+template <typename T, bool RMAP = false>
+__device__ __forceinline__ void epilogue_vec(const GP& p, f32x4 v, int m, int64_t orow, int nb, int64_t rrow = 0) {
+    if constexpr (!RMAP) rrow = orow;
+    const bool has_res = p.residual != nullptr && (!RMAP || rrow >= 0);
     v = v * p.alpha;
     if (p.relu_bwd) {
         T* c = reinterpret_cast<T*>(p.C) + orow * p.ldc + nb;
         if (p.accumulate) v = v + load4(c);
-        if (p.residual) v = v + load4(reinterpret_cast<const T*>(p.residual) + orow * p.ldr + nb);
+        if (has_res) v = v + load4(reinterpret_cast<const T*>(p.residual) + rrow * p.ldr + nb);
         const f32x4 mk = load4(reinterpret_cast<const T*>(p.mask) + orow * p.ldm + nb);
 #pragma unroll
         for (int r = 0; r < 4; ++r) v[r] = mk[r] > 0.f ? v[r] : 0.f;
@@ -717,7 +753,7 @@
     if (p.dropout_p > 0.f) {
         v = v * dropout_mult4(p.seed, (uint64_t)m * ((p.N + 3) >> 2) + (nb >> 2), p.dropout_p);
     }
-    if (p.residual) v = v + load4(reinterpret_cast<const T*>(p.residual) + orow * p.ldr + nb);
+    if (has_res) v = v + load4(reinterpret_cast<const T*>(p.residual) + rrow * p.ldr + nb);
     if (p.relu_after) {
 #pragma unroll
         for (int r = 0; r < 4; ++r) v[r] = v[r] > 0.f ? v[r] : 0.f;
@@ -748,13 +784,15 @@
     }
 }
 
-template <typename T>
-__device__ __forceinline__ void epilogue_elem(const GP& p, float x, int m, int64_t orow, int n) {
+template <typename T, bool RMAP = false>
+__device__ __forceinline__ void epilogue_elem(const GP& p, float x, int m, int64_t orow, int n, int64_t rrow = 0) {
+    if constexpr (!RMAP) rrow = orow;
+    const bool has_res = p.residual != nullptr && (!RMAP || rrow >= 0);
     x *= p.alpha;
     if (p.relu_bwd) {
         T* c = reinterpret_cast<T*>(p.C) + orow * p.ldc + n;
         if (p.accumulate) x += to_f32(*c);
-        if (p.residual) x += to_f32(reinterpret_cast<const T*>(p.residual)[orow * p.ldr + n]);
+        if (has_res) x += to_f32(reinterpret_cast<const T*>(p.residual)[rrow * p.ldr + n]);
         x = to_f32(reinterpret_cast<const T*>(p.mask)[orow * p.ldm + n]) > 0.f ? x : 0.f;
         if (p.C2) reinterpret_cast<T*>(p.C2)[orow * p.ldc2 + n] = from_f32<T>(p.post_scale2 ? x * p.post_scale2[n] : x);
         *c = from_f32<T>(p.post_scale ? x * p.post_scale[n] : x);
@@ -773,7 +811,7 @@
         x = act_of<T>(p.act, x);
     }
     if (p.dropout_p > 0.f) x *= dropout_mult1(p.seed, (uint64_t)m * ((p.N + 3) >> 2) + (n >> 2), n & 3, p.dropout_p);
-    if (p.residual) x += to_f32(reinterpret_cast<const T*>(p.residual)[orow * p.ldr + n]);
+    if (has_res) x += to_f32(reinterpret_cast<const T*>(p.residual)[rrow * p.ldr + n]);
     if (p.relu_after) x = x > 0.f ? x : 0.f;
     if (p.mask) x = to_f32(reinterpret_cast<const T*>(p.mask)[orow * p.ldm + n]) > 0.f ? x : 0.f;
     if (p.dact_pre) {
@@ -833,14 +871,16 @@
 #else
 #define CB_EPI_ST(...) do { __VA_ARGS__; } while (0)
 #endif
-template <typename T, int EPF = 0>
+template <typename T, int EPF = 0, bool RMAP = false>
 __device__ __forceinline__ void epilogue8(const GP& p, float (&v)[8], const float (&sc)[8], const float (&sh)[8],
-                                          int m, int64_t orow, int n, bf16x8 rpre = bf16x8{}, bf16x8 apre = bf16x8{}) {
+                                          int m, int64_t orow, int n, bf16x8 rpre = bf16x8{}, bf16x8 apre = bf16x8{}, int64_t rrow = 0) {
+    if constexpr (!RMAP) rrow = orow;
+    const bool has_res = p.residual != nullptr && (!RMAP || rrow >= 0);
     auto load_res = [&](float (&t)[8]) {
         if constexpr (EPF == 2) {
 #pragma unroll
             for (int r = 0; r < 8; ++r) t[r] = (float)rpre[r];
-        } else load8(reinterpret_cast<const T*>(p.residual) + orow * p.ldr + n, t);
+        } else load8(reinterpret_cast<const T*>(p.residual) + rrow * p.ldr + n, t);
     };
     auto load_aux = [&](const void* base, int64_t ld, float (&t)[8]) {
         if constexpr (EPF >= 1) {
@@ -867,7 +907,7 @@
 #pragma unroll
             for (int r = 0; r < 8; ++r) v[r] += t[r];
         }
-        if (p.residual) {
+        if (has_res) {
             load_res(t);
 #pragma unroll
             for (int r = 0; r < 8; ++r) v[r] += t[r];
@@ -948,7 +988,7 @@
 #pragma unroll
         for (int r = 0; r < 4; ++r) { v[r] *= d0[r]; v[4 + r] *= d1[r]; }
     }
-    if (p.residual) {
+    if (has_res) {
         float t[8];
         load_res(t);
 #pragma unroll
@@ -1032,10 +1072,12 @@
     constexpr uint32_t CESZ = (FLAGS & EF_F32) ? 4u : 2u;
     const uint32_t ldcb = (uint32_t)p.ldc * CESZ, ldc2b = (uint32_t)p.ldc2 * 2u, nb = (uint32_t)n * 2u;
     float sq = 0.f;
-    const rsrc_t rr = make_rsrc(HAS_RES ? p.residual : p.C, HAS_RES ? (uint32_t)((int64_t)p.M * p.ldr * 2) : 0u);
+    constexpr bool RMAP = (FLAGS & EF_RMAP) != 0, CMAP = (FLAGS & EF_CMAP) != 0;
+    const rsrc_t rr = make_rsrc(HAS_RES ? p.residual : p.C, HAS_RES ? (RMAP ? OOB : (uint32_t)((int64_t)p.M * p.ldr * 2)) : 0u);
     const void* auxp = (FLAGS & (EF_MASK | EF_RBWD)) ? p.mask : p.dact_pre;
     const int64_t lda = (FLAGS & (EF_MASK | EF_RBWD)) ? p.ldm : p.ldd;
-    const rsrc_t ra = make_rsrc(HAS_AUX ? auxp : p.C, HAS_AUX ? (uint32_t)((int64_t)p.M * lda * 2) : 0u);
+    const rsrc_t ra = make_rsrc(HAS_AUX ? auxp : p.C, HAS_AUX ? (CMAP ? OOB : (uint32_t)((int64_t)p.M * lda * 2)) : 0u);
+    auto out_row = [&](int m) __attribute__((always_inline)) { if constexpr (CMAP) return (uint32_t)p.c_rowmap[m]; else return (uint32_t)m; };
     const uint32_t ldrb = (uint32_t)p.ldr * 2u, ldab = (uint32_t)lda * 2u;
     f32x2 sc[4], sh[4];
 #pragma unroll
@@ -1067,11 +1109,14 @@
             const int slot = (ALL ? h * ITER : 0) + it;
             if constexpr (HAS_RES) {
                 if (ALL && pre_r) { union { bf16x8 x; u32x4 r; } u; u.x = pre_r[h * ITER + it]; res[slot] = u.r; }
-                else res[slot] = bload16(rr, ok ? (uint32_t)m * ldrb + nb : OOB);
+                else if constexpr (RMAP) {
+                    const int rm = ok ? p.res_rowmap[m] : -1;
+                    res[slot] = bload16(rr, rm >= 0 ? (uint32_t)rm * ldrb + nb : OOB);
+                } else res[slot] = bload16(rr, ok ? (uint32_t)m * ldrb + nb : OOB);
             }
             if constexpr (HAS_AUX) {
                 if (ALL && pre_a) { union { bf16x8 x; u32x4 r; } u; u.x = pre_a[h * ITER + it]; aux[slot] = u.r; }
-                else aux[slot] = bload16(ra, ok ? (uint32_t)m * ldab + nb : OOB);
+                else aux[slot] = bload16(ra, ok ? out_row(ok ? m : 0) * ldab + nb : OOB);
             }
         }
     };
@@ -1154,7 +1199,7 @@
                 else v[r] = v[r] * t[r];
             }
         }
-        __builtin_amdgcn_raw_buffer_store_b128(pack_bf16x8(v), rc, (uint32_t)m * ldcb + nb, 0, 16 );
+        __builtin_amdgcn_raw_buffer_store_b128(pack_bf16x8(v), rc, out_row(m) * ldcb + nb, 0, 16 );
     };
     auto pass = [&](int h) __attribute__((always_inline)) {
         if constexpr ((HAS_RES || HAS_AUX) && !ALL) request(h);
@@ -1198,10 +1243,11 @@
 }
 
 __host__ __device__ constexpr bool fe_in_form(int idx, int form) {
-    if (form == 1) return idx == 1 || idx == 2 || idx == 3 || idx == 4 || idx == 5 || idx == 8 || idx == 9 || idx == 10 || idx == 17;
-    if (form == 2) return idx == 1 || idx == 6 || idx == 7 || (idx >= 11 && idx <= 15);
+    if (form == 1) return idx == 1 || idx == 2 || idx == 3 || idx == 4 || idx == 5 || idx == 8 || idx == 9 || idx == 10 || idx == 17 || idx == 18;
+    if (form == 2) return idx == 1 || idx == 6 || idx == 7 || (idx >= 11 && idx <= 15) || idx == 19 || idx == 20;
     return true;
 }
+__host__ __device__ constexpr bool fe_for_threads(int idx, int nt) { return (FAST_EPI_COMBOS[idx] & (EF_RMAP | EF_CMAP)) == 0 || nt == NTHREADS; }
 template <int NT, int BN, int PR, int NPASS, bool WG = false, int FORM = 0, typename StageFn>
 __device__ __forceinline__ void fast_epilogue_dispatch(const GP& p, unsigned char* smem, int m0, int n0, int tid, StageFn stage,
                                                        const bf16x8* pre_r = nullptr, const bf16x8* pre_a = nullptr, int tile_lin = 0) {
@@ -1210,14 +1256,14 @@
         return;
     }
     switch (p.fast_epi) {
-#define CB_FE_CASE(I) case I: if constexpr (fe_in_form(I, FORM)) fast_epilogue<FAST_EPI_COMBOS[I], NT, BN, PR, NPASS>(p, smem, m0, n0, tid, stage, pre_r, pre_a); break;
+#define CB_FE_CASE(I) case I: if constexpr (fe_in_form(I, FORM) && fe_for_threads(I, NT)) fast_epilogue<FAST_EPI_COMBOS[I], NT, BN, PR, NPASS>(p, smem, m0, n0, tid, stage, pre_r, pre_a); break;
         CB_FE_CASE(1) CB_FE_CASE(2) CB_FE_CASE(3) CB_FE_CASE(4) CB_FE_CASE(5) CB_FE_CASE(6) CB_FE_CASE(7) CB_FE_CASE(8) CB_FE_CASE(9) CB_FE_CASE(10)
-        CB_FE_CASE(11) CB_FE_CASE(12) CB_FE_CASE(13) CB_FE_CASE(14) CB_FE_CASE(15) CB_FE_CASE(17)
+        CB_FE_CASE(11) CB_FE_CASE(12) CB_FE_CASE(13) CB_FE_CASE(14) CB_FE_CASE(15) CB_FE_CASE(17) CB_FE_CASE(18) CB_FE_CASE(19) CB_FE_CASE(20)
 #undef CB_FE_CASE
         default: break;
     }
 }
-static_assert(FAST_EPI_N == 18 && FAST_EPI_COMBOS[FAST_EPI_F32] == EF_F32, "fast_epilogue_dispatch lists every combination");
+static_assert(FAST_EPI_N == 21 && FAST_EPI_COMBOS[FAST_EPI_F32] == EF_F32, "fast_epilogue_dispatch lists every combination");
 
 template <int BM, int BN, bool WITH_R = true>
 struct EpiPre {
@@ -1243,7 +1289,8 @@
             if (m < p.M && n < p.N) {
                 const int64_t orow = p.c_rowmap ? (int64_t)p.c_rowmap[m] : (int64_t)m;
                 if constexpr (WITH_R) {
-                    if (p.residual) pre.r[h * E::ITER + it] = *reinterpret_cast<const bf16x8*>(reinterpret_cast<const T*>(p.residual) + orow * p.ldr + n);
+                    const int64_t rrow = p.res_rowmap ? (int64_t)p.res_rowmap[m] : orow;
+                    if (p.residual && rrow >= 0) pre.r[h * E::ITER + it] = *reinterpret_cast<const bf16x8*>(reinterpret_cast<const T*>(p.residual) + rrow * p.ldr + n);
                 }
                 if (aux) pre.a[h * E::ITER + it] = *reinterpret_cast<const bf16x8*>(reinterpret_cast<const T*>(aux) + orow * lda + n);
             }
@@ -1318,15 +1365,16 @@
                 }
                 if (m < p.M && nok) {
                     const int64_t orow = p.c_rowmap ? (int64_t)p.c_rowmap[m] : (int64_t)m;
+                    const int64_t rrow = p.res_rowmap ? (int64_t)p.res_rowmap[m] : orow;
                     float v[8];
                     load8(reinterpret_cast<const float*>(smem + rl * SROW + cc * 32), v);
                     if constexpr (EPF == 2) {
-                        if (use_pre) epilogue8<T, 2>(p, v, sc, sh, m, orow, n, rp, ap);
-                        else epilogue8<T>(p, v, sc, sh, m, orow, n);
+                        if (use_pre) epilogue8<T, 2, true>(p, v, sc, sh, m, orow, n, rp, ap, rrow);
+                        else epilogue8<T, 0, true>(p, v, sc, sh, m, orow, n, bf16x8{}, bf16x8{}, rrow);
                     } else if constexpr (EPF == 1) {
-                        if (use_pre) epilogue8<T, 1>(p, v, sc, sh, m, orow, n, bf16x8{}, ap);
-                        else epilogue8<T>(p, v, sc, sh, m, orow, n);
-                    } else epilogue8<T>(p, v, sc, sh, m, orow, n);
+                        if (use_pre) epilogue8<T, 1, true>(p, v, sc, sh, m, orow, n, bf16x8{}, ap, rrow);
+                        else epilogue8<T, 0, true>(p, v, sc, sh, m, orow, n, bf16x8{}, bf16x8{}, rrow);
+                    } else epilogue8<T, 0, true>(p, v, sc, sh, m, orow, n, bf16x8{}, bf16x8{}, rrow);
                 }
             }
         }
@@ -1367,10 +1415,11 @@
             const int m = m0 + wm * WM + i * 16 + (lane & 15);
             const bool mok = m < p.M;
             const int64_t orow = (mok && p.c_rowmap) ? (int64_t)p.c_rowmap[m] : (int64_t)m;
+            const int64_t rrow = (mok && p.res_rowmap) ? (int64_t)p.res_rowmap[m] : orow;
 #pragma unroll
             for (int j = 0; j < FN; ++j) {
                 const int nb = n0 + wn * WN + j * 16 + 4 * (lane >> 4);
-                if (mok) epilogue_vec<T>(p, acc[i][j], m, orow, nb);
+                if (mok) epilogue_vec<T, true>(p, acc[i][j], m, orow, nb, rrow);
             }
         }
     } else {
@@ -1392,7 +1441,7 @@
                 const int m = m0 + h * WM + rl, n = n0 + cl;
                 if (m < p.M && n < p.N) {
                     const int64_t orow = p.c_rowmap ? (int64_t)p.c_rowmap[m] : (int64_t)m;
-                    epilogue_elem<T>(p, stage[idx], m, orow, n);
+                    epilogue_elem<T, true>(p, stage[idx], m, orow, n, p.res_rowmap ? (int64_t)p.res_rowmap[m] : orow);
                 }
             }
         }
@@ -1418,6 +1467,7 @@
 #endif
     const int tile_lin = ((p.batch > 1 ? bid.bz / p.split_k : 0) * ((p.M + BM - 1) / BM) + bid.by) * ((p.N + BN - 1) / BN) + bid.bx;
     apply_batch(p, bid);
+    if constexpr (!LA::KROW && LB::KROW) dgrad_s2_class<BM, BK>(p, bid);
     const int m0 = bid.by * BM, n0 = bid.bx * BN;
     const int kt_per = (p.ktiles + p.split_k - 1) / p.split_k;
     const int kt0 = bid.bz * kt_per;
@@ -1744,7 +1794,7 @@
 
 template <typename T, int BM, int BN, int PF, int OCC, typename LA, typename LB, bool RS = false>
 int launch_k(const GP& p, hipStream_t st) {
-    dim3 grid((p.N + BN - 1) / BN, (p.M + BM - 1) / BM, p.split_k * (p.batch > 1 ? p.batch : 1));
+    dim3 grid((p.N + BN - 1) / BN, dgrad_s2_grid_y(p, BM), p.split_k * (p.batch > 1 ? p.batch : 1));
     hipLaunchKernelGGL((gemm_kernel<T, BM, BN, LA, LB, PF, RS, OCC>), grid, dim3(NTHREADS), 0, st, p);
     return cb_launch_status("cb_gemm");
 }
diff --git a/clipbert_amd/csrc/gemm_skinny.hip b/clipbert_amd/csrc/gemm_skinny.hip
--- a/clipbert_amd/csrc/gemm_skinny.hip
+++ b/clipbert_amd/csrc/gemm_skinny.hip
@@ -128,7 +128,7 @@
 
 bool skinny_covers(const cb_gemm_desc* d, const GP& p) {
     if (d->dtype != CB_BF16 || d->a_mode != CB_ROWK || (d->b_mode != CB_ROWK && d->b_mode != CB_KROW)) return false;
-    if (p.batch > 1 || p.split_k > 1 || d->zero_fill_pitch || d->a_rowsum || d->sq_slots || d->accumulate == 2) return false;
+    if (p.batch > 1 || p.split_k > 1 || d->zero_fill_pitch || d->a_rowsum || d->sq_slots || d->accumulate == 2 || d->res_rowmap) return false;
     if (d->b_mode == CB_KROW && !(d->N % 8 == 0 && d->ldb % 8 == 0 && aligned16(d->B))) return false;
     return true;
 }
diff --git a/clipbert_amd/gemm_log.py b/clipbert_amd/gemm_log.py
--- a/clipbert_amd/gemm_log.py
+++ b/clipbert_amd/gemm_log.py
@@ -28,6 +28,9 @@
     cnn = bool(d.scale) or bool(d.relu_bwd) or bool(d.a_tab) or bool(d.b_tab) or bool(d.c_rowmap) or d.zero_fill_pitch != 0 or bool(d.post_scale)
     M, N, K = int(d.M), int(d.N), int(d.K)
     K_alg = 147 if (d.a_mode == ops.ROWK_GATHER and int(d.R) == 7 and int(d.Cin) == 32 and K == 224) else K
+    s2 = bool(d.dgrad_s2)
+    if s2:
+        K_alg = K / 4
     cnn = cnn or (wgrad and K % 49 == 0 and K >= 49) or (not wgrad and M % 49 == 0 and M >= 49 * 16)
     if wgrad:
         fam = "weight gradients (linear + conv)"
@@ -40,9 +43,9 @@
         else:
             fam = "encoder linear (fwd + dgrad)"
         extra = sum(1 for p in (d.residual, d.mask, d.C2, d.gelu_grad_pre) if p) + (1 if d.accumulate else 0) + (2 if d.relu_bwd else 0)
-        alg = batch * ((M * K / taps + N * K) * esz + M * N * c_esz + extra * M * N * esz)
+        alg = batch * (((M // 4 if s2 else M) * K / taps + N * K) * esz + M * N * c_esz + extra * M * N * esz)
     return {"family": fam, "flop": 2.0 * M * N * K_alg * batch, "bytes": float(alg), "M": M, "N": N, "K": K, "batch": batch, "taps": taps,
-            "form": "wgrad" if wgrad else ("dgrad" if d.b_mode in (ops.KROW, ops.KROW_TAPS) else "fwd")}
+            "form": "wgrad" if wgrad else ("dgrad" if d.b_mode in (ops.KROW, ops.KROW_TAPS) else "fwd"), "s2": s2}
 
 
 class GemmLog:
diff --git a/clipbert_amd/modeling/cnn.py b/clipbert_amd/modeling/cnn.py
--- a/clipbert_amd/modeling/cnn.py
+++ b/clipbert_amd/modeling/cnn.py
@@ -7,7 +7,7 @@
 from ..data import RawFrames
 from ..ops import ACT_NONE, ACT_RELU, KROW, KROW_GATHER, KROW_TAPS, ROWK_GATHER
 from .modules import RESNET50_STAGES, BottleneckBlock, Conv2d, _Detectron2Model, _GridConv, as_config
-from .runtime import Runtime, _pick_split
+from .runtime import Runtime, _pick_split, even_pixel_index, even_pixel_rows, parity_class_rows
 
 
 def _out_hw(h, w, k, stride, pad):
@@ -24,7 +24,15 @@
     return kw
 
 
-def _conv_fwd(rt: Runtime, x, conv, act=ACT_NONE, residual=None, relu_after=False):
+class _ConvAs:
+    def __init__(self, conv, stride):
+        self.conv, self.stride = conv, stride
+
+    def __getattr__(self, name):
+        return getattr(self.conv, name)
+
+
+def _conv_fwd(rt: Runtime, x, conv, act=ACT_NONE, residual=None, relu_after=False, res_rowmap=None):
     n, h, w, cin = x.shape
     k, s, p = conv.k, conv.stride, conv.pad
     oh, ow = _out_hw(h, w, k, s, p)
@@ -33,26 +41,26 @@
     y = torch.empty(n, oh, ow, cout, dtype=x.dtype, device=x.device)
     wk = rt.bank.compute(conv.weight).view(cout, k * k * cin)
     scale, shift = conv.scale_shift()
-    res2d = residual.view(m, cout) if residual is not None else None
+    res2d = residual.view(-1, cout) if residual is not None else None
     plain = k == 1 and s == 1
     gather = {} if plain else conv_gather(rt, "a", n, h, w, cin, k, s, p, x.device)
     ops.gemm(x.view(m, cin) if plain else x, wk, m, cout, k * k * cin, out=y.view(m, cout), ldb=k * k * cin, **gather, scale=scale, shift=shift,
-             act=act, residual=res2d, relu_after=relu_after)
+             act=act, residual=res2d, relu_after=relu_after, res_rowmap=res_rowmap)
     return y
 
 
-def _conv_dgrad(rt: Runtime, g, conv, in_shape, scale=None, mask=None, residual=None, out=None, accumulate=False, fuse=None):
+def _conv_dgrad(rt: Runtime, g, conv, in_shape, scale=None, mask=None, residual=None, out=None, accumulate=False, fuse=None, res_rowmap=None):
     n, h, w, cin = in_shape
     _, oh, ow, cout = g.shape
     k, s, p = conv.k, conv.stride, conv.pad
     wk = rt.bank.compute(conv.weight).view(cout, k * k * cin)
     mi = n * h * w
     zfill = w if (k == 1 and s == 2 and h % 2 == 0 and w % 2 == 0 and cin % 8 == 0) else 0
-    alloc = torch.zeros if (s > 1 and not zfill) else torch.empty
+    alloc = torch.zeros if (k == 1 and s > 1 and not zfill) else torch.empty
     if out is None:
         out = alloc(n, h, w, cin, dtype=g.dtype, device=g.device)
     o2 = out.view(mi, cin)
-    r2 = residual.view(mi, cin) if residual is not None else None
+    r2 = residual.view(-1, cin) if residual is not None else None
     k2 = mask.view(mi, cin) if mask is not None else None
     extra = {}
     second = None
@@ -66,7 +74,12 @@
         rowmap = rt.strided_rowmap(n, h, w, oh, ow, s, g.device) if s > 1 else None
         ops.gemm(g.view(n * oh * ow, cout), wk, n * oh * ow, cin, cout, out=o2, b_mode=KROW_TAPS, ldb=cin, R=1, S=1,
                  Cin=cout, c_rowmap=rowmap, scale=scale, mask=k2, residual=r2, accumulate=accumulate, zero_fill_pitch=zfill if s > 1 else 0,
-                 **extra)
+                 res_rowmap=res_rowmap, **extra)
+    elif s == 2:
+        assert k == 3 and p == 1 and h == 2 * oh and w == 2 * ow and residual is None and fuse is None and not accumulate
+        ops.gemm(g, wk, mi, cin, 9 * cout, out=o2, b_mode=KROW_TAPS, ldb=9 * cin, dgrad_s2=True,
+                 **conv_gather(rt, "a", n, oh, ow, cout, 3, 1, 0, g.device, out_hw=(oh, ow)), c_rowmap=rt.rowmap(parity_class_rows, n, h, w, g.device),
+                 scale=scale, mask=k2)
     else:
         assert s == 1
         ops.gemm(g, wk, mi, cin, k * k * cout, out=o2, b_mode=KROW_TAPS, ldb=k * k * cin, flip_taps=True,
@@ -130,6 +143,44 @@
     c1, c2, c3 = blk.conv1, blk.conv2, blk.conv3
     return (c1.cout == 64 and c2.cin == 64 and c2.cout == 64 and c3.cout == 256 and c1.stride == 1 and c1.k == 1 and c2.k == 3 and c2.stride == 1
             and c3.k == 1 and c1.cin in (64, 256) and (blk.shortcut is not None) == (c1.cin == 64) and x.shape[-1] == c1.cin and x.is_contiguous())
+
+
+def _reads_even_pixels_only(blk: BottleneckBlock) -> bool:
+    sc, c1 = blk.shortcut, blk.conv1
+    return sc is not None and all(c.k == 1 and c.stride == 2 and c.pad == 0 for c in (sc, c1))
+
+
+def _tail_form(blk: BottleneckBlock, nxt: Optional[BottleneckBlock], x) -> bool:
+    c1, c2, c3 = blk.conv1, blk.conv2, blk.conv3
+    return (nxt is not None and _reads_even_pixels_only(nxt) and blk.shortcut is None and x.shape[1] % 2 == 0 and x.shape[2] % 2 == 0
+            and c1.k == 1 and c1.stride == 1 and c2.k == 3 and c2.stride == 1 and c2.pad == 1 and c3.k == 1 and c3.stride == 1
+            and c1.cin % 8 == 0 and c2.cin % 8 == 0 and c3.cin % 8 == 0)
+
+
+def blocks_forward(rt: Runtime, x, stages, save: bool, tail: bool = True):
+    saved = []
+    flat = [(blk, stage[i + 1] if i + 1 < len(stage) else (stages[si + 1][0] if si + 1 < len(stages) and stages[si + 1] else None), i + 1 == len(stage))
+            for si, stage in enumerate(stages) for i, blk in enumerate(stage)]
+    compact_in = False
+    for blk, nxt, last in flat:
+        if not compact_in and _res2_fusable(rt, x, blk, save):
+            x = _res2_block_fused(rt, x, blk)
+            continue
+        as_tail = tail and last and _tail_form(blk, nxt, x)
+        c1, csc = (_ConvAs(blk.conv1, 1), _ConvAs(blk.shortcut, 1)) if compact_in else (blk.conv1, blk.shortcut)
+        sc = _conv_fwd(rt, x, csc) if blk.shortcut is not None else x
+        y1 = _conv_fwd(rt, x, c1, act=ACT_RELU)
+        if as_tail:
+            n, h, w, _ = x.shape
+            y2 = _conv_fwd(rt, y1, _ConvAs(blk.conv2, 2), act=ACT_RELU)
+            out = _conv_fwd(rt, y2, blk.conv3, residual=sc, relu_after=True, res_rowmap=rt.rowmap(even_pixel_rows, n, h, w, x.device))
+        else:
+            y2 = _conv_fwd(rt, y1, blk.conv2, act=ACT_RELU)
+            out = _conv_fwd(rt, y2, blk.conv3, residual=sc, relu_after=True)
+        if save and _block_trainable(rt, blk):
+            saved.append((blk, x, y1, y2, out, as_tail, compact_in))
+        x, compact_in = out, as_tail
+    return x, saved
 
 
 def _stem_forward(bb: "GridFeatBackbone", x5):
@@ -170,19 +221,7 @@
     b, t = x5.shape[:2]
     net = bb.feature.backbone
     x = _stem_forward(bb, x5)
-    saved = []
-    for name, _nb, _mid, _cout, _s in RESNET50_STAGES:
-        for blk in getattr(net, name):
-            if _res2_fusable(rt, x, blk, save):
-                x = _res2_block_fused(rt, x, blk)
-                continue
-            sc = _conv_fwd(rt, x, blk.shortcut) if blk.shortcut is not None else x
-            y1 = _conv_fwd(rt, x, blk.conv1, act=ACT_RELU)
-            y2 = _conv_fwd(rt, y1, blk.conv2, act=ACT_RELU)
-            out = _conv_fwd(rt, y2, blk.conv3, residual=sc, relu_after=True)
-            if save and _block_trainable(rt, blk):
-                saved.append((blk, x, y1, y2, out))
-            x = out
+    x, saved = blocks_forward(rt, x, [list(getattr(net, name)) for name, *_ in RESNET50_STAGES], save)
     gconv = bb.grid_encoder[0]
     gy = _conv_fwd(rt, x, gconv)
     grid = ops.maxpool_fwd(gy, 2, 2, 0, relu=True)
@@ -211,37 +250,53 @@
         ops.gemm_group(pend, dg)
         pend.clear()
 
-    def fuse_spec(i):
-        b, _x, _y1, _y2, o = saved[i]
-        s3_, _ = b.conv3.scale_shift()
-        ssc_ = b.shortcut.scale_shift()[0] if b.shortcut is not None else None
-        return (o, s3_, ssc_)
-
-    g3, sec = _conv_dgrad(rt, dg, gconv, res5.shape, fuse=fuse_spec(len(saved) - 1))
+    g3, sec = _conv_dgrad(rt, dg, gconv, res5.shape, fuse=_fuse_spec(saved[-1]))
+    yield from blocks_backward(rt, saved, g3, sec, stage_of, flush, pend, first_res5)
+
+
+def _fuse_spec(rec):
+    b, o = rec[0], rec[4]
+    s3_, _ = b.conv3.scale_shift()
+    ssc_ = b.shortcut.scale_shift()[0] if b.shortcut is not None else None
+    return (o, s3_, ssc_)
+
+
+def blocks_backward(rt: Runtime, saved, g3, sec, stage_of, flush, pend, first_res5=None, dx_out=None):
     for idx in range(len(saved) - 1, -1, -1):
-        blk, x, y1, y2, out = saved[idx]
-        need_dx = idx > 0
+        blk, x, y1, y2, out, tail, compact_in = saved[idx]
+        need_dx = idx > 0 or dx_out is not None
         s2, _ = blk.conv2.scale_shift()
         s1, _ = blk.conv1.scale_shift()
         dz, gsc = (sec, None) if blk.shortcut is None else (None, sec)
+        c1, csc = (_ConvAs(blk.conv1, 1), _ConvAs(blk.shortcut, 1)) if compact_in else (blk.conv1, blk.shortcut)
+        c2 = _ConvAs(blk.conv2, 2) if tail else blk.conv2
         _conv_wgrad(rt, g3, y2, blk.conv3, pend)
         if blk.shortcut is not None:
-            _conv_wgrad(rt, gsc, x, blk.shortcut, pend)
+            _conv_wgrad(rt, gsc, x, csc, pend)
         g2 = _conv_dgrad(rt, g3, blk.conv3, y2.shape, scale=s2, mask=y2)
-        _conv_wgrad(rt, g2, y1, blk.conv2, pend)
-        g1 = _conv_dgrad(rt, g2, blk.conv2, y1.shape, scale=s1, mask=y1)
-        _conv_wgrad(rt, g1, x, blk.conv1, pend)
+        _conv_wgrad(rt, g2, y1, c2, pend)
+        g1 = _conv_dgrad(rt, g2, c2, y1.shape, scale=s1, mask=y1)
+        _conv_wgrad(rt, g1, x, c1, pend)
         if idx == 0 or stage_of.get(id(saved[idx - 1][0])) != stage_of.get(id(blk)):
             flush()
         if idx == first_res5 and idx > 0:
             yield "grid_encoder+res5"
         if need_dx:
-            spec = fuse_spec(idx - 1)
+            n, h, w, _ = x.shape
+            if idx > 0:
+                spec = _fuse_spec(saved[idx - 1])
             if blk.shortcut is None:
-                g3, sec = _conv_dgrad(rt, g1, blk.conv1, x.shape, residual=dz, fuse=spec)
+                rmap = dict(res_rowmap=rt.rowmap(even_pixel_index, n, h, w, x.device)) if tail else {}
+                if idx > 0:
+                    g3, sec = _conv_dgrad(rt, g1, c1, x.shape, residual=dz, fuse=spec, **rmap)
+                else:
+                    dx_out.append(_conv_dgrad(rt, g1, c1, x.shape, residual=dz, **rmap))
             else:
-                dout = _conv_dgrad(rt, g1, blk.conv1, x.shape)
-                g3, sec = _conv_dgrad(rt, gsc, blk.shortcut, x.shape, out=dout, accumulate=True, fuse=spec)
+                dout = _conv_dgrad(rt, g1, c1, x.shape)
+                if idx > 0:
+                    g3, sec = _conv_dgrad(rt, gsc, csc, x.shape, out=dout, accumulate=True, fuse=spec)
+                else:
+                    dx_out.append(_conv_dgrad(rt, gsc, csc, x.shape, out=dout, accumulate=True))
 
 
 class _CnnFn(torch.autograd.Function):
diff --git a/clipbert_amd/modeling/runtime.py b/clipbert_amd/modeling/runtime.py
--- a/clipbert_amd/modeling/runtime.py
+++ b/clipbert_amd/modeling/runtime.py
@@ -6,6 +6,22 @@
 from ..params import ParamBank
 
 _HOOK = {"encoder": "after_encoder_backward", "cnn": "after_res5_backward"}
+
+
+def even_pixel_rows(n, h, w):
+    return (torch.arange(n).view(n, 1, 1) * (h * w) + (torch.arange(0, h, 2)).view(1, -1, 1) * w + torch.arange(0, w, 2).view(1, 1, -1)).reshape(-1)
+
+
+def parity_class_rows(n, h, w):
+    even = even_pixel_rows(n, h, w)
+    return torch.cat([even + py * w + px for py in (0, 1) for px in (0, 1)])
+
+
+def even_pixel_index(n, h, w):
+    even = even_pixel_rows(n, h, w)
+    t = torch.full((n * h * w,), -1, dtype=torch.int64)
+    t[even] = torch.arange(even.numel())
+    return t
 
 
 class Runtime:
@@ -55,6 +71,13 @@
             self.rowmaps[key] = t
         return t
 
+    def rowmap(self, kind, n, h, w, device):
+        key = (kind.__name__, n, h, w, str(device))
+        t = self.rowmaps.get(key)
+        if t is None:
+            t = self.rowmaps[key] = kind(n, h, w).to(torch.int32).to(device)
+        return t
+
 
 def _pick_split(mo, no, kred):
     ktiles = (kred + 63) // 64
diff --git a/clipbert_amd/ops.py b/clipbert_amd/ops.py
--- a/clipbert_amd/ops.py
+++ b/clipbert_amd/ops.py
@@ -46,7 +46,8 @@
               sH=0, sW=0, flip_taps=False, c_rowmap=None, accumulate=False, split_k=1, act=ACT_NONE,
               scale=None, shift=None, residual=None, ldr=None, relu_after=False, mask=None, ldm=None,
               out2=None, ldc2=None, alpha=1.0, dropout_p=0.0, dropout_seed=0, seed_ptr=None, tile=0, gelu_grad_pre=None, a_rowsum=None, batch=1, batch_strides=None,
-              relu_bwd=False, post_scale=None, post_scale2=None, xcd_order=0, zero_fill_pitch=0, splitk_ws=None, schedule=0, sq_slots=None) -> GemmDesc:
+              relu_bwd=False, post_scale=None, post_scale2=None, xcd_order=0, zero_fill_pitch=0, splitk_ws=None, schedule=0, sq_slots=None,
+              res_rowmap=None, dgrad_s2=False) -> GemmDesc:
     d = GemmDesc()
     d.dtype = dtype_code(a.dtype)
     assert b.dtype == a.dtype
@@ -69,6 +70,10 @@
     d.scale, d.shift = _ptr(scale), _ptr(shift)
     d.residual = _ptr(residual)
     d.ldr = (ldr if ldr is not None else residual.stride(0)) if residual is not None else 0
+    if res_rowmap is not None:
+        assert residual is not None and res_rowmap.dtype == torch.int32 and res_rowmap.numel() == M
+        d.res_rowmap, d.res_rows = _ptr(res_rowmap), residual.shape[0]
+    d.dgrad_s2 = int(dgrad_s2)
     d.relu_after = int(relu_after)
     d.mask = _ptr(mask)
     d.ldm = (ldm if ldm is not None else mask.stride(0)) if mask is not None else 0
@@ -109,7 +114,7 @@
         assert sq_slots.dtype == torch.float32 and sq_slots.is_contiguous()
         d.sq_slots, d.sq_slots_n = _ptr(sq_slots), sq_slots.numel()
     d._refs = (a, b, out, a_tab, b_tab, c_rowmap, scale, shift, residual, mask, out2, seed_ptr, gelu_grad_pre, a_rowsum, post_scale,
-               post_scale2, splitk_ws, sq_slots)
+               post_scale2, splitk_ws, sq_slots, res_rowmap)
     return d
 
 
diff --git a/include/clipbert_hip.h b/include/clipbert_hip.h
--- a/include/clipbert_hip.h
+++ b/include/clipbert_hip.h
@@ -67,6 +67,9 @@
     int64_t splitk_ws_bytes;
     float* sq_slots;
     int64_t sq_slots_n;
+    const int32_t* res_rowmap;
+    int32_t res_rows;
+    int32_t dgrad_s2;
 } cb_gemm_desc;
 
 int cb_gemm(const cb_gemm_desc* d, void* stream);
```

After: 4244 clips/s (median of 6 runs). +2.8%, better.
